# takah29/3d-reconstruction-from-multi-view-exp

Measured on AMD Instinct MI355X. Metric: BA iterations/sec + residual-Jacobian GObs/s, 1M pts x 100 cams fp64, higher is better.
Workload: dtype f64

## Files before the change

### 3d-reconstruction-from-multi-view-exp_amd/csrc/mvba.hip

```cpp
#include <dlfcn.h>
#include <hip/hip_runtime.h>
#include <rccl/rccl.h>

#include <algorithm>
#include <atomic>
#include <chrono>
#include <cmath>
#include <cstdlib>
#include <cstring>
#include <thread>
#include <type_traits>
#include <utility>
#include <vector>

#include "mvba_common.h"
#include "mvba_host.h"

namespace mvba {
thread_local std::string g_err;
}
using namespace mvba;

namespace {
struct Rccl {
// ... 13 lines not shown
int rccl_load() {
  if (g_rccl.lib) return MVBA_OK;
  const char *names[] = {"librccl.so.1", "librccl.so"};
  void *lib = nullptr;
  std::string origin;
  for (const char *n : names)
    if (!lib && (lib = dlopen(n, RTLD_NOW | RTLD_NOLOAD))) origin = std::string(n) + " (already mapped by the process)";
  if (const char *ev = getenv("MVBA_RCCL_LIBRARY"))
    if (!lib && (lib = dlopen(ev, RTLD_NOW | RTLD_GLOBAL))) origin = ev;
  for (const char *n : {"/opt/rocm/lib/librccl.so.1", "librccl.so.1"})
    if (!lib && (lib = dlopen(n, RTLD_NOW | RTLD_GLOBAL))) origin = n;
  if (!lib) return fail(MVBA_ERR_RCCL, std::string("librccl not found: ") + dlerror());
  Rccl r;
  r.lib = lib;
  r.origin = origin;
#define BIND(field, sym)                                                                       \
  if (!(r.field = reinterpret_cast<decltype(r.field)>(dlsym(lib, sym))))                       \
    return fail(MVBA_ERR_RCCL, std::string("librccl (") + origin + ") lacks " + sym)
  BIND(GetVersion, "ncclGetVersion");
  BIND(GetUniqueId, "ncclGetUniqueId");
  BIND(CommInitRank, "ncclCommInitRank");
  BIND(CommDestroy, "ncclCommDestroy");
  BIND(AllReduce, "ncclAllReduce");
  BIND(AllGather, "ncclAllGather");
  BIND(GetErrorString, "ncclGetErrorString");
#undef BIND
  if (r.GetVersion(&r.version) != ncclSuccess) return fail(MVBA_ERR_RCCL, "ncclGetVersion failed");
  const int major = r.version >= 10000 ? r.version / 10000 : r.version / 1000;
  if (major != NCCL_MAJOR)
    return fail(MVBA_ERR_RCCL, "librccl (" + origin + ") is NCCL " + std::to_string(r.version) + ", this library was built against " +
                                   std::to_string(NCCL_VERSION_CODE));
  g_rccl = r;
  return MVBA_OK;
}
}

namespace {

__device__ __forceinline__ double wave_sum(double v) {
#pragma unroll
  for (int off = 32; off > 0; off >>= 1) v += __shfl_down(v, off, 64);
  return v;
}

__device__ __forceinline__ double block_sum(double v, double *s_red ) {
  v = wave_sum(v);
  const int lane = threadIdx.x & 63, w = threadIdx.x >> 6;
  if (lane == 0) s_red[w] = v;
  __syncthreads();
  double t = 0.0;
  if (threadIdx.x == 0) {
    const int nw = (blockDim.x + 63) >> 6;
    for (int i = 0; i < nw; ++i) t += s_red[i];
  }
  return t;
}

__device__ __forceinline__ void load_cams_to_lds(const double *__restrict__ cam15, int m, double f0,
                                                 double *s_cam) {
  for (int k = threadIdx.x; k < m; k += blockDim.x) expand_cam(cam15 + (size_t)k * CAM_IN, f0, s_cam + k * CAM_LDS);
}

__host__ __device__ __forceinline__ size_t strip_offset(int k, int m) {
  return 81 * ((size_t)k * m - (size_t)k * (k - 1) / 2);
}

__device__ __forceinline__ int keep_index(int i, int gauge_axis) {
  if (i < 3) return i;
  return (i + 6 < 12 + gauge_axis) ? i + 6 : i + 7;
}

#define MVBA_CONST_AS __attribute__((address_space(4)))
template <typename T>
__device__ __forceinline__ const T MVBA_CONST_AS *as_const(const T *p) {
#pragma clang diagnostic push
#pragma clang diagnostic ignored "-Wold-style-cast"
  return (const T MVBA_CONST_AS *)p;
#pragma clang diagnostic pop
}

constexpr int REC = 8;
constexpr int LDS_CAMERAS = 646;

#define MVBA_RESID_JAC_ARGS                                                                                                 \
  long long nobs, int m, const double *__restrict__ cam15, const double *__restrict__ X, const int *__restrict__ obs_pt,   \
      const int *__restrict__ cam_idx, const double2 *__restrict__ xy, double f0, const int *__restrict__ tile_start,     \
      int n_tiles, double2 *__restrict__ rec, double *__restrict__ PL, const int *__restrict__ tile_slot,                 \
      double *__restrict__ PLsplit, const double *__restrict__ gcam
struct LossArgs {
  double b;
  double *sqw;
};
template <bool GCAM, int LOSS = LOSS_SQUARED, typename... Robust>
__global__ __launch_bounds__(1024, 4) void k_resid_jac(MVBA_RESID_JAC_ARGS, Robust... robust) {
  extern __shared__ __attribute__((aligned(16))) double smem[];
  double *s_cam = smem;
  const int lane = threadIdx.x & 63, wave = threadIdx.x >> 6, nwave = blockDim.x >> 6;
  double2 *stage = reinterpret_cast<double2 *>(smem + (GCAM ? 0 : ((m * CAM_LDS + 1) & ~1))) + wave * (64 * REC);
  constexpr int CS = 65;
  double *contrib = reinterpret_cast<double *>(stage);
  int *seg_start = reinterpret_cast<int *>(contrib + 9 * CS), *seg_pt = seg_start + 66;
  if (!GCAM) {
    load_cams_to_lds(cam15, m, f0, s_cam);
    __syncthreads();
  }
  for (int tile = blockIdx.x * nwave + wave; tile < n_tiles; tile += gridDim.x * nwave) {
    const int ts0 = tile_start[tile], ts1 = tile_start[tile + 1];
    const bool split = ts0 < 0;
    const int slot = split ? as_const(tile_slot)[tile] : 0;
    const long long wbase = split ? ~ts0 : ts0;
    const int n = (int)((ts1 < 0 ? ~ts1 : ts1) - wbase);
    const long long o = wbase + lane;
    const bool live = lane < n;
    int a = -1;
    double c9[9] = {0, 0, 0, 0, 0, 0, 0, 0, 0};
    if (live) {
      a = obs_pt[o];
      const int k = cam_idx[o];
      const double2 z = xy[o];
      const double *Xa = X + 3 * (size_t)a;
      ObsJ J;
      obs_math(Xa[0], Xa[1], Xa[2], GCAM ? gcam + (size_t)k * CAM_LDS : s_cam + k * CAM_LDS, z.x, z.y, f0, J);
      if constexpr (LOSS != LOSS_SQUARED) {
        const LossArgs la = (robust, ...);
        const double sw = loss_sqrt_w<LOSS>(J.e0 * J.e0 + J.e1 * J.e1, la.b);
        J.e0 *= sw;
        J.e1 *= sw;
#pragma unroll
        for (int rr = 0; rr < 2; ++rr) {
#pragma unroll
          for (int i = 0; i < 3; ++i) J.jx[rr][i] *= sw;
          J.jc[rr][0] *= sw;
#pragma unroll
          for (int i = 6; i < 9; ++i) J.jc[rr][i] *= sw;
        }
        la.sqw[o] = sw;
      }
      double2 *row = stage + lane * REC;
      const int sw = lane & 7;
      row[0 ^ sw] = make_double2(J.jx[0][0], J.jx[1][0]);
      row[1 ^ sw] = make_double2(J.jx[0][1], J.jx[1][1]);
      row[2 ^ sw] = make_double2(J.jx[0][2], J.jx[1][2]);
      row[3 ^ sw] = make_double2(J.jc[0][0], J.jc[1][0]);
      row[4 ^ sw] = make_double2(J.jc[0][6], J.jc[1][6]);
      row[5 ^ sw] = make_double2(J.jc[0][7], J.jc[1][7]);
      row[6 ^ sw] = make_double2(J.jc[0][8], J.jc[1][8]);
      row[7 ^ sw] = make_double2(J.e0, J.e1);
      c9[0] = 2.0 * (J.jx[0][0] * J.jx[0][0] + J.jx[1][0] * J.jx[1][0]);
      c9[1] = 2.0 * (J.jx[0][0] * J.jx[0][1] + J.jx[1][0] * J.jx[1][1]);
      c9[2] = 2.0 * (J.jx[0][0] * J.jx[0][2] + J.jx[1][0] * J.jx[1][2]);
      c9[3] = 2.0 * (J.jx[0][1] * J.jx[0][1] + J.jx[1][1] * J.jx[1][1]);
      c9[4] = 2.0 * (J.jx[0][1] * J.jx[0][2] + J.jx[1][1] * J.jx[1][2]);
      c9[5] = 2.0 * (J.jx[0][2] * J.jx[0][2] + J.jx[1][2] * J.jx[1][2]);
      c9[6] = 2.0 * (J.jx[0][0] * J.e0 + J.jx[1][0] * J.e1);
      c9[7] = 2.0 * (J.jx[0][1] * J.e0 + J.jx[1][1] * J.e1);
      c9[8] = 2.0 * (J.jx[0][2] * J.e0 + J.jx[1][2] * J.e1);
    }
    wave_sync();
#pragma unroll
    for (int q = 0; q < REC; ++q) {
      const int ol = q * 8 + (lane >> 3), pos = lane & 7;
      const double2 v = stage[ol * REC + pos];
      if (ol < n) rec[(wbase + ol) * REC + (pos ^ (ol & 7))] = v;
    }
    wave_sync();
    const int a_prev = __shfl_up(a, 1, 64);
    const bool head = live && (lane == 0 || a != a_prev);
    const unsigned long long heads = __ballot(head);
    const int nseg = __popcll(heads);
#pragma unroll
    for (int q = 0; q < 9; ++q) contrib[q * CS + lane] = c9[q];
    if (head) {
      const int rank = __popcll(heads & ((1ull << lane) - 1ull));
      seg_start[rank] = lane;
      seg_pt[rank] = a;
    }
    if (lane == 0) seg_start[nseg] = n;
    wave_sync();
    const int sl = lane / 9, comp = lane - 9 * sl;
    for (int s0 = 0; s0 < nseg; s0 += 7) {
      const int sg = s0 + sl;
      if (sl < 7 && sg < nseg) {
        const int i0 = seg_start[sg], i1 = seg_start[sg + 1];
        double acc = 0.0;
        for (int i = i0; i < i1; ++i) acc += contrib[comp * CS + i];
        if (split) PLsplit[9 * (size_t)slot + comp] = acc;
        else PL[9 * (size_t)seg_pt[sg] + comp] = acc;
      }
    }
    wave_sync();
  }
}

__global__ void k_sum_split(int n_split, const int4 *__restrict__ splits ,
                            const double *__restrict__ PLsplit, double *__restrict__ PL) {
  const int t = blockIdx.x * blockDim.x + threadIdx.x, sp = t / 9, comp = t - 9 * sp;
  if (sp >= n_split) return;
  const int4 d = splits[sp];
  double v = 0.0;
  for (int q = 0; q < d.z; ++q) v += PLsplit[9 * (size_t)(d.y + q) + comp];
  PL[9 * (size_t)d.x + comp] = v;
}

constexpr int PBS = 16;
constexpr int PACE_STRIDE = 32;
__global__ __launch_bounds__(256) void k_point_inv(long long npts, double c, const double *__restrict__ PL,
                                                   double *__restrict__ PB, int *__restrict__ flag,
                                                   double *__restrict__ Ab, long long nAb, int *__restrict__ prog, long long nprog, int want_r) {
  __shared__ double2 s_out[256 * 8];
  double *s_in = reinterpret_cast<double *>(s_out);
  const long long a0 = (long long)blockIdx.x * 256, a = a0 + threadIdx.x;
  for (long long i = a; i < nAb; i += (long long)gridDim.x * blockDim.x) Ab[i] = 0.0;
  for (long long i = a; i < nprog; i += (long long)gridDim.x * blockDim.x) prog[i] = 0;
  if (a0 >= npts) return;
  const int np = (int)min<long long>(256, npts - a0);
  {
    double t[9];
#pragma unroll
    for (int i = 0; i < 9; ++i) t[i] = PL[9 * a0 + min((int)threadIdx.x + 256 * i, 9 * np - 1)];
#pragma unroll
    for (int i = 0; i < 9; ++i)
      if ((int)threadIdx.x + 256 * i < 9 * np) s_in[threadIdx.x + 256 * i] = t[i];
  }
  __syncthreads();
  double in[9];
#pragma unroll
  for (int i = 0; i < 9; ++i) in[i] = s_in[9 * min((int)threadIdx.x, np - 1) + i];
  __syncthreads();
  if (threadIdx.x < np) {
    const double s = 1.0 + c;
    const double xx = in[0] * s, xy = in[1], xz = in[2], yy = in[3] * s, yz = in[4], zz = in[5] * s;
    const double c00 = yy * zz - yz * yz, c01 = xz * yz - xy * zz, c02 = xy * yz - xz * yy;
    const double det = xx * c00 + xy * c01 + xz * c02;
    if (!(det != 0.0) || !isfinite(det)) atomicOr(flag, 1);
    const double id = 1.0 / det;
    const double i00 = c00 * id, i01 = c01 * id, i02 = c02 * id;
    const double i11 = (xx * zz - xz * xz) * id, i12 = (xy * xz - xx * yz) * id, i22 = (xx * yy - xy * xy) * id;
    const double g0 = in[6], g1 = in[7], g2 = in[8];
    double2 *out = s_out + 8 * threadIdx.x;
    const int sw = threadIdx.x & 7;
    out[0 ^ sw] = make_double2(i00, i01);
    out[1 ^ sw] = make_double2(i02, i11);
    out[2 ^ sw] = make_double2(i12, i22);
    out[3 ^ sw] = make_double2(i00 * g0 + i01 * g1 + i02 * g2, i01 * g0 + i11 * g1 + i12 * g2);
    out[4 ^ sw] = make_double2(i02 * g0 + i12 * g1 + i22 * g2, 1.0);
    if (want_r) {
      const double d0 = i00, q0 = d0 != 0.0 ? 1.0 / d0 : 0.0, l10 = i01 * q0, l20 = i02 * q0;
      const double d1 = i11 - l10 * i01, q1 = d1 != 0.0 ? 1.0 / d1 : 0.0, l21 = (i12 - l20 * i01) * q1;
      const double d2 = i22 - l20 * i02 - l21 * l21 * d1;
      const double a0 = sqrt(fabs(d0)), a1 = sqrt(fabs(d1)), a2 = sqrt(fabs(d2));
      out[4 ^ sw].y = 1.0 + (d0 < 0.0 ? 1.0 : 0.0) + (d1 < 0.0 ? 2.0 : 0.0) + (d2 < 0.0 ? 4.0 : 0.0);
      out[5 ^ sw] = make_double2(a0, l10 * a0);
      out[6 ^ sw] = make_double2(l20 * a0, a1);
      out[7 ^ sw] = make_double2(l21 * a1, a2);
    } else {
      out[5 ^ sw] = out[6 ^ sw] = out[7 ^ sw] = make_double2(0.0, 0.0);
    }
  }
  __syncthreads();
  double2 *dst = reinterpret_cast<double2 *>(PB + PBS * a0);
  for (int e = threadIdx.x; e < 8 * np; e += 256) {
    const int p = e >> 3, sl = e & 7;
    dst[e] = s_out[8 * p + (sl ^ (p & 7))];
  }
}


constexpr int PSTEP = 21;
constexpr int PROW = 7 * 16;
constexpr int PWAVE_LDS = PSTEP * (2 * PROW + 5 * 16);
constexpr int UNIT_STRIDE = 104;
constexpr int SLOT_BUF = PSTEP * (2 * PROW + 3 * 16);
constexpr int SLOT_IDX = 64;
constexpr int SLOT_IDX_RING = 3;
constexpr int PAIRS_LDS = 2 * PWAVE_LDS;
constexpr int SLOT_LDS = 3 * SLOT_BUF + SLOT_IDX_RING * SLOT_IDX * 4;
static_assert(9 * ((SLOT_LDS + 511) / 512 * 512) <= 160 * 1024, "nine waves per CU");

__device__ __forceinline__ void lds_dma16(const void *gsrc, void *lds_wave_uniform) {
  __builtin_amdgcn_global_load_lds(gsrc, (__attribute__((address_space(3))) void *)lds_wave_uniform, 16, 0, 0);
}

struct SlotPace {
  const int *seg_end;
  int *prog;
  int need, nseg, lag;
};
template <bool DIAG, bool BIG, bool SLOTS = false, bool ROBUST = false>
__device__ __forceinline__ void schur_pairs_unit(char *wbuf, const int lane, const long long beg, const int n,
                                                 const int *__restrict__ it_k, const int *__restrict__ it_l,
                                                 const int *__restrict__ it_a, const double2 *__restrict__ rec,
                                                 const double *__restrict__ PB, const double c, const double cu,
                                                 double *__restrict__ out, const int *__restrict__ slot_unit = nullptr,
                                                 const SlotPace pace = SlotPace{nullptr, nullptr, 0, 0, 2},
                                                 const double *__restrict__ sqw = nullptr) {
  static_assert(!(SLOTS && ROBUST), "the slot form has no robust build");
  constexpr int NPS = DIAG ? 5 : 3;
  const int it = lane / 3, cg = lane - 3 * it;
  const int drow = lane / 7, dslot = lane - 7 * drow;
  const int prow = lane / NPS, pslot = lane - NPS * prow;
  const int prow2 = (64 + lane) / 5, pslot2 = (64 + lane) - 5 * prow2;
  const int sel0 = cg == 0 ? 3 : (cg == 1 ? 0 : 4);
  const int sel1 = cg == 0 ? 0 : sel0 + 1, sel2 = cg == 0 ? 0 : sel0 + 2;
  const double al12 = cg == 0 ? 0.0 : 1.0, bx1 = cg == 0 ? 1.0 : 0.0;
  double acc[9][3];
#pragma unroll
  for (int i = 0; i < 9; ++i)
#pragma unroll
    for (int q = 0; q < 3; ++q) acc[i][q] = 0.0;
  double dg[3] = {0.0, 0.0, 0.0}, rb[3] = {0.0, 0.0, 0.0};

  constexpr int LB_OFF = PSTEP * PROW;
  constexpr int PB_OFF = LB_OFF + ((SLOTS && DIAG) ? PSTEP * 16 : PSTEP * PROW);
  constexpr int BUFSZ = SLOTS ? PB_OFF + PSTEP * 16 * NPS : PWAVE_LDS;
  static_assert(!SLOTS || BUFSZ <= SLOT_BUF, "slot form: staging buffer larger than the launch provides");
  constexpr int W_OFF = DIAG ? LB_OFF + PSTEP * 16 : PB_OFF + PSTEP * 16 * NPS;
  static_assert(!ROBUST || (DIAG ? W_OFF + PSTEP * 8 <= PB_OFF : W_OFF + 2 * PSTEP * 8 <= BUFSZ), "robust weights fit the staging buffer");
  int ixk[1][3], ixl[1][3], ixa[1][2];
  int ixw[2] = {0, 0};
  auto load_idx = [&](int s0, int (&xk)[3], int (&xl)[3], int (&xa)[2]) {
    const unsigned last = (unsigned)(min(PSTEP, n - s0) - 1);
    typedef const int __attribute__((address_space(1))) *gint_p;
    auto uni = [](const int *p) {
      const unsigned long long v = (unsigned long long)p;
      const unsigned lo = __builtin_amdgcn_readfirstlane((unsigned)v), hi = __builtin_amdgcn_readfirstlane((unsigned)(v >> 32));
      return (gint_p)(((unsigned long long)hi << 32) | lo);
    };
    typedef const char __attribute__((address_space(1))) *gchar_p;
    auto row_of = [&](int r) {
      unsigned off = min((unsigned)r, last) << 2;
      asm("" : "+v"(off));
      return off;
    };
    auto at = [](gint_p base, unsigned off) { return *(gint_p)((gchar_p)base + off); };
    const gint_p pk = uni(it_k + (beg + s0)), pl = DIAG ? pk : uni(it_l + (beg + s0)), pa = uni(it_a + (beg + s0));
#pragma unroll
    for (int q = 0; q < 3; ++q) {
      const unsigned row = row_of(9 * q + drow);
      xk[q] = at(pk, row);
      if (!DIAG) xl[q] = at(pl, row);
    }
    if (DIAG) xl[0] = at(pk, row_of(lane));
    xa[0] = at(pa, row_of(prow));
    if (DIAG) xa[1] = at(pa, row_of(prow2));
    if (ROBUST) {
      ixw[0] = at(pk, row_of(lane >> 1));
      if (!DIAG) ixw[1] = at(pl, row_of(lane >> 1));
// ... 1945 lines not shown
    if (FILL && lo < NONE && lane == 0)
      while (sg < nSeg && lo >= o_lo + (sg + 1) * segG) seg_end[b * nSeg + sg++] = steps;
    if (lo >= NONE) break;
    const bool take = k0 < NONE && k0 <= lo + skew;
    if (FILL && slot) {
      const long long o = (base + steps) * PSTEP + lane;
      st_k[o] = take ? (int)(it_k[cur] - o_lo) : pad_obs;
      st_l[o] = take ? (int)(it_l[cur] - o_lo) : pad_obs;
      st_a[o] = take ? it_a[cur] : pad_pt;
    }
    if (take) {
      ++cur;
      k0 = k1;
      k1 = cur + 1 < end ? key_at(cur + 1) : NONE;
    }
    ++steps;
  }
  if (FILL) {
    if (lane == 0)
      while (sg < nSeg) seg_end[b * nSeg + sg++] = steps;
  } else if (lane == 0) {
    w_steps[b] = steps;
  }
}

__global__ void k_idx_interleave(long long n_steps, const int *__restrict__ st_k, const int *__restrict__ st_l, const int *__restrict__ st_a,
                                 int *__restrict__ out) {
  const long long t = (long long)blockIdx.x * blockDim.x + threadIdx.x;
  if (t >= n_steps * SLOT_IDX) return;
  const long long st = t / SLOT_IDX;
  const int e = (int)(t - st * SLOT_IDX), which = e / PSTEP, sl = e - which * PSTEP;
  const int *src = which == 0 ? st_k : (which == 1 ? st_l : st_a);
  out[t] = which < 3 ? src[st * PSTEP + sl] : 0;
}

#include "mvba_cov.h"
#include "mvba_map.h"

}

enum { SCHUR_PAIRS = 1, SCHUR_SLOTS = 2, SCHUR_DENSE = 3 };
struct mvba_handle {
  int device = 0;
  hipStream_t stream = nullptr;
  DevBufs mem;
  long long N = 0, nobs = 0;
  int m = 0, gauge_axis = 0, D = 0, ld = 0;
  double f0 = 1.0;
  long long *d_pt_ptr = nullptr;
  int *d_cam = nullptr, *d_obs_pt = nullptr;
  double2 *d_xy = nullptr;
  int *d_tiles = nullptr;
  int *d_tile_slot = nullptr;
  int4 *d_splits = nullptr;
  double *d_PLsplit = nullptr;
  int n_splits = 0;
  int n_tiles = 0;
  bool any_split = false;
  int k1_threads = 512;
  bool use_pairs = true;
  int schur_mode = 2;
  long long n_items = 0, n_items_offdiag = 0, n_slot_items = 0;
  int n_units = 0, rccl_version = 0, q_max = 0, n_waves = 0, slot_nR = 8, slot_nseg = 0;
  long long *d_range_o0 = nullptr;
  int *d_seg_end = nullptr, *d_prog = nullptr;
  bool check_solve = false;
  double check_solve_tol = 1e-8;
  bool gcam = false;
  double *d_cam18 = nullptr, *d_dxi10 = nullptr;
  bool index_on_device = false;
  int4 *d_wdesc = nullptr;
  int *d_it_x = nullptr;
  int *d_wunits = nullptr;
  bool force_big = false;
  int *d_it_k = nullptr, *d_it_l = nullptr, *d_it_a = nullptr, *d_unit_ptr = nullptr, *d_q_ptr = nullptr, *d_q_units = nullptr;
  int4 *d_units = nullptr;
  double *d_partial = nullptr;
  double *d_dense_part = nullptr;
  int *d_dense_obs = nullptr;
  int dense_blocks = 0, dense_tiles = 0;
  double *d_X[2] = {nullptr, nullptr}, *d_cam15[2] = {nullptr, nullptr};
  int cur = 0;
  bool have_params = false, linearized = false, have_trial = false;
  double2 *d_rec = nullptr;
  double *d_PL = nullptr, *d_PB = nullptr;
  double *d_Ab = nullptr, *d_Ared = nullptr, *d_Ztiles = nullptr, *d_Lblk = nullptr, *d_dxi = nullptr, *d_dX = nullptr, *d_lu = nullptr;
  int *d_ipiv = nullptr;
  double *d_partials = nullptr, *d_cost = nullptr, *h_cost = nullptr;
  double *d_mail = nullptr;
  unsigned long long cost_seq = 0;
  bool mail_pending = false;
  int n_partials = 0, cost_grid = 0;
  int *d_flag = nullptr, *h_flag = nullptr;
  unsigned *d_bar = nullptr;
  int n_cu = 1;
  bool chol_onepass = true;
  int trail64_min = 200;
  unsigned barrier_polls = 1u << 22;
  ncclComm_t comm = nullptr;
  mvba_host_allreduce_fn host_ar = nullptr;
  void *host_ar_user = nullptr;
  std::vector<double> host_buf;
  int rank = 0, nranks = 1;
  double *d_allcost = nullptr, *h_allcost = nullptr, *d_sim = nullptr;
  std::vector<double *> snap_slabs;
  long long n_snap = 0;
  int profiling = 0;
  mvba_stats stats{};
  struct Ev { int kid; hipEvent_t a, b; };
  std::vector<Ev> pending;
  std::vector<hipEvent_t> pool;
  double *d_cov_sig = nullptr, *d_cov_panel = nullptr, *d_cov_pts = nullptr, *d_cov_cam = nullptr;
  int loss = LOSS_SQUARED;
  double loss_b = 0.0;
  double *d_sqw = nullptr;
  double2 *d_resid = nullptr;
  double *d_init_cams = nullptr;
  bool mapped = false;
  int n_free = 0, map_ld = 0, map_U = 0;
  std::vector<int> map_col, map_ptr, map_mem;
  int *d_map_col = nullptr, *d_map_ptr = nullptr, *d_map_mem = nullptr;
  double *d_map_x = nullptr, *d_cov_sigv = nullptr;
  int2 *d_map_pairs = nullptr;
  double *d_map_part = nullptr;
  int n_map_pairs = 0, map_nblk = 1;
  int solve_D() const { return mapped ? n_free : D; }
  int solve_ld() const { return mapped ? map_ld : ld; }
};

namespace {

const char *kKernelNames[MVBA_K_COUNT] = {"resid_jac", "point_blocks", "point_inv", "schur",
                                          "allreduce", "solve",        "backsub_cost", "cost"};

struct Timed {
  mvba_handle *h;
  int kid;
  hipEvent_t a = nullptr, b = nullptr;
  bool on = false;
  Timed(mvba_handle *h_, int kid_) : h(h_), kid(kid_) {
    on = kid >= 0 && (h->profiling == 1 || (h->profiling == 2 && (kid == MVBA_K_SCHUR || kid == MVBA_K_RESID_JAC)));
    if (!on) return;
    auto get = [&]() {
      hipEvent_t e;
      if (!h->pool.empty()) { e = h->pool.back(); h->pool.pop_back(); }
      else hipEventCreate(&e);
      return e;
    };
    a = get(); b = get();
    hipEventRecord(a, h->stream);
  }
  ~Timed() {
    if (!on) return;
    hipEventRecord(b, h->stream);
    h->pending.push_back({kid, a, b});
  }
};

void drain_events(mvba_handle *h) {
  for (auto &p : h->pending) {
    float ms = 0.f;
    if (hipEventElapsedTime(&ms, p.a, p.b) == hipSuccess) {
      h->stats.ms[p.kid] += ms;
      h->stats.launches[p.kid] += 1;
    }
    h->pool.push_back(p.a);
// ... 15 lines not shown
}

double *cost_mail(mvba_handle *h) {
  if (h->comm || h->host_ar || h->profiling == 1 || !h->d_mail) return nullptr;
  ++h->cost_seq;
  h->mail_pending = true;
  return h->d_mail;
}

int global_cost(mvba_handle *h, double *E) {
  if (h->mail_pending) {
    h->mail_pending = false;
    volatile unsigned long long *seq = reinterpret_cast<volatile unsigned long long *>(h->h_cost + 2);
    const auto t0 = std::chrono::steady_clock::now();
    bool seen = false;
    for (unsigned spins = 0;; ++spins) {
      if (*seq == h->cost_seq) { seen = true; break; }
      if ((spins & 1023) == 1023 && std::chrono::steady_clock::now() - t0 > std::chrono::seconds(2)) break;
      cpu_relax();
    }
    if (seen) {
      std::atomic_thread_fence(std::memory_order_acquire);
      drain_events(h);
      *E = h->h_cost[0];
      return MVBA_OK;
    }
    int rc = sync_and_drain(h);
    if (rc) return rc;
    *E = h->h_cost[0];
    return MVBA_OK;
  }
  if (h->comm) {
    Timed t(h, MVBA_K_ALLREDUCE);
    ncclResult_t r = g_rccl.AllGather(h->d_cost, h->d_allcost, 2, ncclDouble, h->comm, h->stream);
    if (r != ncclSuccess) return fail(MVBA_ERR_RCCL, std::string("ncclAllGather: ") + g_rccl.GetErrorString(r));
    MVBA_HIP(hipMemcpyAsync(h->h_allcost, h->d_allcost, 2 * sizeof(double) * h->nranks, hipMemcpyDeviceToHost, h->stream));
  } else {
    MVBA_HIP(hipMemcpyAsync(h->h_cost, h->d_cost, 2 * sizeof(double), hipMemcpyDeviceToHost, h->stream));
  }
  int rc = sync_and_drain(h);
  if (rc) return rc;
  if (h->host_ar) {
    std::vector<double> v(2 * (size_t)h->nranks, 0.0);
    v[2 * h->rank] = h->h_cost[0];
    v[2 * h->rank + 1] = (double)*h->h_flag;
    if (h->host_ar(h->host_ar_user, v.data(), (int64_t)v.size())) return fail(MVBA_ERR_RCCL, "host all-reduce callback failed");
    double s = 0.0;
    int fl = 0;
    for (int i = 0; i < h->nranks; ++i) { s += v[2 * i]; fl |= (int)v[2 * i + 1]; }
    *E = s;
    *h->h_flag = fl;
  } else if (h->comm) {
    double s = 0.0;
    int fl = 0;
    for (int i = 0; i < h->nranks; ++i) {
      s += h->h_allcost[2 * i];
      int f;
      memcpy(&f, &h->h_allcost[2 * i + 1], sizeof(int));
      fl |= f;
    }
    *E = s;
    *h->h_flag = fl;
  } else {
    *E = *h->h_cost;
  }
  return MVBA_OK;
}

template <typename... A>
struct LossKernel {
  void (*squared)(A...);
  void (*robust)(A..., LossArgs);
  const void *fn(bool rb) const { return rb ? (const void *)robust : (const void *)squared; }
};
template <typename... A>
LossKernel<A...> loss_kernel(void (*squared)(A...), void (*robust)(A..., LossArgs)) { return {squared, robust}; }

template <typename... A, typename... Args>
void launch_loss(mvba_handle *h, LossKernel<A...> k, dim3 grid, dim3 block, size_t lds, Args... args) {
  if (h->loss != LOSS_SQUARED) hipLaunchKernelGGL(k.robust, grid, block, lds, h->stream, args..., LossArgs{h->loss_b, h->d_sqw});
  else hipLaunchKernelGGL(k.squared, grid, block, lds, h->stream, args...);
}

auto resid_jac_kernel(bool gcam, int loss) {
  if (loss == LOSS_CAUCHY)
    return gcam ? loss_kernel(k_resid_jac<true>, k_resid_jac<true, LOSS_CAUCHY, LossArgs>) : loss_kernel(k_resid_jac<false>, k_resid_jac<false, LOSS_CAUCHY, LossArgs>);
  return gcam ? loss_kernel(k_resid_jac<true>, k_resid_jac<true, LOSS_HUBER, LossArgs>) : loss_kernel(k_resid_jac<false>, k_resid_jac<false, LOSS_HUBER, LossArgs>);
}
auto cost_kernel(bool gcam, int loss) {
  if (loss == LOSS_CAUCHY)
    return gcam ? loss_kernel(k_cost<true>, k_cost<true, LOSS_CAUCHY, LossArgs>) : loss_kernel(k_cost<false>, k_cost<false, LOSS_CAUCHY, LossArgs>);
  return gcam ? loss_kernel(k_cost<true>, k_cost<true, LOSS_HUBER, LossArgs>) : loss_kernel(k_cost<false>, k_cost<false, LOSS_HUBER, LossArgs>);
}
template <int G>
auto backsub_kernel_g(int bt, bool gcam) {
  if (gcam) return loss_kernel(k_backsub<G, 256, true>, k_backsub<G, 256, true, true, LossArgs>);
  if (bt == 1024) return loss_kernel(k_backsub<G, 1024>, k_backsub<G, 1024, false, true, LossArgs>);
  if (bt == 512) return loss_kernel(k_backsub<G, 512>, k_backsub<G, 512, false, true, LossArgs>);
  return loss_kernel(k_backsub<G>, k_backsub<G, 256, false, true, LossArgs>);
}
auto backsub_kernel(int G, int bt, bool gcam) {
  return G == 2 ? backsub_kernel_g<2>(bt, gcam) : (G == 4 ? backsub_kernel_g<4>(bt, gcam) : backsub_kernel_g<8>(bt, gcam));
}
template <int T>
auto dense_kernel_t(bool table) {
  return table ? loss_kernel(k_schur_dense<T, true>, k_schur_dense<T, true, true, LossArgs>)
               : loss_kernel(k_schur_dense<T, false>, k_schur_dense<T, false, true, LossArgs>);
}
auto dense_kernel(int T, bool table) {
  switch (T) {
    case 1: return dense_kernel_t<1>(table);
    case 2: return dense_kernel_t<2>(table);
    case 3: return dense_kernel_t<3>(table);
    case 4: return dense_kernel_t<4>(table);
    case 5: return dense_kernel_t<5>(table);
    case 6: return dense_kernel_t<6>(table);
    case 7: return dense_kernel_t<7>(table);
    case 8: return dense_kernel_t<8>(table);
    case 9: return dense_kernel_t<9>(table);
    case 10: return dense_kernel_t<10>(table);
    case 11: return dense_kernel_t<11>(table);
    default: return dense_kernel_t<12>(table);
  }
}
size_t dense_lds_bytes(int T, int mm) {
  const int CH = dense_ch(T);
  return sizeof(double) * ((size_t)2 * 3 * CH * 16 * T + (size_t)2 * CH * mm * 32) + sizeof(double2) * CH * ((size_t)mm * REC + 8) +
         sizeof(double) * (CH * (size_t)mm + 2 * 3 * CH);
}

size_t k1_lds_bytes(int m, bool gcam, int threads) {
  return (size_t)((gcam ? 0 : ((m * CAM_LDS + 1) & ~1)) + (threads / 64) * 64 * 2 * REC) * sizeof(double);
}
size_t cam_lds_bytes(int m, bool gcam, bool with_dxi) { return gcam ? 0 : (size_t)m * (CAM_LDS + (with_dxi ? DXI_LDS : 0)) * sizeof(double); }

void cam_tables(mvba_handle *h, const double *cam15, const double *dxi) {
  if (h->gcam) hipLaunchKernelGGL(k_cam_tables, dim3((h->m + 255) / 256), dim3(256), 0, h->stream, h->m, cam15, dxi, h->f0, h->d_cam18, h->d_dxi10);
}
int launch_cost(mvba_handle *h, const double *cam15, const double *X) {
  const size_t lds = cam_lds_bytes(h->m, h->gcam, false);
  cam_tables(h, cam15, nullptr);
  launch_loss(h, cost_kernel(h->gcam, h->loss), dim3(h->cost_grid), dim3(lds > 40 * 1024 ? 512 : 256), lds, h->nobs, h->m, cam15, X,
              h->d_obs_pt, h->d_cam, h->d_xy, h->f0, h->d_partials, h->d_cam18);
  double *mail = cost_mail(h);
  const unsigned long long seq = h->cost_seq;
  hipLaunchKernelGGL(k_sum_partials, dim3(1), dim3(1024), 0, h->stream, h->d_partials, h->cost_grid, h->d_cost, h->d_flag, mail, seq);
  MVBA_HIP(hipGetLastError());
  return MVBA_OK;
}

struct CreateKnobs {
  bool schur_set = false;
  bool schur_slots = false, schur_pairs = false, schur_dense = false;
  bool index_host = false, index_global = false;
  bool force_big = false;
  bool chol_launches = false;
  int trail64_min = 200;
  unsigned barrier_polls = 1u << 22;
  bool check_solve = false;
  double check_solve_tol = 1e-8;
  bool timing = false;
};

CreateKnobs read_create_knobs() {
  CreateKnobs k;
  auto is = [](const char *ev, const char *v) { return ev && !strcmp(ev, v); };
  const char *schur = getenv("MVBA_SCHUR");
  k.schur_set = schur != nullptr;
  k.schur_slots = is(schur, "slots");
  k.schur_pairs = is(schur, "pairs");
  k.schur_dense = is(schur, "dense");
  const char *index = getenv("MVBA_INDEX");
  k.index_host = is(index, "host");
  k.index_global = is(index, "global");
  k.force_big = getenv("MVBA_FORCE_BIG") != nullptr;
  k.chol_launches = is(getenv("MVBA_CHOL"), "launches");
  if (const char *ev = getenv("MVBA_TRAIL64_MIN")) k.trail64_min = std::max(0, atoi(ev));
  if (const char *ev = getenv("MVBA_CHOL_BARRIER_POLLS")) k.barrier_polls = (unsigned)std::max(0LL, atoll(ev));
  if (const char *ev = getenv("MVBA_CHECK_SOLVE")) {
    const double v = atof(ev);
    k.check_solve = v != 0.0;
    if (v > 0.0 && v < 1.0) k.check_solve_tol = v;
  }
  k.timing = getenv("MVBA_CREATE_TIMING") != nullptr;
  return k;
}

#include "mvba_create.h"

}

extern "C" {

const char *mvba_version(void) { return "mvba 0.2 (gfx950)"; }
const char *mvba_last_error(void) { return g_err.c_str(); }
const char *mvba_kernel_name(int32_t k) { return (k >= 0 && k < MVBA_K_COUNT) ? kKernelNames[k] : ""; }

int mvba_device_count(int32_t *count) {
  int n = 0;
  hipError_t e = hipGetDeviceCount(&n);
  if (e != hipSuccess) {
    *count = 0;
    return fail(MVBA_ERR_HIP, std::string("hipGetDeviceCount: ") + hipGetErrorString(e));
  }
  *count = n;
  return MVBA_OK;
}

int mvba_create(const mvba_problem *p, mvba_handle **out) { return create_engine(p, LOSS_SQUARED, 0.0, out); }

int mvba_create_robust(const mvba_problem *p, int32_t loss, double scale, mvba_handle **out) {
  if (!p || !out) return fail(MVBA_ERR_BADARG, "null argument");
  if (loss == LOSS_SQUARED) return create_engine(p, LOSS_SQUARED, 0.0, out);
  if (loss != LOSS_HUBER && loss != LOSS_CAUCHY)
    return fail(MVBA_ERR_BADARG, "loss = " + std::to_string(loss) + " is not a loss (0 squared, 1 Huber, 2 Cauchy)");
  if (!(scale > 0.0) || !std::isfinite(scale))
    return fail(MVBA_ERR_BADARG, "loss scale = " + std::to_string(scale) + " must be finite and > 0 for a robust loss");
  if (!(p->f0 > 0.0) || !std::isfinite(p->f0)) return fail(MVBA_ERR_BADARG, "a robust loss needs f0 > 0");
  const double r = scale / p->f0;
  return create_engine(p, loss, r * r, out);
}

void mvba_destroy(mvba_handle *h) {
  if (!h) return;
  hipSetDevice(h->device);
  if (h->stream) hipStreamSynchronize(h->stream);
  if (h->comm) g_rccl.CommDestroy(h->comm);
  h->mem.release_all();
  if (h->h_cost) hipHostFree(h->h_cost);
  if (h->h_allcost) hipHostFree(h->h_allcost);
  for (auto &p : h->pending) { hipEventDestroy(p.a); hipEventDestroy(p.b); }
  for (auto e : h->pool) hipEventDestroy(e);
  if (h->stream) hipStreamDestroy(h->stream);
  delete h;
}

int mvba_set_params(mvba_handle *h, const double *X, const double *f, const double *u, const double *t, const double *R) {
  if (!h || !X || !f || !u || !t || !R) return fail(MVBA_ERR_BADARG, "null argument");
  MVBA_HIP(hipSetDevice(h->device));
  std::vector<double> cam((size_t)h->m * CAM_IN);
  for (int k = 0; k < h->m; ++k) {
    double *c = cam.data() + (size_t)k * CAM_IN;
    c[0] = f[k]; c[1] = u[2 * k]; c[2] = u[2 * k + 1];
    for (int i = 0; i < 3; ++i) c[3 + i] = t[3 * k + i];
    for (int i = 0; i < 9; ++i) c[6 + i] = R[9 * k + i];
  }
  MVBA_HIP(hipMemcpyAsync(h->d_X[h->cur], X, sizeof(double) * 3 * h->N, hipMemcpyHostToDevice, h->stream));
  MVBA_HIP(hipMemcpyAsync(h->d_cam15[h->cur], cam.data(), sizeof(double) * cam.size(), hipMemcpyHostToDevice, h->stream));
  MVBA_HIP(hipStreamSynchronize(h->stream));
  h->have_params = true; h->linearized = false; h->have_trial = false;
  return MVBA_OK;
}

int mvba_get_params(mvba_handle *h, double *X, double *f, double *u, double *t, double *R) {
  if (!h || !X || !f || !u || !t || !R) return fail(MVBA_ERR_BADARG, "null argument");
  if (!h->have_params) return fail(MVBA_ERR_STATE, "no parameters set");
  MVBA_HIP(hipSetDevice(h->device));
  std::vector<double> cam((size_t)h->m * CAM_IN);
  MVBA_HIP(hipMemcpyAsync(X, h->d_X[h->cur], sizeof(double) * 3 * h->N, hipMemcpyDeviceToHost, h->stream));
  MVBA_HIP(hipMemcpyAsync(cam.data(), h->d_cam15[h->cur], sizeof(double) * cam.size(), hipMemcpyDeviceToHost, h->stream));
  MVBA_HIP(hipStreamSynchronize(h->stream));
  for (int k = 0; k < h->m; ++k) {
    const double *c = cam.data() + (size_t)k * CAM_IN;
    f[k] = c[0]; u[2 * k] = c[1]; u[2 * k + 1] = c[2];
    for (int i = 0; i < 3; ++i) t[3 * k + i] = c[3 + i];
    for (int i = 0; i < 9; ++i) R[9 * k + i] = c[6 + i];
  }
  return MVBA_OK;
}

int mvba_apply_similarity(mvba_handle *h, const double *R0, const double *t0, double scale) {
  if (!h || !R0 || !t0) return fail(MVBA_ERR_BADARG, "null argument");
  if (!h->have_params) return fail(MVBA_ERR_STATE, "no parameters set");
  MVBA_HIP(hipSetDevice(h->device));
  double T[13];
  memcpy(T, R0, 9 * sizeof(double));
  memcpy(T + 9, t0, 3 * sizeof(double));
  T[12] = scale;
  if (!h->d_sim) {
    int rc = h->mem.alloc(&h->d_sim, 13);
    if (rc) return rc;
  }
  MVBA_HIP(hipMemcpyAsync(h->d_sim, T, sizeof(T), hipMemcpyHostToDevice, h->stream));
  const long long n = std::max<long long>(h->N, h->m);
  hipLaunchKernelGGL(k_similarity, dim3((unsigned)((n + 255) / 256)), dim3(256), 0, h->stream, h->N, h->m, h->d_X[h->cur],
                     h->d_cam15[h->cur], h->d_sim);
  MVBA_HIP(hipGetLastError());
  MVBA_HIP(hipStreamSynchronize(h->stream));
  h->linearized = false; h->have_trial = false;
  return MVBA_OK;
}

int mvba_cost(mvba_handle *h, double *E) {
  if (!h || !E) return fail(MVBA_ERR_BADARG, "null argument");
  if (!h->have_params) return fail(MVBA_ERR_STATE, "no parameters set");
  MVBA_HIP(hipSetDevice(h->device));
  {
    Timed t(h, MVBA_K_COST);
    int rc = launch_cost(h, h->d_cam15[h->cur], h->d_X[h->cur]);
    if (rc) return rc;
  }
  return global_cost(h, E);
}

namespace {
void launch_resid_jac(mvba_handle *h) {
  const int kt = h->k1_threads;
  cam_tables(h, h->d_cam15[h->cur], nullptr);
  const int wpb = kt / 64;
  const int grid = std::max(1, std::min(2048 * 256 / kt, (h->n_tiles + wpb - 1) / wpb));
  launch_loss(h, resid_jac_kernel(h->gcam, h->loss), dim3(grid), dim3(kt), k1_lds_bytes(h->m, h->gcam, kt), h->nobs, h->m, h->d_cam15[h->cur],
              h->d_X[h->cur], h->d_obs_pt, h->d_cam, h->d_xy, h->f0, h->d_tiles, h->n_tiles, h->d_rec, h->d_PL,
              h->d_tile_slot, h->d_PLsplit, h->d_cam18);
  if (h->n_splits)
    hipLaunchKernelGGL(k_sum_split, dim3((9 * h->n_splits + 255) / 256), dim3(256), 0, h->stream, h->n_splits, h->d_splits,
                       h->d_PLsplit, h->d_PL);
}

void launch_point_inv(mvba_handle *h, double c) {
  const int m = h->m;
  const size_t n9 = 9 * (size_t)m, nA = strip_offset(m, m);
  const long long nAb = (long long)(nA + n9);
  const unsigned grid = (unsigned)std::max<long long>((h->N + 255) / 256, std::min<long long>((nAb + 1023) / 1024, 4096));
  hipLaunchKernelGGL(k_point_inv, dim3(std::max(grid, 1u)), dim3(256), 0, h->stream, h->N, c, h->d_PL, h->d_PB, h->d_flag,
                     h->d_Ab, nAb, h->d_prog, (long long)h->slot_nR * h->slot_nseg * PACE_STRIDE,
                     h->schur_mode == SCHUR_DENSE ? 1 : 0);
}

void launch_schur(mvba_handle *h, double c) {
  const int m = h->m;
  const size_t nA = strip_offset(m, m);
  double *d_A = h->d_Ab, *d_b = h->d_Ab + nA;
  if (h->use_pairs) {
    const bool big = (std::max<long long>(h->nobs, h->N) + 1) * 128LL >= (1LL << 32) || h->force_big;
    if (h->schur_mode == SCHUR_SLOTS) {
      if (h->n_waves)
        hipLaunchKernelGGL(k_schur_slots, dim3(h->n_waves), dim3(64), SLOT_LDS, h->stream, h->d_wdesc,
                           h->d_wunits, h->d_it_x, (const int *)nullptr, (const int *)nullptr, h->d_rec, h->d_PB, c, h->f0, h->d_partial,
                           h->slot_nR, h->d_seg_end, h->d_prog, h->slot_nseg, SLOT_LAG, h->d_range_o0);
    } else if (h->n_units) {
      auto launch = [&](auto kern, auto... robust) {
        hipLaunchKernelGGL(kern, dim3(8 * h->q_max), dim3(64), PAIRS_LDS, h->stream, h->d_units, h->d_q_ptr, h->d_q_units, h->d_it_k, h->d_it_l,
                           h->d_it_a, h->d_rec, h->d_PB, c, h->f0, h->d_partial, robust...);
      };
      if (h->loss != LOSS_SQUARED) launch(big ? k_schur_pairs_big_robust : k_schur_pairs_robust, (const double *)h->d_sqw);
      else launch(big ? k_schur_pairs_big : k_schur_pairs);
    }
    hipLaunchKernelGGL(k_schur_reduce, dim3((unsigned)((long long)m * (m + 1) / 2)), dim3(128), 0, h->stream, m, h->d_unit_ptr,
                       h->d_partial, d_A, d_b);
  } else if (h->schur_mode == SCHUR_DENSE) {
    const int T = (9 * m + 15) / 16;
    launch_loss(h, dense_kernel(T, h->d_dense_obs != nullptr), dim3(h->dense_blocks), dim3(64 * (dense_consumers(T) + dense_ch(T))), dense_lds_bytes(T, m),
                (const double2 *)h->d_rec, (const double *)h->d_PB, (const int *)h->d_dense_obs, (long long)h->N, m, 1.0 / h->f0, h->d_dense_part);
    const long long n_el = (long long)nA + 9 * m;
    hipLaunchKernelGGL(k_schur_dense_finish, dim3((unsigned)((n_el + 3) / 4)), dim3(256), 0, h->stream, m, T, h->dense_blocks,
                       (const double *)h->d_dense_part, c, d_A, d_b);
  }
}

int allreduce_Ab(mvba_handle *h, bool timed) {
  const int m = h->m;
  const size_t n9 = 9 * (size_t)m, nA = strip_offset(m, m);
  if (h->comm) {
    Timed t(h, timed ? MVBA_K_ALLREDUCE : -1);
    ncclResult_t r = g_rccl.AllReduce(h->d_Ab, h->d_Ab, nA + n9, ncclDouble, ncclSum, h->comm, h->stream);
    if (r != ncclSuccess) return fail(MVBA_ERR_RCCL, std::string("ncclAllReduce: ") + g_rccl.GetErrorString(r));
  } else if (h->host_ar) {
    h->host_buf.resize(nA + n9);
    MVBA_HIP(hipMemcpyAsync(h->host_buf.data(), h->d_Ab, sizeof(double) * (nA + n9), hipMemcpyDeviceToHost, h->stream));
    MVBA_HIP(hipStreamSynchronize(h->stream));
    const auto t0 = std::chrono::steady_clock::now();
    if (h->host_ar(h->host_ar_user, h->host_buf.data(), (int64_t)(nA + n9))) return fail(MVBA_ERR_RCCL, "host all-reduce callback failed");
    MVBA_HIP(hipMemcpyAsync(h->d_Ab, h->host_buf.data(), sizeof(double) * (nA + n9), hipMemcpyHostToDevice, h->stream));
    if (timed && h->profiling) {
      h->stats.ms[MVBA_K_ALLREDUCE] += std::chrono::duration<double, std::milli>(std::chrono::steady_clock::now() - t0).count();
      h->stats.launches[MVBA_K_ALLREDUCE] += 1;
    }
  }
  return MVBA_OK;
}

void launch_map_tied(mvba_handle *h, double *M, int ld, int mirror) {
  if (!h->n_map_pairs) return;
  hipLaunchKernelGGL(k_map_tied, dim3(h->n_map_pairs, h->map_nblk), dim3(256), 0, h->stream, h->m, (const double *)h->d_Ab,
                     (const int *)h->d_map_ptr, (const int *)h->d_map_mem, (const int2 *)h->d_map_pairs, h->d_map_part);
  hipLaunchKernelGGL(k_map_tied_finish, dim3((h->n_map_pairs + 255) / 256), dim3(256), 0, h->stream, h->n_map_pairs, h->map_nblk, ld,
                     mirror, (const int2 *)h->d_map_pairs, (const double *)h->d_map_part, M);
}

void launch_factor(mvba_handle *h) {
  const int m = h->m, D = h->solve_D();
  double *d_A = h->d_Ab, *d_b = h->d_Ab + strip_offset(m, m);
  const int ld = h->solve_ld();
  const int ntc = (D + NB - 1) / NB;
  if (h->mapped) {
    const int U = h->map_U, ntu = (U + NB - 1) / NB;
    hipLaunchKernelGGL(k_map_compact, dim3(ntu * (ntu + 1) / 2 + (D + 255) / 256), dim3(256), 0, h->stream, D, ld, m, U, ntu, d_A, d_b,
                       h->d_map_ptr, h->d_map_mem, h->d_Ared, h->d_bar, 1 + 4 * ((D + SBW - 1) / SBW));
    if (U < D)
      hipLaunchKernelGGL(k_map_rows, dim3((D + 63) / 64, D - U), dim3(256), 0, h->stream, D, ld, m, U, d_A, h->d_map_ptr, h->d_map_mem,
                         h->d_Ared);
    launch_map_tied(h, h->d_Ared, ld, 0);
  } else
  hipLaunchKernelGGL(k_compact, dim3(ntc * (ntc + 1) / 2 + (D + 255) / 256), dim3(256), 0, h->stream, D, ld, m, h->gauge_axis, ntc, d_A, d_b,
                     h->d_Ared, h->d_bar, 1 + 4 * ((D + SBW - 1) / SBW));
  for (int jS = 0; jS < D; jS += SBW) {
    const int jE = std::min(jS + SBW, D);
    hipLaunchKernelGGL(k_chol_super, dim3((D + 1 - jE + 63) / 64), dim3(SUPER_THREADS), SUPER_LDS, h->stream, h->d_Ared, ld, D, jS,
                       h->d_Ztiles + (size_t)(jS / NB) * NB * NB, h->d_Lblk + (size_t)(jS / SBW) * SBW * SBW, h->d_flag);
    if (jE < D) {
      const int nt32 = (D + 1 - jE + NB - 1) / NB, nt64 = (D + 1 - jE + TB - 1) / TB;
      if (jE - jS == SBW && nt64 * (nt64 + 1) / 2 >= h->trail64_min)
        hipLaunchKernelGGL(k_chol_trail64, dim3(nt64 * (nt64 + 1) / 2), dim3(256), TRAIL64_LDS, h->stream, h->d_Ared, ld, D, jS, jE);
      else
        hipLaunchKernelGGL(k_chol_trail32, dim3(nt32 * (nt32 + 1) / 2), dim3(256), 0, h->stream, h->d_Ared, ld, D, jS, jE);
    }
  }
}
}

int mvba_linearize(mvba_handle *h) {
  if (!h) return fail(MVBA_ERR_BADARG, "null handle");
  if (!h->have_params) return fail(MVBA_ERR_STATE, "no parameters set");
  MVBA_HIP(hipSetDevice(h->device));
  if (h->nobs) {
    Timed t(h, MVBA_K_RESID_JAC);
    launch_resid_jac(h);
  }
  MVBA_HIP(hipGetLastError());
  h->linearized = true; h->have_trial = false;
  h->stats.n_linearize++;
  return MVBA_OK;
}

namespace {
double *solve_x(mvba_handle *h) { return h->mapped ? h->d_map_x : h->d_dxi; }
void launch_expand(mvba_handle *h) {
  const size_t n9 = 9 * (size_t)h->m;
  if (h->mapped && h->solve_D() > 0)
    hipLaunchKernelGGL(k_map_expand, dim3((unsigned)((n9 + 255) / 256)), dim3(256), 0, h->stream, (int)n9, h->gauge_axis, h->d_map_col,
                       h->d_map_x, h->d_dxi);
}

void launch_solve(mvba_handle *h, bool onepass) {
  const int m = h->m, D = h->solve_D();
  double *d_x = solve_x(h);
  Timed t(h, MVBA_K_SOLVE);
  if (D == 0) {
    hipMemsetAsync(h->d_dxi, 0, sizeof(double) * 9 * (size_t)m, h->stream);
    return;
  }
  launch_factor(h);
  const int ld = h->solve_ld();
  const int S = (D + SBW - 1) / SBW;
  if (onepass && (S == 1 || S < h->n_cu)) {
    const int ngrp = ((S - 1) * SBW + 31) / 32, nbulk = S > 1 ? std::max(1, std::min(h->n_cu - S, ngrp)) : 0;
    hipLaunchKernelGGL(k_chol_backsolve_all<true>, dim3(S + nbulk), dim3(SUPER_THREADS),
                       BACKSOLVE_LDS, h->stream, h->d_Ared, ld, D, m, h->gauge_axis, h->d_Ztiles, h->d_Lblk, d_x, h->d_flag,
                       h->d_bar, h->barrier_polls);
  } else
  for (int jS = ((D - 1) / SBW) * SBW; jS >= 0; jS -= SBW) {
    const int jE = std::min(jS + SBW, D), jE2 = std::min(jE + SBW, D);
    const int nwg = (jE == D) ? 1 : 1 + (jS + 255) / 256;
    hipLaunchKernelGGL(k_chol_backsolve, dim3(nwg), dim3(256), 0, h->stream, h->d_Ared, ld, D, m, h->gauge_axis, h->d_Ztiles,
                       h->d_Lblk + (size_t)(jS / SBW) * SBW * SBW, d_x, jS, jE, jE2);
  }
  launch_expand(h);
}

int launch_lu_solve(mvba_handle *h) {
  const int m = h->m, D = h->solve_D();
  double *d_A = h->d_Ab, *d_b = h->d_Ab + strip_offset(m, m), *d_x = solve_x(h);
  if (!h->d_lu) {
    int rc_ = h->mem.alloc(&h->d_lu, (size_t)h->D * (h->D + 1));
    if (rc_) return rc_;
    rc_ = h->mem.alloc(&h->d_ipiv, (size_t)h->D);
    if (rc_) return rc_;
  }
  MVBA_HIP(hipMemsetAsync(h->d_flag, 0, sizeof(int), h->stream));
  Timed t(h, MVBA_K_SOLVE);
  if (h->mapped) {
    hipLaunchKernelGGL(k_map_full, dim3((D + 1 + 255) / 256, D), dim3(256), 0, h->stream, D, m, d_A, d_b, h->d_map_ptr, h->d_map_mem, h->d_lu);
    launch_map_tied(h, h->d_lu, D + 1, 1);
  } else
  hipLaunchKernelGGL(k_compact_full, dim3((D + 1 + 255) / 256, D), dim3(256), 0, h->stream, D, m, h->gauge_axis, d_A, d_b, h->d_lu);
  for (int j0 = 0; j0 < D; j0 += LU_NB) {
    const int nb = std::min(LU_NB, D - j0), right = D + 1 - (j0 + nb);
    hipLaunchKernelGGL(k_lu_panel, dim3(1), dim3(1024), 0, h->stream, h->d_lu, D, j0, nb, h->d_ipiv, h->d_flag);
    hipLaunchKernelGGL(k_lu_swap, dim3((D + 1 - nb + 255) / 256), dim3(256), 0, h->stream, h->d_lu, D, j0, nb, h->d_ipiv);
    if (right > 0) hipLaunchKernelGGL(k_lu_trsm, dim3((right + 255) / 256), dim3(256), 0, h->stream, h->d_lu, D, j0, nb);
    const int below = D - (j0 + nb);
    if (below > 0)
      hipLaunchKernelGGL(k_lu_gemm, dim3((right + 63) / 64, (below + 63) / 64), dim3(256), 0, h->stream, h->d_lu, D, j0, nb);
  }
  hipLaunchKernelGGL(k_lu_backsub, dim3(1), dim3(1024), 0, h->stream, h->d_lu, D, m, h->gauge_axis, d_x);
  launch_expand(h);
  return MVBA_OK;
}

int launch_tail_and_cost(mvba_handle *h, double *E_trial) {
  const int m = h->m, trial = 1 - h->cur;
  {
    Timed t(h, MVBA_K_BACKSUB_COST);
    hipLaunchKernelGGL(k_update_cams, dim3((m + 63) / 64), dim3(64), 0, h->stream, m, h->d_cam15[h->cur], h->d_dxi,
                       h->d_cam15[trial]);
    if (h->N) {
      const size_t lds = cam_lds_bytes(m, h->gcam, true);
      cam_tables(h, h->d_cam15[h->cur], h->d_dxi);
      const double deg = (double)h->nobs / (double)h->N;
      const int G = deg <= 40.0 ? 2 : (deg <= 100.0 ? 4 : 8);
      const int bt = lds > 80 * 1024 ? 1024 : (lds > 40 * 1024 ? 512 : 256);
      const int nblk = (int)std::min<long long>(4096 * 256 / bt, (h->N * G + bt - 1) / bt);
      launch_loss(h, backsub_kernel(G, bt, h->gcam), dim3(nblk), dim3(bt), lds, h->N, m, h->d_pt_ptr, h->d_cam, h->d_PB, h->d_dxi,
                  h->d_X[h->cur], h->d_cam15[h->cur], h->f0, h->d_X[trial], h->d_dX, h->d_cam18, h->d_dxi10);
    }
    int rc = launch_cost(h, h->d_cam15[trial], h->d_X[trial]);
    if (rc) return rc;
  }
  return global_cost(h, E_trial);
}

int check_solve_residual(mvba_handle *h) {
  const int m = h->m, D = h->solve_D();
  const size_t n9 = 9 * (size_t)m, nA = strip_offset(m, m);
  std::vector<double> Ab(nA + n9), x(n9);
  MVBA_HIP(hipMemcpyAsync(Ab.data(), h->d_Ab, sizeof(double) * (nA + n9), hipMemcpyDeviceToHost, h->stream));
  MVBA_HIP(hipMemcpyAsync(x.data(), h->d_dxi, sizeof(double) * n9, hipMemcpyDeviceToHost, h->stream));
  MVBA_HIP(hipStreamSynchronize(h->stream));
  auto kept = [&](size_t g) { return !((g >= 3 && g <= 8) || g == (size_t)(12 + h->gauge_axis)); };
  std::vector<double> r(n9, 0.0), an(n9, 0.0);
  for (int k = 0; k < m; ++k) {
    const double *Ak = Ab.data() + strip_offset(k, m);
    const int Wk = 9 * (m - k);
    for (int i = 0; i < 9; ++i)
      for (int c = 0; c < Wk; ++c) {
        const size_t gi = 9 * (size_t)k + i, gj = 9 * (size_t)k + c;
        const double a = Ak[(size_t)i * Wk + c];
        r[gi] += a * x[gj]; an[gi] += std::fabs(a * x[gj]);
        if (c >= 9) { r[gj] += a * x[gi]; an[gj] += std::fabs(a * x[gi]); }
      }
  }
  double worst = 0.0;
  if (h->mapped) {
    for (int j = 0; j < D; ++j) {
      double res = 0.0, scale = 0.0;
      for (int q = h->map_ptr[j]; q < h->map_ptr[j + 1]; ++q) {
        const size_t g = (size_t)h->map_mem[q];
        res += Ab[nA + g] - r[g];
        scale += an[g] + std::fabs(Ab[nA + g]);
      }
      worst = std::max(worst, scale > 0.0 ? std::fabs(res) / scale : 0.0);
    }
  } else
  for (size_t g = 0; g < n9; ++g)
    if (kept(g)) {
      const double bg = Ab[nA + g], scale = an[g] + std::fabs(bg);
      worst = std::max(worst, scale > 0.0 ? std::fabs(bg - r[g]) / scale : 0.0);
    }
  if (!(worst <= h->check_solve_tol))
    return fail(MVBA_ERR_STATE, "MVBA_CHECK_SOLVE: the dense solve left a relative residual of " + std::to_string(worst) +
                                    " on the reduced camera system (a stale hand-over in the back-substitution?)");
  return MVBA_OK;
}
}

int mvba_try_step(mvba_handle *h, double c, double *E_trial) {
  if (!h || !E_trial) return fail(MVBA_ERR_BADARG, "null argument");
  if (!h->linearized) return fail(MVBA_ERR_STATE, "try_step before linearize");
  MVBA_HIP(hipSetDevice(h->device));
  {
    Timed t(h, MVBA_K_POINT_INV);
    launch_point_inv(h, c);
  }
  if (h->use_pairs || h->schur_mode == SCHUR_DENSE) {
    Timed t(h, MVBA_K_SCHUR);
    launch_schur(h, c);
  }
  MVBA_HIP(hipGetLastError());
  int rc = allreduce_Ab(h, true);
  if (rc) return rc;
  launch_solve(h, h->chol_onepass);
  MVBA_HIP(hipGetLastError());
  h->stats.n_try_step++;
  rc = launch_tail_and_cost(h, E_trial);
  if (rc) return rc;
  if ((*h->h_flag & 8) && !(*h->h_flag & 1)) {
    MVBA_HIP(hipMemsetAsync(h->d_flag, 0, sizeof(int), h->stream));
    h->chol_onepass = false;
    h->stats.n_barrier_fallback++;
    launch_solve(h, false);
    rc = launch_tail_and_cost(h, E_trial);
    if (rc) return rc;
  }
  if ((*h->h_flag & 2) && !(*h->h_flag & (1 | 8))) {
    rc = launch_lu_solve(h);
    if (rc) return rc;
    h->stats.n_lu_fallback++;
    rc = launch_tail_and_cost(h, E_trial);
    if (rc) return rc;
  }
  if (*h->h_flag) {
    const int fl = *h->h_flag;
    hipMemsetAsync(h->d_flag, 0, sizeof(int), h->stream);
    if (fl & 8) return fail(MVBA_ERR_HIP, "k_chol_backsolve_all: a wait for a progress word timed out twice (is another process holding the CUs?)");
    return fail(MVBA_ERR_SINGULAR, (fl & 1) ? "Singular matrix" : "Singular matrix (reduced camera system)");
  }
  if (h->check_solve) {
    rc = check_solve_residual(h);
    if (rc) return rc;
  }
  h->have_trial = true;
  return MVBA_OK;
}

int mvba_commit(mvba_handle *h) {
  if (!h) return fail(MVBA_ERR_BADARG, "null handle");
  if (!h->have_trial) return fail(MVBA_ERR_STATE, "commit without a trial step");
  h->cur = 1 - h->cur;
  h->have_trial = false; h->linearized = false;
  h->stats.n_commit++;
  return MVBA_OK;
}

int mvba_set_parameter_map(mvba_handle *h, const int32_t *col, int32_t n_free) {
  if (!h) return fail(MVBA_ERR_BADARG, "null handle");
  MVBA_HIP(hipSetDevice(h->device));
  const int m = h->m, n9 = 9 * m;
  auto is_gauge = [&](int g) { return (g >= 3 && g <= 8) || g == 12 + h->gauge_axis; };
  if (!col) {
    h->mapped = false;
    h->have_trial = false;
    return MVBA_OK;
  }
  if (n_free < 0 || n_free > h->D)
    return fail(MVBA_ERR_BADARG, "mvba_set_parameter_map: n_free = " + std::to_string(n_free) + " must be in 0 .. 9 n_images - 7 = " + std::to_string(h->D));
  std::vector<int> cnt(n_free + 1, 0), first(n_free, -1);
  for (int g = 0; g < n9; ++g) {
    const int j = col[g];
    if (j < -1 || j >= n_free)
      return fail(MVBA_ERR_BADARG, "mvba_set_parameter_map: col[" + std::to_string(g) + "] = " + std::to_string(j) + " is neither -1 nor below n_free = " + std::to_string(n_free));
    if (j >= 0 && is_gauge(g))
      return fail(MVBA_ERR_BADARG, "mvba_set_parameter_map: col[" + std::to_string(g) + "] is a gauge slot and must be -1");
    if (j < 0) continue;
    if (first[j] < 0) first[j] = g;
    else if (g % 9 != first[j] % 9 || g % 9 > 2)
      return fail(MVBA_ERR_BADARG, "mvba_set_parameter_map: col[" + std::to_string(g) + "] ties slot " + std::to_string(g) + " to slot " + std::to_string(first[j]) +
                                       " (unknown " + std::to_string(j) + "): only the same intrinsic parameter (f, u or v) of different cameras can be tied");
    ++cnt[j];
  }
  for (int j = 0; j < n_free; ++j)
    if (!cnt[j]) return fail(MVBA_ERR_BADARG, "mvba_set_parameter_map: unknown " + std::to_string(j) + " has no parameter slot");
  bool is_default = n_free == h->D;
  for (int g = 0, j = 0; is_default && g < n9; ++g) is_default = col[g] == (is_gauge(g) ? -1 : j++);
  h->have_trial = false;
  if (is_default) {
    h->mapped = false;
    return MVBA_OK;
  }
  std::vector<int> ptr(n_free + 1, 0), mem;
  for (int j = 0; j < n_free; ++j) ptr[j + 1] = ptr[j] + cnt[j];
  mem.resize(std::max(ptr[n_free], 1));
  {
    std::vector<int> fill(ptr.begin(), ptr.end() - 1);
    for (int g = 0; g < n9; ++g)
      if (col[g] >= 0) mem[fill[col[g]]++] = g;
  }
  int U = 0;
  while (U < n_free && cnt[U] == 1) ++U;
  std::vector<int2> pairs;
  int max_cnt = 1;
  {
    std::vector<int> tied;
    for (int j = 0; j < n_free; ++j)
      if (cnt[j] > 1) { tied.push_back(j); max_cnt = std::max(max_cnt, cnt[j]); }
    for (size_t a = 0; a < tied.size(); ++a)
      for (size_t b = 0; b <= a; ++b) pairs.push_back(make_int2(tied[a], tied[b]));
  }
  const int nblk = std::min(64, (max_cnt + 7) / 8);
  int2 *d_pairs = nullptr;
  double *d_part = nullptr;
  if (!pairs.empty()) {
    int rc = h->mem.alloc(&d_pairs, pairs.size());
    if (!rc) rc = h->mem.alloc(&d_part, pairs.size() * (size_t)nblk);
    if (rc) {
      h->mem.release(d_pairs);
      return rc;
    }
  }
  if (!h->d_map_col) {
    int rc = h->mem.alloc(&h->d_map_col, (size_t)n9);
    if (!rc) rc = h->mem.alloc(&h->d_map_ptr, (size_t)h->D + 1);
    if (!rc) rc = h->mem.alloc(&h->d_map_mem, (size_t)n9);
    if (!rc) rc = h->mem.alloc(&h->d_map_x, (size_t)n9 + 16);
    if (rc) {
      h->mem.release(h->d_map_col); h->mem.release(h->d_map_ptr); h->mem.release(h->d_map_mem); h->mem.release(h->d_map_x);
      h->mem.release(d_pairs); h->mem.release(d_part);
      return rc;
    }
  }
  MVBA_HIP(hipStreamSynchronize(h->stream));
  h->mem.release(h->d_map_pairs);
  h->mem.release(h->d_map_part);
  h->d_map_pairs = d_pairs;
  h->d_map_part = d_part;
  h->n_map_pairs = (int)pairs.size();
  h->map_nblk = nblk;
  if (!pairs.empty()) MVBA_HIP(hipMemcpy(h->d_map_pairs, pairs.data(), sizeof(int2) * pairs.size(), hipMemcpyHostToDevice));
  MVBA_HIP(hipMemcpy(h->d_map_col, col, sizeof(int) * n9, hipMemcpyHostToDevice));
  MVBA_HIP(hipMemcpy(h->d_map_ptr, ptr.data(), sizeof(int) * (n_free + 1), hipMemcpyHostToDevice));
  MVBA_HIP(hipMemcpy(h->d_map_mem, mem.data(), sizeof(int) * mem.size(), hipMemcpyHostToDevice));
  h->map_col.assign(col, col + n9);
  h->map_ptr = ptr;
  h->map_mem = mem;
  h->n_free = n_free;
  h->map_ld = (n_free + 3) & ~3;
  h->map_U = U;
  h->mapped = true;
  return MVBA_OK;
}

int mvba_residuals(mvba_handle *h, double *e) {
  if (!h || !e) return fail(MVBA_ERR_BADARG, "null argument");
  if (!h->have_params) return fail(MVBA_ERR_STATE, "no parameters set");
  MVBA_HIP(hipSetDevice(h->device));
  if (!h->nobs) return MVBA_OK;
  if (!h->d_resid) {
    int rc = h->mem.alloc(&h->d_resid, h->nobs);
    if (rc) return rc;
  }
  const size_t lds = h->gcam ? 0 : (size_t)h->m * CAM_LDS * sizeof(double);
  cam_tables(h, h->d_cam15[h->cur], nullptr);
  const unsigned grid = (unsigned)std::min<long long>(4096, (h->nobs + 255) / 256);
  hipLaunchKernelGGL(h->gcam ? k_residuals<true> : k_residuals<false>, dim3(grid), dim3(256), lds, h->stream, h->nobs, h->m,
                     (const double *)h->d_cam15[h->cur], (const double *)h->d_X[h->cur], (const int *)h->d_obs_pt, (const int *)h->d_cam,
                     (const double2 *)h->d_xy, h->f0, h->d_resid, (const double *)h->d_cam18);
  MVBA_HIP(hipGetLastError());
  MVBA_HIP(hipMemcpyAsync(e, h->d_resid, sizeof(double2) * h->nobs, hipMemcpyDeviceToHost, h->stream));
  MVBA_HIP(hipStreamSynchronize(h->stream));
  return MVBA_OK;
}

int mvba_covariance(mvba_handle *h, double *point_cov, double *cam_cov, double *cam_cov_full, double *timings_ms) {
  if (!h) return fail(MVBA_ERR_BADARG, "null handle");
  if (h->loss != LOSS_SQUARED)
    return fail(MVBA_ERR_BADARG, "mvba_covariance: the covariance is defined for the squared loss only (this engine has a robust loss)");
  if (!h->have_params) return fail(MVBA_ERR_STATE, "no parameters set");
  MVBA_HIP(hipSetDevice(h->device));
  const int m = h->m, D = h->solve_D(), ld = h->solve_ld(), nt = (D + NB - 1) / NB;
  const size_t n_sig = sig_block(m, m, m);
  auto free_cov = [&]() {
    for (double **q : {&h->d_cov_sig, &h->d_cov_panel, &h->d_cov_pts, &h->d_cov_cam}) h->mem.release(*q);
  };
  int local_rc = MVBA_OK;
  if (!h->d_cov_sig || !h->d_cov_panel || !h->d_cov_pts || !h->d_cov_cam) {
    free_cov();
    local_rc = h->mem.alloc(&h->d_cov_sig, n_sig);
    if (!local_rc) local_rc = h->mem.alloc(&h->d_cov_panel, 2 * (size_t)h->D * NB);
    if (!local_rc) local_rc = h->mem.alloc(&h->d_cov_pts, 6 * (size_t)h->N);
    if (!local_rc) local_rc = h->mem.alloc(&h->d_cov_cam, 81 * (size_t)m);
    if (local_rc) free_cov();
  }
  hipEvent_t ev[5] = {};
  struct EvFree { hipEvent_t *e; ~EvFree() { for (int i = 0; i < 5; ++i) if (e[i]) hipEventDestroy(e[i]); } } ev_free{ev};
  for (auto &e : ev)
    if (!local_rc && hipEventCreate(&e) != hipSuccess) local_rc = fail(MVBA_ERR_HIP, "hipEventCreate failed");
  const int mv = (D + 6) / 9 + 1;
  if (!local_rc && h->mapped && D > 0 && !h->d_cov_sigv) local_rc = h->mem.alloc(&h->d_cov_sigv, n_sig);
  const bool sharded = h->comm || h->host_ar;
  if (local_rc && !sharded) return local_rc;
  const std::string local_err = local_rc ? g_err : std::string();
  double *d_b = h->d_Ab + strip_offset(m, m);
  if (!local_rc) {
    MVBA_HIP(hipEventRecord(ev[0], h->stream));
    if (h->nobs) launch_resid_jac(h);
    h->linearized = true; h->have_trial = false;
    launch_point_inv(h, 0.0);
    launch_schur(h, 0.0);
    MVBA_HIP(hipGetLastError());
  } else {
    MVBA_HIP(hipMemsetAsync(d_b + 3, 0xFF, sizeof(double), h->stream));
  }
  {
    int rc = allreduce_Ab(h, false);
    if (rc) return rc;
  }
  if (sharded) {
    double mark = 0.0;
    MVBA_HIP(hipMemcpyAsync(&mark, d_b + 3, sizeof(double), hipMemcpyDeviceToHost, h->stream));
    MVBA_HIP(hipStreamSynchronize(h->stream));
    if (local_rc) return fail(local_rc, local_err);
    if (std::isnan(mark))
      return fail(MVBA_ERR_HIP, "mvba_covariance: another rank could not allocate its covariance buffers (or the reduced system is not finite)");
  }
  MVBA_HIP(hipEventRecord(ev[1], h->stream));
  if (D > 0) launch_factor(h);
  MVBA_HIP(hipEventRecord(ev[2], h->stream));
  if (D > 0)
  hipLaunchKernelGGL(k_cov_assemble, dim3(nt), dim3(256), 0, h->stream, h->d_Ared, ld, D, (const double *)h->d_Ztiles,
                     (const double *)h->d_Lblk);
  double *panel[2] = {h->d_cov_panel, h->d_cov_panel + (size_t)D * NB};
  for (int J = nt - 1; J >= 0; --J) {
    const int grid = (nt - 1 - J) + (J >= 1 ? nt - J : 0);
    if (grid)
      hipLaunchKernelGGL(k_cov_trtri, dim3(grid), dim3(256), 0, h->stream, h->d_Ared, ld, D, nt, J, (const double *)panel[J & 1],
                         panel[(J + 1) & 1]);
  }
  MVBA_HIP(hipMemsetAsync(h->d_cov_sig, 0, sizeof(double) * n_sig, h->stream));
  if (h->mapped) {
    if (D > 0) {
      hipLaunchKernelGGL(k_cov_lauum, dim3(nt * (nt + 1) / 2), dim3(256), 0, h->stream, (const double *)h->d_Ared, ld, D, nt, mv,
                         h->gauge_axis, h->d_cov_sigv);
      hipLaunchKernelGGL(k_map_cov_expand, dim3((unsigned)((81 * m + 255) / 256), m), dim3(256), 0, h->stream, m, mv, h->gauge_axis,
                         (const int *)h->d_map_col, (const double *)h->d_cov_sigv, h->d_cov_sig);
    }
  } else
  hipLaunchKernelGGL(k_cov_lauum, dim3(nt * (nt + 1) / 2), dim3(256), 0, h->stream, (const double *)h->d_Ared, ld, D, nt, m,
                     h->gauge_axis, h->d_cov_sig);
  MVBA_HIP(hipEventRecord(ev[3], h->stream));
  if (h->N && point_cov) {
    const double pairs = h->N ? 0.5 * ((double)h->nobs / (double)h->N) * ((double)h->nobs / (double)h->N + 1.0) : 0.0;
    const int G = pairs > 48.0 ? 64 : (pairs > 24.0 ? 32 : (pairs > 12.0 ? 16 : 8));
    const unsigned grid = (unsigned)std::min<long long>(8192, (h->N * G + 255) / 256);
    auto kern = G == 64 ? k_point_cov<64> : (G == 32 ? k_point_cov<32> : (G == 16 ? k_point_cov<16> : k_point_cov<8>));
    hipLaunchKernelGGL(kern, dim3(grid), dim3(256), 0, h->stream, h->N, m, (const long long *)h->d_pt_ptr, (const int *)h->d_cam,
                       (const double2 *)h->d_rec, (const double *)h->d_PL, (const double *)h->d_cov_sig, 1.0 / h->f0, h->d_cov_pts,
                       h->d_flag);
  }
  if (cam_cov)
    hipLaunchKernelGGL(k_cov_cam_diag, dim3((unsigned)((81LL * m + 255) / 256)), dim3(256), 0, h->stream, m,
                       (const double *)h->d_cov_sig, h->d_cov_cam);
  MVBA_HIP(hipGetLastError());
  MVBA_HIP(hipEventRecord(ev[4], h->stream));
  int fl = 0;
  MVBA_HIP(hipMemcpyAsync(&fl, h->d_flag, sizeof(int), hipMemcpyDeviceToHost, h->stream));
  MVBA_HIP(hipStreamSynchronize(h->stream));
  if (fl) {
    MVBA_HIP(hipMemsetAsync(h->d_flag, 0, sizeof(int), h->stream));
    MVBA_HIP(hipStreamSynchronize(h->stream));
    if (fl & (1 | COV_FLAG_POINT)) return fail(MVBA_ERR_SINGULAR, "Singular matrix (a point block E_a is singular: a point seen once, or without parallax)");
    return fail(MVBA_ERR_SINGULAR, "Singular matrix (the undamped reduced camera system is not positive definite)");
  }
  if (timings_ms)
    for (int i = 0; i < 4; ++i) {
      float ms = 0.f;
      MVBA_HIP(hipEventElapsedTime(&ms, ev[i], ev[i + 1]));
      timings_ms[i] = ms;
    }
  if (point_cov && h->N) MVBA_HIP(hipMemcpy(point_cov, h->d_cov_pts, sizeof(double) * 6 * h->N, hipMemcpyDeviceToHost));
  if (cam_cov) MVBA_HIP(hipMemcpy(cam_cov, h->d_cov_cam, sizeof(double) * 81 * m, hipMemcpyDeviceToHost));
  if (cam_cov_full) {
    std::vector<double> strip((size_t)SIG_BS * m);
    const size_t n9 = 9 * (size_t)m;
    for (int k = 0; k < m; ++k) {
      MVBA_HIP(hipMemcpy(strip.data(), h->d_cov_sig + sig_block(k, k, m), sizeof(double) * SIG_BS * (m - k), hipMemcpyDeviceToHost));
      for (int l = k; l < m; ++l) {
        const double *b = strip.data() + (size_t)SIG_BS * (l - k);
        for (int i = 0; i < 9; ++i)
          for (int j = 0; j < 9; ++j) {
            const double v = 2.0 * b[9 * i + j];
            cam_cov_full[(9 * (size_t)k + i) * n9 + 9 * (size_t)l + j] = v;
            cam_cov_full[(9 * (size_t)l + j) * n9 + 9 * (size_t)k + i] = v;
          }
      }
    }
  }
  return MVBA_OK;
}

namespace {
constexpr int SNAP_SLAB = 8;
size_t snap_stride(const mvba_handle *h) { return (3 * (size_t)h->N + (size_t)CAM_IN * h->m + 1) & ~(size_t)1; }
}

int mvba_snapshot(mvba_handle *h) {
  if (!h) return fail(MVBA_ERR_BADARG, "null handle");
  if (!h->have_params) return fail(MVBA_ERR_STATE, "no parameters set");
  MVBA_HIP(hipSetDevice(h->device));
  const size_t stride = snap_stride(h);
  const size_t slab = (size_t)(h->n_snap / SNAP_SLAB);
  if (slab >= h->snap_slabs.size()) {
    double *p = nullptr;
    int rc = h->mem.alloc(&p, stride * SNAP_SLAB);
    if (rc) return rc;
    h->snap_slabs.push_back(p);
  }
  double *dst = h->snap_slabs[slab] + stride * (size_t)(h->n_snap % SNAP_SLAB);
  MVBA_HIP(hipMemcpyAsync(dst, h->d_X[h->cur], sizeof(double) * 3 * h->N, hipMemcpyDeviceToDevice, h->stream));
  MVBA_HIP(hipMemcpyAsync(dst + 3 * h->N, h->d_cam15[h->cur], sizeof(double) * CAM_IN * h->m, hipMemcpyDeviceToDevice, h->stream));
  h->n_snap++;
  return MVBA_OK;
}

int mvba_snapshot_count(mvba_handle *h, int64_t *n) {
  if (!h || !n) return fail(MVBA_ERR_BADARG, "null argument");
  *n = h->n_snap;
  return MVBA_OK;
}

int mvba_snapshot_read(mvba_handle *h, int64_t i, double *X, double *f, double *u, double *t, double *R) {
  if (!h || !X || !f || !u || !t || !R) return fail(MVBA_ERR_BADARG, "null argument");
  if (i < 0 || i >= h->n_snap) return fail(MVBA_ERR_BADARG, "no such log entry");
  MVBA_HIP(hipSetDevice(h->device));
  const double *src = h->snap_slabs[(size_t)(i / SNAP_SLAB)] + snap_stride(h) * (size_t)(i % SNAP_SLAB);
  std::vector<double> cam((size_t)h->m * CAM_IN);
  MVBA_HIP(hipMemcpyAsync(X, src, sizeof(double) * 3 * h->N, hipMemcpyDeviceToHost, h->stream));
  MVBA_HIP(hipMemcpyAsync(cam.data(), src + 3 * h->N, sizeof(double) * cam.size(), hipMemcpyDeviceToHost, h->stream));
  MVBA_HIP(hipStreamSynchronize(h->stream));
  for (int k = 0; k < h->m; ++k) {
    const double *c = cam.data() + (size_t)k * CAM_IN;
    f[k] = c[0]; u[2 * k] = c[1]; u[2 * k + 1] = c[2];
    for (int q = 0; q < 3; ++q) t[3 * k + q] = c[3 + q];
    for (int q = 0; q < 9; ++q) R[9 * k + q] = c[6 + q];
  }
  return MVBA_OK;
}

int mvba_snapshot_restore(mvba_handle *h, int64_t i) {
  if (!h) return fail(MVBA_ERR_BADARG, "null handle");
  if (i < 0 || i >= h->n_snap) return fail(MVBA_ERR_BADARG, "no such log entry");
  MVBA_HIP(hipSetDevice(h->device));
  const double *src = h->snap_slabs[(size_t)(i / SNAP_SLAB)] + snap_stride(h) * (size_t)(i % SNAP_SLAB);
  MVBA_HIP(hipMemcpyAsync(h->d_X[h->cur], src, sizeof(double) * 3 * h->N, hipMemcpyDeviceToDevice, h->stream));
  MVBA_HIP(hipMemcpyAsync(h->d_cam15[h->cur], src + 3 * h->N, sizeof(double) * CAM_IN * h->m, hipMemcpyDeviceToDevice, h->stream));
  h->have_params = true; h->linearized = false; h->have_trial = false;
  return MVBA_OK;
}

int mvba_snapshot_clear(mvba_handle *h) {
  if (!h) return fail(MVBA_ERR_BADARG, "null handle");
  h->n_snap = 0;
  return MVBA_OK;
}

int mvba_set_profiling(mvba_handle *h, int32_t enabled) {
  if (!h) return fail(MVBA_ERR_BADARG, "null handle");
  h->profiling = enabled == 2 ? 2 : (enabled != 0);
  return MVBA_OK;
}

int mvba_get_stats(mvba_handle *h, mvba_stats *out) {
  if (!h || !out) return fail(MVBA_ERR_BADARG, "null argument");
  MVBA_HIP(hipSetDevice(h->device));
  int rc = sync_and_drain(h);
  if (rc) return rc;
  *out = h->stats;
  return MVBA_OK;
}

int mvba_get_info(mvba_handle *h, int64_t *out8) {
  if (!h || !out8) return fail(MVBA_ERR_BADARG, "null argument");
  out8[0] = h->n_items;
  out8[1] = h->n_items_offdiag;
  out8[2] = h->n_units;
  out8[3] = h->schur_mode;
  out8[4] = h->rccl_version;
  out8[5] = NCCL_VERSION_CODE;
  out8[6] = h->nranks;
  out8[7] = h->schur_mode == SCHUR_SLOTS ? h->n_slot_items : 0;
  return MVBA_OK;
}

int mvba_reset_stats(mvba_handle *h) {
  if (!h) return fail(MVBA_ERR_BADARG, "null handle");
  MVBA_HIP(hipSetDevice(h->device));
  int rc = sync_and_drain(h);
  if (rc) return rc;
  h->stats = mvba_stats{};
  return MVBA_OK;
}

int mvba_comm_unique_id(void *id128) {
  if (!id128) return fail(MVBA_ERR_BADARG, "null argument");
  static_assert(sizeof(ncclUniqueId) == 128, "ncclUniqueId size");
  if (int rc = rccl_load()) return rc;
  ncclUniqueId id;
  ncclResult_t r = g_rccl.GetUniqueId(&id);
  if (r != ncclSuccess) return fail(MVBA_ERR_RCCL, std::string("ncclGetUniqueId: ") + g_rccl.GetErrorString(r));
  memcpy(id128, &id, 128);
  return MVBA_OK;
}

int mvba_comm_init(mvba_handle *h, const void *id128, int32_t rank, int32_t n_ranks) {
  if (!h || !id128 || n_ranks < 1 || rank < 0 || rank >= n_ranks) return fail(MVBA_ERR_BADARG, "bad comm arguments");
  MVBA_HIP(hipSetDevice(h->device));
  if (int rc = rccl_load()) return rc;
  ncclUniqueId id;
  memcpy(&id, id128, 128);
  ncclResult_t r = g_rccl.CommInitRank(&h->comm, n_ranks, id, rank);
  if (r != ncclSuccess) return fail(MVBA_ERR_RCCL, std::string("ncclCommInitRank: ") + g_rccl.GetErrorString(r));
  h->rank = rank; h->nranks = n_ranks;
  h->rccl_version = g_rccl.version;
  int rc = h->mem.alloc(&h->d_allcost, 2 * (size_t)n_ranks);
  if (rc) return rc;
  MVBA_HIP(hipHostMalloc((void **)&h->h_allcost, 2 * sizeof(double) * n_ranks));
  return MVBA_OK;
}

int mvba_comm_init_host(mvba_handle *h, int32_t rank, int32_t n_ranks, mvba_host_allreduce_fn fn, void *user) {
  if (!h || !fn || n_ranks < 1 || rank < 0 || rank >= n_ranks) return fail(MVBA_ERR_BADARG, "bad comm arguments");
  if (h->comm) return fail(MVBA_ERR_STATE, "handle already has an RCCL communicator");
  h->host_ar = fn; h->host_ar_user = user;
  h->rank = rank; h->nranks = n_ranks;
  return MVBA_OK;
}

int mvba_debug_read(mvba_handle *h, int32_t which, double *out, int64_t capacity, int64_t *n) {
  if (!h || !n) return fail(MVBA_ERR_BADARG, "null argument");
// ... 171 lines not shown
```

### 3d-reconstruction-from-multi-view-exp_amd/csrc/mvba_common.h

```cpp
#pragma once
#include <hip/hip_runtime.h>

#include <cstdint>
#include <cstdio>
#include <string>

#include "../../include/mvba.h"

namespace mvba {

extern thread_local std::string g_err;
inline int fail(int code, const std::string &msg) {
  g_err = msg;
  return code;
}

#define MVBA_HIP(expr)                                                                        \
  do {                                                                                        \
    hipError_t e_ = (expr);                                                                   \
    if (e_ != hipSuccess)                                                                     \
      return ::mvba::fail(MVBA_ERR_HIP, std::string(#expr) + ": " + hipGetErrorString(e_));   \
  } while (0)

constexpr int CAM_IN = 15;
// ... 70 lines not shown
                                                     double f0, double &y0, double &y1, double &y2) {
  double cc[CAM_LDS], dd[DXI_LDS];
  load_row(c, cc);
  load_row(dk, dd);
  c = cc;
  dk = dd;
  const double f = c[0], u = c[1], v = c[2];
  const double d0 = X0 - c[3], d1 = X1 - c[4], d2 = X2 - c[5];
  const double *R = c + 6;
  const double c1 = R[0] * d0 + R[3] * d1 + R[6] * d2;
  const double c2 = R[1] * d0 + R[4] * d1 + R[7] * d2;
  const double c3 = R[2] * d0 + R[5] * d1 + R[8] * d2;
  const double p = f * c1 + u * c3, q = f * c2 + v * c3, r = f0 * c3;
  const double g0 = d1 * dk[8] - d2 * dk[7] - dk[3];
  const double g1 = d2 * dk[6] - d0 * dk[8] - dk[4];
  const double g2 = d0 * dk[7] - d1 * dk[6] - dk[5];
  const double h1 = R[0] * g0 + R[3] * g1 + R[6] * g2;
  const double h2 = R[1] * g0 + R[4] * g1 + R[7] * g2;
  const double h3 = R[2] * g0 + R[5] * g1 + R[8] * g2;
  const double dpdf = (p - c[16] * r) * c[15], dqdf = (q - c[17] * r) * c[15];
  const double dp = dpdf * dk[0] + f * h1 + u * h3, dq = dqdf * dk[0] + f * h2 + v * h3, dr = f0 * h3;
  const double inv_r2 = 1.0 / (r * r), cu = 1.0 / f0;
  const double s0 = (r * dp - p * dr) * inv_r2 + cu * dk[1];
  const double s1 = (r * dq - q * dr) * inv_r2 + cu * dk[2];
  const double w0 = r * f * s0, w1 = r * f * s1, w2 = r * (u * s0 + v * s1) - f0 * (p * s0 + q * s1);
  const double sc = 2.0 * inv_r2;
  y0 = sc * (R[0] * w0 + R[1] * w1 + R[2] * w2);
  y1 = sc * (R[3] * w0 + R[4] * w1 + R[5] * w2);
  y2 = sc * (R[6] * w0 + R[7] * w1 + R[8] * w2);
}

enum { LOSS_SQUARED = 0, LOSS_HUBER = 1, LOSS_CAUCHY = 2 };
template <int LOSS>
__host__ __device__ __forceinline__ double loss_rho(double s, double b) {
  if (LOSS == LOSS_HUBER) return s <= b ? s : 2.0 * sqrt(b * s) - b;
  if (LOSS == LOSS_CAUCHY) return b * log1p(s / b);
  return s;
}
template <int LOSS>
__host__ __device__ __forceinline__ double loss_sqrt_w(double s, double b) {
  if (LOSS == LOSS_HUBER) return s <= b ? 1.0 : sqrt(sqrt(b / s));
  if (LOSS == LOSS_CAUCHY) return rsqrt(1.0 + s / b);
  return 1.0;
}

__host__ __device__ __forceinline__ void obs_resid(double X0, double X1, double X2, const double *c, double x, double y,
                                                   double f0, double &e0, double &e1) {
  double cc[CAM_LDS];
  load_row(c, cc);
  c = cc;
  const double d0 = X0 - c[3], d1 = X1 - c[4], d2 = X2 - c[5];
  const double *R = c + 6;
  const double c1 = R[0] * d0 + R[3] * d1 + R[6] * d2;
  const double c2 = R[1] * d0 + R[4] * d1 + R[7] * d2;
  const double c3 = R[2] * d0 + R[5] * d1 + R[8] * d2;
  const double p = c[0] * c1 + c[1] * c3, q = c[0] * c2 + c[2] * c3, r = f0 * c3;
  e0 = p / r - x / f0;
  e1 = q / r - y / f0;
}

__host__ __device__ __forceinline__ double obs_cost(double X0, double X1, double X2, const double *c,
                                                    double x, double y, double f0) {
  double cc[CAM_LDS];
  load_row(c, cc);
  c = cc;
  const double d0 = X0 - c[3], d1 = X1 - c[4], d2 = X2 - c[5];
  const double *R = c + 6;
  const double c1 = R[0] * d0 + R[3] * d1 + R[6] * d2;
  const double c2 = R[1] * d0 + R[4] * d1 + R[7] * d2;
  const double c3 = R[2] * d0 + R[5] * d1 + R[8] * d2;
  const double p = c[0] * c1 + c[1] * c3, q = c[0] * c2 + c[2] * c3, r = f0 * c3;
  const double e0 = p / r - x / f0, e1 = q / r - y / f0;
  return e0 * e0 + e1 * e1;
}

__host__ __device__ __forceinline__ void expand_cam(const double *in15, double f0, double *out18) {
#pragma unroll
  for (int i = 0; i < CAM_IN; ++i) out18[i] = in15[i];
  out18[15] = 1.0 / in15[0];
  out18[16] = in15[1] / f0;
  out18[17] = in15[2] / f0;
}


#if defined(__HIP_DEVICE_COMPILE__)
__device__ __forceinline__ void wave_sync() {
  __builtin_amdgcn_fence(__ATOMIC_RELEASE, "wavefront");
  __builtin_amdgcn_wave_barrier();
  __builtin_amdgcn_fence(__ATOMIC_ACQUIRE, "wavefront");
}
#else
__device__ inline void wave_sync() {}
#endif

}
```

### 3d-reconstruction-from-multi-view-exp_amd/csrc/mvba_create.h

```cpp

__global__ __launch_bounds__(256) void k_xy_from_planes(const double2 *__restrict__ planes, long long N, int m, double2 *__restrict__ xy) {
  const long long a = (long long)blockIdx.x * 256 + threadIdx.x;
  const int k = blockIdx.y;
  if (a < N) xy[a * m + k] = planes[(long long)k * N + a];
}

#define CR(x) do { int rc_ = (x); if (rc_) return rc_; } while (0)
#define CRH(x) do { hipError_t e_ = (x); if (e_ != hipSuccess) return fail(MVBA_ERR_HIP, std::string(#x) + ": " + hipGetErrorString(e_)); } while (0)

struct CreateTimer {
  bool on;
  std::chrono::steady_clock::time_point t_last = std::chrono::steady_clock::now();
  void lap(const char *what) {
    if (!on) return;
    const auto now = std::chrono::steady_clock::now();
    fprintf(stderr, "mvba_create: %-28s %8.1f ms\n", what, std::chrono::duration<double, std::milli>(now - t_last).count());
    t_last = now;
  }
};

int validate_problem(const mvba_problem *p, std::vector<int> &obs_pt) {
  if (p->n_points < 0 || p->n_images < 2 || p->n_obs < 0 || !p->pt_ptr || (p->n_obs && (!p->cam_idx || !p->xy)))
    return fail(MVBA_ERR_BADARG, "bad problem sizes or null arrays (need n_images >= 2)");
  if (p->gauge_axis != 0 && p->gauge_axis != 1) return fail(MVBA_ERR_BADARG, "gauge_axis must be 0 or 1");
  if (p->xy_layout != 0 && p->xy_layout != 1) return fail(MVBA_ERR_BADARG, "xy_layout must be 0 (observation order) or 1 (image planes)");
  if (p->xy_layout == 1 && p->n_obs != p->n_points * (int64_t)p->n_images)
    return fail(MVBA_ERR_BADARG, "xy as image planes needs every point observed in every image (n_obs = n_points * n_images)");
  static_assert(LDS_CAMERAS * CAM_LDS + 8 * 64 * 2 * 8 + 2 <= 160 * 1024 / 8 && LDS_CAMERAS * (CAM_LDS + DXI_LDS) <= 160 * 1024 / 8,
                "the camera tables of LDS_CAMERAS cameras fit one workgroup's LDS");
  constexpr int MAX_CAMERAS = 4096;
  if (p->n_images > MAX_CAMERAS)
    return fail(MVBA_ERR_BADARG, "n_images = " + std::to_string(p->n_images) + " exceeds the " + std::to_string(MAX_CAMERAS) +
                                     " cameras this build solves a dense reduced system for");
  if (p->pt_ptr[0] != 0 || p->pt_ptr[p->n_points] != p->n_obs) return fail(MVBA_ERR_BADARG, "pt_ptr does not span n_obs");
  if (p->n_obs >= (1LL << 31) || p->n_points >= (1LL << 31))
    return fail(MVBA_ERR_BADARG, "n_obs and n_points per handle must be < 2^31");
  const long long N = p->n_points, nobs = p->n_obs;
  const int m = p->n_images;
  obs_pt.resize(nobs);
  for (long long a = 0; a < N; ++a) {
    const long long o0 = p->pt_ptr[a], o1 = p->pt_ptr[a + 1];
    if (o1 < o0 || o1 > nobs) return fail(MVBA_ERR_BADARG, "pt_ptr not monotone / out of range");
    for (long long o = o0; o < o1; ++o) {
      const int k = p->cam_idx[o];
      if (k < 0 || k >= m) return fail(MVBA_ERR_BADARG, "cam_idx out of range");
      if (o > o0 && p->cam_idx[o - 1] >= k) return fail(MVBA_ERR_BADARG, "cam_idx must ascend within a point");
      obs_pt[o] = (int)a;
    }
  }
  return MVBA_OK;
}

struct K1Tiles {
  std::vector<int> tiles, tile_slot;
  std::vector<int4> splits;
  int n_split_slots = 0;
  bool any_split = false;
};

K1Tiles build_k1_tiles(const mvba_problem *p) {
  K1Tiles t;
  const long long N = p->n_points;
  long long cur0 = 0, fill = 0;
  auto flush = [&](bool split_flag) { t.tiles.push_back(split_flag ? ~(int)cur0 : (int)cur0); };
  for (long long a = 0; a < N; ++a) {
    const long long d = p->pt_ptr[a + 1] - p->pt_ptr[a];
    if (d > 64) {
      if (fill) { flush(false); cur0 += fill; fill = 0; }
      t.any_split = true;
      t.splits.push_back(make_int4((int)a, t.n_split_slots, (int)((d + 63) / 64), 0));
      for (long long q = 0; q < d; q += 64) {
        t.tile_slot.resize(t.tiles.size() + 1, -1);
        t.tile_slot[t.tiles.size()] = t.n_split_slots++;
        flush(true);
        cur0 += std::min<long long>(64, d - q);
      }
      continue;
    }
    if (fill + d > 64) { flush(false); cur0 += fill; fill = 0; }
    fill += d;
  }
  if (fill) { flush(false); cur0 += fill; }
  t.tiles.push_back((int)p->n_obs);
  return t;
}

int k1_block_threads(int m, bool gcam) {
  int best_w = 8, best_tot = 0;
  for (int w = 8; w <= 16; ++w) {
    const size_t per = k1_lds_bytes(m, gcam, 64 * w);
    if (per > 160 * 1024) break;
    const int tot = std::min<int>(16, (int)(160 * 1024 / per) * w);
    if (tot > best_tot) { best_tot = tot; best_w = w; }
  }
  return 64 * best_w;
}

inline long long pair_id(int m, int k, int l) { return (long long)k * m - (long long)k * (k - 1) / 2 + (l - k); }

template <typename F>
void on_threads(int n_thr, F body) {
  std::vector<std::thread> th;
  for (int t = 1; t < n_thr; ++t) th.emplace_back(body, t);
  body(0);
  for (auto &x : th) x.join();
}

struct IndexInput {
  const mvba_problem *p;
  long long N, nobs, P;
  int m, n_thr;
  hipStream_t stream;
  const long long *d_pt_ptr;
  const int *d_cam;
};

struct PairLists {
  std::vector<long long> cnt;
  long long T = 0, Tdiag = 0;
  long long target = 1;
  long long unit_items = 600;
  std::vector<int> S, vp_ptr;
  int VP = 0;
  std::vector<long long> vp_off;
  long long slot_waves = 0;
};

int size_pair_lists(const IndexInput &in, PairLists &L) {
  const int m = in.m;
  const long long P = in.P, N = in.N;
  for (int k = 0; k < m; ++k) L.Tdiag += L.cnt[pair_id(m, k, k)];
  for (long long q = 0; q < P; ++q) L.T += L.cnt[q];
  if (L.T >= (1LL << 40)) return fail(MVBA_ERR_BADARG, "too many (point, camera pair) items");
  const long long T = L.T, Tdiag = L.Tdiag;
  L.target = std::max<long long>(1, (T - Tdiag) / std::max<long long>(1, P - m));
  const double pair_rate = N > 0 && P > m ? (double)(T - Tdiag) / ((double)(P - m) * (double)N) : 0.01;
  L.unit_items = (long long)std::max(300.0, std::min(600.0, 200.0 + 4000.0 * std::sqrt(pair_rate)));
  L.S.resize(P);
  L.vp_ptr.assign(P + 1, 0);
  for (long long q = 0; q < P; ++q) {
    L.S[q] = (int)std::max<long long>(1, std::min<long long>(256, (L.cnt[q] + L.target / 2) / L.target));
    L.vp_ptr[q + 1] = L.vp_ptr[q] + L.S[q];
  }
  L.VP = L.vp_ptr[P];
  long long n_diag_lists = 0, n_off_lists = 0;
  for (int k = 0; k < m; ++k) {
    n_diag_lists += L.S[pair_id(m, k, k)];
    for (int l = k + 1; l < m; ++l) n_off_lists += L.S[pair_id(m, k, l)];
  }
// ... 386 lines not shown
int build_index_device(const IndexInput &in, const SchurPlan &plan, DeviceIndexBuild &dv, DevBufs &engine, SchurIndex &ix, CreateTimer &timer) {
  const PairLists &L = plan.L;
  const PointRanges &R = plan.R;
  const long long N = in.N, P = in.P;
  const int m = in.m, nR = R.nR, VP = L.VP;
  hipStream_t stream = in.stream;
  DevBufs &tmp = dv.mem;
  int *d_pk = nullptr, *d_pl = nullptr, *d_pa = nullptr, *d_S = nullptr, *d_vp_ptr = nullptr;
  long long *d_vp_off = nullptr;
  CR(tmp.alloc(&d_pk, (size_t)L.T)); CR(tmp.alloc(&d_pl, (size_t)L.T)); CR(tmp.alloc(&d_pa, (size_t)L.T));
  CR(tmp.alloc(&d_S, (size_t)P)); CR(tmp.alloc(&d_vp_ptr, (size_t)P + 1)); CR(tmp.alloc(&d_vp_off, (size_t)VP + 1));
  CRH(hipMemcpyAsync(d_S, L.S.data(), sizeof(int) * P, hipMemcpyHostToDevice, stream));
  CRH(hipMemcpyAsync(d_vp_ptr, L.vp_ptr.data(), sizeof(int) * (P + 1), hipMemcpyHostToDevice, stream));
  CRH(hipMemcpyAsync(d_vp_off, L.vp_off.data(), sizeof(long long) * (VP + 1), hipMemcpyHostToDevice, stream));
  hipLaunchKernelGGL(dv.hist_lds ? k_idx_fill<false> : k_idx_fill<true>, dim3((unsigned)(dv.idx_waves / IDX_WAVES)), dim3(64 * IDX_WAVES), dv.idx_lds,
                     stream, N, m, (int)P, in.d_pt_ptr, in.d_cam, dv.idx_chunk, dv.d_hist, d_S, d_vp_ptr, d_vp_off, d_pk, d_pl, d_pa,
                     (const int *)nullptr);
  CRH(hipGetLastError());
  timer.lap("items sorted by pair");
  std::vector<long long> lo_tab((size_t)VP * (nR + 1));
  {
    long long *d_rl = nullptr, *d_lo = nullptr;
    CR(tmp.alloc(&d_rl, (size_t)nR + 1)); CR(tmp.alloc(&d_lo, lo_tab.size()));
    CRH(hipMemcpyAsync(d_rl, R.lo.data(), sizeof(long long) * (nR + 1), hipMemcpyHostToDevice, stream));
    const long long nt = (long long)lo_tab.size();
    hipLaunchKernelGGL(k_idx_bounds, dim3((unsigned)((nt + 255) / 256)), dim3(256), 0, stream, VP, nR, d_vp_off, d_rl, d_pa, d_lo, (const int *)nullptr);
    CRH(hipMemcpyAsync(lo_tab.data(), d_lo, sizeof(long long) * nt, hipMemcpyDeviceToHost, stream));
    CRH(hipStreamSynchronize(stream));
    tmp.release(d_rl); tmp.release(d_lo);
  }
  std::vector<int> uid;
  number_units(in, plan, [&](int v, int r) { return lo_tab[(size_t)v * (nR + 1) + r]; }, ix, uid);
  timer.lap("units");
  if (plan.mode == SCHUR_SLOTS) {
    SlotWaves sw = make_slot_waves(in, plan, uid, ix);
    const long long n_waves = sw.n_waves;
    const int nSeg = sw.nSeg;
    CR(upload_range_o0(in, R, engine, ix));
    long long *d_slbeg = nullptr, *d_wbeg = nullptr;
    int *d_sllen = nullptr, *d_wsteps = nullptr;
    CR(tmp.alloc(&d_slbeg, sw.sl_beg.size())); CR(tmp.alloc(&d_sllen, sw.sl_len.size()));
    CR(tmp.alloc(&d_wsteps, (size_t)n_waves)); CR(tmp.alloc(&d_wbeg, (size_t)n_waves + 1));
    CRH(hipMemcpyAsync(d_slbeg, sw.sl_beg.data(), sizeof(long long) * sw.sl_beg.size(), hipMemcpyHostToDevice, stream));
    CRH(hipMemcpyAsync(d_sllen, sw.sl_len.data(), sizeof(int) * sw.sl_len.size(), hipMemcpyHostToDevice, stream));
    hipLaunchKernelGGL(k_idx_merge<false>, dim3((unsigned)n_waves), dim3(64), 0, stream, n_waves, nR, nSeg, SLOT_SKEW, SLOT_SEG, d_slbeg, d_sllen,
                       ix.d_range_o0, d_pk, d_pl, d_pa, d_wbeg, 0, (int)N, d_wsteps, (int *)nullptr, (int *)nullptr, (int *)nullptr,
                       (int *)nullptr, (const long long *)in.d_pt_ptr);
    std::vector<int> ws32(n_waves);
    CRH(hipMemcpyAsync(ws32.data(), d_wsteps, sizeof(int) * n_waves, hipMemcpyDeviceToHost, stream));
    CRH(hipStreamSynchronize(stream));
    for (long long b = 0; b < n_waves; ++b) sw.w_steps[b] = ws32[b];
    timer.lap("slot merge (count)");
    long long total_steps = 0;
    CR(place_slot_steps(plan, sw, ix, total_steps));
    const size_t rows = (size_t)total_steps * PSTEP;
    CR(engine.alloc(&ix.d_it_k, rows)); CR(engine.alloc(&ix.d_it_l, rows)); CR(engine.alloc(&ix.d_it_a, rows));
    CR(engine.alloc(&ix.d_seg_end, ix.seg_end.size()));
    CRH(hipMemcpyAsync(d_wbeg, sw.w_beg.data(), sizeof(long long) * (n_waves + 1), hipMemcpyHostToDevice, stream));
    hipLaunchKernelGGL(k_idx_merge<true>, dim3((unsigned)n_waves), dim3(64), 0, stream, n_waves, nR, nSeg, SLOT_SKEW, SLOT_SEG, d_slbeg, d_sllen,
                       ix.d_range_o0, d_pk, d_pl, d_pa, d_wbeg, 0, (int)N, d_wsteps, ix.d_it_k, ix.d_it_l, ix.d_it_a, ix.d_seg_end, (const long long *)in.d_pt_ptr);
    CRH(hipGetLastError());
    CRH(hipStreamSynchronize(stream));
    timer.lap("slot merge (fill)");
    finish_slot_waves(R, sw, total_steps, ix);
  } else {
    build_work_queues(in, plan, uid, ix);
    engine.adopt(tmp, d_pk); engine.adopt(tmp, d_pl); engine.adopt(tmp, d_pa);
    ix.d_it_k = d_pk; ix.d_it_l = d_pl; ix.d_it_a = d_pa;
  }
  tmp.release_all();
  ix.on_device = true;
  return MVBA_OK;
}

int alloc_engine_buffers(mvba_handle *h, K1Tiles &t) {
  const long long N = h->N, nobs = h->nobs;
  const int m = h->m;
  h->cost_grid = (int)std::max<long long>(1, std::min<long long>(2048, (nobs + 255) / 256));
  h->n_partials = std::max(h->cost_grid, 4096);
  CR(h->mem.alloc(&h->d_obs_pt, nobs));
  CR(h->mem.alloc(&h->d_xy, nobs));
  h->n_tiles = (int)t.tiles.size() - 1;
  h->any_split = t.any_split;
  if (t.any_split) {
    t.tile_slot.resize(t.tiles.size(), -1);
    h->n_splits = (int)t.splits.size();
    CR(h->mem.alloc(&h->d_tile_slot, t.tile_slot.size()));
    CR(h->mem.alloc(&h->d_splits, t.splits.size()));
    CR(h->mem.alloc(&h->d_PLsplit, 9 * (size_t)t.n_split_slots));
    CRH(hipMemcpy(h->d_tile_slot, t.tile_slot.data(), sizeof(int) * t.tile_slot.size(), hipMemcpyHostToDevice));
    CRH(hipMemcpy(h->d_splits, t.splits.data(), sizeof(int4) * t.splits.size(), hipMemcpyHostToDevice));
  }
  CR(h->mem.alloc(&h->d_tiles, t.tiles.size()));
  for (int i = 0; i < 2; ++i) { CR(h->mem.alloc(&h->d_X[i], 3 * N)); CR(h->mem.alloc(&h->d_cam15[i], (size_t)CAM_IN * m)); }
  CR(h->mem.alloc(&h->d_rec, (size_t)REC * (nobs + 1)));
  if (h->loss != LOSS_SQUARED) {
    CR(h->mem.alloc(&h->d_sqw, nobs + 1));
    CRH(hipMemset(h->d_sqw, 0, sizeof(double) * (nobs + 1)));
  }
  CR(h->mem.alloc(&h->d_PL, 9 * N));
  CR(h->mem.alloc(&h->d_PB, (size_t)PBS * (N + 1)));
  CRH(hipMemset(h->d_rec + (size_t)REC * nobs, 0, sizeof(double2) * REC));
  CRH(hipMemset(h->d_PB + (size_t)PBS * N, 0, sizeof(double) * PBS));
  const size_t n9 = 9 * (size_t)m;
  CR(h->mem.alloc(&h->d_Ab, strip_offset(m, m) + n9));
  CR(h->mem.alloc(&h->d_Ared, (size_t)(h->D + 1) * h->ld));
  CR(h->mem.alloc(&h->d_Lblk, (size_t)((h->D + SBW - 1) / SBW) * SBW * SBW));
  CR(h->mem.alloc(&h->d_Ztiles, (size_t)((h->D + NB - 1) / NB) * NB * NB));
  CR(h->mem.alloc(&h->d_dxi, n9));
  CR(h->mem.alloc(&h->d_dX, 3 * N));
  CR(h->mem.alloc(&h->d_partials, h->n_partials));
  CR(h->mem.alloc(&h->d_cost, 2));
  CR(h->mem.alloc(&h->d_flag, 1));
  CR(h->mem.alloc(&h->d_bar, 1 + 4 * (size_t)((9 * m + SBW - 1) / SBW)));
  CRH(hipHostMalloc((void **)&h->h_cost, 4 * sizeof(double), hipHostMallocMapped));
  memset(h->h_cost, 0, 4 * sizeof(double));
  if (hipHostGetDevicePointer((void **)&h->d_mail, h->h_cost, 0) != hipSuccess) h->d_mail = nullptr;
  h->h_flag = reinterpret_cast<int *>(h->h_cost + 1);
  return MVBA_OK;
}

int upload_schur_index(mvba_handle *h, const SchurPlan &plan, SchurIndex &ix) {
  const int m = h->m;
  h->n_items = plan.L.T;
  h->n_items_offdiag = plan.L.T - plan.L.Tdiag;
  h->n_units = (int)ix.units.size();
  h->n_waves = ix.n_waves; h->slot_nR = ix.slot_nR; h->slot_nseg = ix.slot_nseg; h->n_slot_items = ix.n_slot_items;
  h->index_on_device = ix.on_device;
  h->d_range_o0 = ix.d_range_o0;
  if (ix.on_device) { h->d_it_k = ix.d_it_k; h->d_it_l = ix.d_it_l; h->d_it_a = ix.d_it_a; h->d_seg_end = ix.d_seg_end; }
  const size_t P1 = (size_t)m * (m + 1) / 2 + 1;
  if (!ix.on_device) { CR(h->mem.alloc(&h->d_it_k, ix.it_k.size())); CR(h->mem.alloc(&h->d_it_l, ix.it_l.size())); CR(h->mem.alloc(&h->d_it_a, ix.it_a.size())); }
  CR(h->mem.alloc(&h->d_units, ix.units.size())); CR(h->mem.alloc(&h->d_unit_ptr, P1));
  CR(h->mem.alloc(&h->d_q_ptr, 9)); CR(h->mem.alloc(&h->d_q_units, ix.q_units.size()));
  CR(h->mem.alloc(&h->d_wdesc, ix.wdesc.size())); CR(h->mem.alloc(&h->d_wunits, ix.wunits.size()));
  if (!ix.on_device) CR(h->mem.alloc(&h->d_seg_end, ix.seg_end.size()));
  CR(h->mem.alloc(&h->d_prog, (size_t)h->slot_nR * std::max(1, h->slot_nseg) * PACE_STRIDE));
  if (!ix.seg_end.empty() && !ix.on_device) CRH(hipMemcpy(h->d_seg_end, ix.seg_end.data(), sizeof(int) * ix.seg_end.size(), hipMemcpyHostToDevice));
  if (!ix.wdesc.empty()) {
    CRH(hipMemcpy(h->d_wdesc, ix.wdesc.data(), sizeof(int4) * ix.wdesc.size(), hipMemcpyHostToDevice));
    CRH(hipMemcpy(h->d_wunits, ix.wunits.data(), sizeof(int) * ix.wunits.size(), hipMemcpyHostToDevice));
  }
  CR(h->mem.alloc(&h->d_partial, (size_t)UNIT_STRIDE * ix.units.size()));
  if (!ix.it_k.empty()) {
    CRH(hipMemcpy(h->d_it_k, ix.it_k.data(), sizeof(int) * ix.it_k.size(), hipMemcpyHostToDevice));
    CRH(hipMemcpy(h->d_it_l, ix.it_l.data(), sizeof(int) * ix.it_l.size(), hipMemcpyHostToDevice));
    CRH(hipMemcpy(h->d_it_a, ix.it_a.data(), sizeof(int) * ix.it_a.size(), hipMemcpyHostToDevice));
  }
  if (!ix.it_k.empty() || ix.on_device) {
    if (h->schur_mode == SCHUR_PAIRS) {
      std::vector<int4> qdesc(ix.units.size());
      for (size_t i = 0; i < ix.q_units.size(); ++i) qdesc[i] = ix.units[ix.q_units[i]];
      CRH(hipMemcpy(h->d_units, qdesc.data(), sizeof(int4) * qdesc.size(), hipMemcpyHostToDevice));
      int mx = 0;
      for (int x = 0; x < 8; ++x) mx = std::max(mx, ix.q_ptr[x + 1] - ix.q_ptr[x]);
      h->q_max = mx;
    }
    if (!ix.q_units.empty()) CRH(hipMemcpy(h->d_q_units, ix.q_units.data(), sizeof(int) * ix.q_units.size(), hipMemcpyHostToDevice));
  }
  if (h->schur_mode == SCHUR_SLOTS && h->n_slot_items) {
    const long long n_steps = h->n_slot_items / PSTEP;
    CR(h->mem.alloc(&h->d_it_x, (size_t)n_steps * SLOT_IDX));
    hipLaunchKernelGGL(k_idx_interleave, dim3((unsigned)((n_steps * SLOT_IDX + 255) / 256)), dim3(256), 0, h->stream, n_steps, h->d_it_k, h->d_it_l,
                       h->d_it_a, h->d_it_x);
    CRH(hipGetLastError());
    CRH(hipStreamSynchronize(h->stream));
    h->mem.release(h->d_it_k); h->mem.release(h->d_it_l); h->mem.release(h->d_it_a);
  }
  CRH(hipMemcpy(h->d_unit_ptr, ix.unit_ptr.data(), sizeof(int) * P1, hipMemcpyHostToDevice));
  CRH(hipMemcpy(h->d_q_ptr, ix.q_ptr.data(), sizeof(int) * 9, hipMemcpyHostToDevice));
  CRH(hipMemset(h->d_partial, 0, sizeof(double) * UNIT_STRIDE * std::max<size_t>(ix.units.size(), 1)));
  return MVBA_OK;
}

int upload_engine(mvba_handle *h, const mvba_problem *p, const std::vector<int> &obs_pt, const K1Tiles &t, const SchurPlan &plan, SchurIndex &ix) {
  const long long N = h->N, nobs = h->nobs;
  const int m = h->m;
  if (nobs) {
    CRH(hipMemcpy(h->d_obs_pt, obs_pt.data(), sizeof(int) * nobs, hipMemcpyHostToDevice));
    if (p->xy_layout == 1) {
      DevBufs tmp;
      double2 *planes = nullptr;
      CRH(hipMalloc((void **)&planes, sizeof(double2) * nobs));
      tmp.own(planes);
      hipError_t e = hipMemcpy(planes, p->xy, sizeof(double2) * nobs, hipMemcpyHostToDevice);
      if (e == hipSuccess) {
        hipLaunchKernelGGL(k_xy_from_planes, dim3((unsigned)((N + 255) / 256), m), dim3(256), 0, 0, planes, N, m, h->d_xy);
        e = hipGetLastError();
        if (e == hipSuccess) e = hipDeviceSynchronize();
      }
      CRH(e);
    } else {
      CRH(hipMemcpy(h->d_xy, p->xy, sizeof(double2) * nobs, hipMemcpyHostToDevice));
    }
  }
  CRH(hipMemcpy(h->d_tiles, t.tiles.data(), sizeof(int) * t.tiles.size(), hipMemcpyHostToDevice));
  CRH(hipMemset(h->d_PL, 0, sizeof(double) * 9 * std::max<long long>(N, 1)));
  CRH(hipMemset(h->d_flag, 0, sizeof(int)));
  if (h->schur_mode == SCHUR_DENSE) {
    const int T = (9 * m + 15) / 16;
    int n_cu_dense = 256;
    hipDeviceGetAttribute(&n_cu_dense, hipDeviceAttributeMultiprocessorCount, h->device);
    h->dense_tiles = T * (T + 1) / 2 + m;
    h->dense_blocks = (int)std::max<long long>(1, std::min<long long>((N + dense_ch(T) - 1) / dense_ch(T), (long long)n_cu_dense * dense_wgs(T)));
    CR(h->mem.alloc(&h->d_dense_part, (size_t)h->dense_blocks * h->dense_tiles * 256));
    if (!plan.dense_obs.empty()) {
      CR(h->mem.alloc(&h->d_dense_obs, plan.dense_obs.size()));
      CRH(hipMemcpy(h->d_dense_obs, plan.dense_obs.data(), sizeof(int) * plan.dense_obs.size(), hipMemcpyHostToDevice));
    }
  }
  if (h->use_pairs) CR(upload_schur_index(h, plan, ix));
  return MVBA_OK;
}

int set_kernel_attributes(mvba_handle *h, const CreateKnobs &knobs) {
  const int m = h->m;
  const bool robust = h->loss != LOSS_SQUARED;
  auto set_lds = [](const void *f, size_t bytes) { return hipFuncSetAttribute(f, hipFuncAttributeMaxDynamicSharedMemorySize, (int)bytes); };
  const size_t cam_lds = cam_lds_bytes(m, h->gcam, true);
  if (h->gcam) { CR(h->mem.alloc(&h->d_cam18, (size_t)m * CAM_LDS)); CR(h->mem.alloc(&h->d_dxi10, (size_t)m * DXI_LDS)); }
  for (int G : {2, 4, 8})
    for (int bt : {256, 512, 1024}) {
      CRH(set_lds(backsub_kernel(G, bt, false).fn(false), cam_lds));
      if (robust) CRH(set_lds(backsub_kernel(G, bt, false).fn(true), cam_lds));
    }
  CRH(set_lds((const void *)k_chol_super, SUPER_LDS));
  CRH(set_lds((const void *)k_chol_backsolve_all<true>, BACKSOLVE_LDS));
  {
    int per_cu = 0;
    CRH(hipDeviceGetAttribute(&h->n_cu, hipDeviceAttributeMultiprocessorCount, h->device));
    CRH(hipOccupancyMaxActiveBlocksPerMultiprocessor(&per_cu, (const void *)k_chol_backsolve_all<true>, SUPER_THREADS, BACKSOLVE_LDS));
    h->chol_onepass = per_cu >= 1 && !knobs.chol_launches;
    h->trail64_min = knobs.trail64_min;
    h->barrier_polls = knobs.barrier_polls;
  }
  const size_t k1_lds = k1_lds_bytes(m, h->gcam, h->k1_threads);
  CRH(set_lds(resid_jac_kernel(h->gcam, h->loss).fn(false), k1_lds));
  CRH(set_lds(cost_kernel(false, h->loss).fn(false), cam_lds));
  CRH(set_lds((const void *)k_residuals<false>, cam_lds));
  if (robust) {
    CRH(set_lds(resid_jac_kernel(h->gcam, h->loss).fn(true), k1_lds));
    CRH(set_lds(cost_kernel(false, h->loss).fn(true), cam_lds));
  }
  if (h->schur_mode == SCHUR_DENSE) {
    const int T = (9 * m + 15) / 16;
    CRH(set_lds(dense_kernel(T, h->d_dense_obs != nullptr).fn(robust), dense_lds_bytes(T, 16 * T / 9)));
  }
  return MVBA_OK;
}

int build_engine(mvba_handle *h, const mvba_problem *p, const CreateKnobs &knobs, const std::vector<int> &obs_pt, K1Tiles &tiles, CreateTimer &timer) {
  const long long N = h->N, nobs = h->nobs;
  const int m = h->m;
  if (p->device >= 0) CRH(hipSetDevice(p->device));
  CRH(hipGetDevice(&h->device));
  CRH(hipStreamCreateWithFlags(&h->stream, hipStreamNonBlocking));
  CR(h->mem.alloc(&h->d_pt_ptr, N + 1));
  CR(h->mem.alloc(&h->d_cam, nobs));
  CRH(hipMemcpy(h->d_pt_ptr, p->pt_ptr, sizeof(long long) * (N + 1), hipMemcpyHostToDevice));
  if (nobs) CRH(hipMemcpy(h->d_cam, p->cam_idx, sizeof(int) * nobs, hipMemcpyHostToDevice));
  timer.lap("device, topology upload");
  h->k1_threads = k1_block_threads(m, h->gcam);

  const bool dev_build = N > 0 && nobs > 0 && !knobs.index_host;
  const IndexInput in{p, N, nobs, (long long)m * (m + 1) / 2, m,
                      (int)std::max(1u, std::min({std::thread::hardware_concurrency(), 16u, (unsigned)m})), h->stream, h->d_pt_ptr, h->d_cam};
  DeviceIndexBuild dv;
  SchurPlan plan;
  SchurIndex ix;
  CR(decide_schur_form(in, knobs, h->loss, h->device, [&](std::vector<long long> &cnt) {
    return dev_build ? count_pairs_device(in, knobs, dv, cnt) : count_pairs_host(in, cnt);
  }, plan, timer));
  h->schur_mode = plan.mode;
  h->use_pairs = plan.mode != SCHUR_DENSE;
  if (h->use_pairs) CR(dev_build ? build_index_device(in, plan, dv, h->mem, ix, timer) : build_index_host(in, plan, h->mem, ix, timer));
  timer.lap("queues / wave descriptors");

  CR(alloc_engine_buffers(h, tiles));
  timer.lap("allocations");
  CR(upload_engine(h, p, obs_pt, tiles, plan, ix));
  timer.lap("uploads");
  CR(set_kernel_attributes(h, knobs));
  timer.lap("attributes");
  return MVBA_OK;
}

int create_engine(const mvba_problem *p, int loss, double loss_b, mvba_handle **out) {
  if (!p || !out) return fail(MVBA_ERR_BADARG, "null argument");
  const CreateKnobs knobs = read_create_knobs();
  CreateTimer timer{knobs.timing};
  std::vector<int> obs_pt;
  CR(validate_problem(p, obs_pt));
  timer.lap("validate, obs_pt");
  K1Tiles tiles = build_k1_tiles(p);
  timer.lap("K1 tiles");

  mvba_handle *h = new mvba_handle();
  const int m = p->n_images;
  h->N = p->n_points; h->nobs = p->n_obs; h->m = m; h->gauge_axis = p->gauge_axis; h->f0 = p->f0; h->D = 9 * m - 7; h->ld = (h->D + 3) & ~3;
  h->loss = loss; h->loss_b = loss_b;
  h->gcam = m > LDS_CAMERAS;
  h->force_big = knobs.force_big;
  h->check_solve = knobs.check_solve;
  h->check_solve_tol = knobs.check_solve_tol;
  if (int rc = build_engine(h, p, knobs, obs_pt, tiles, timer)) {
    const std::string err = g_err;
    mvba_destroy(h);
    g_err = err;
    return rc;
  }
  *out = h;
  return MVBA_OK;
}

#undef CR
#undef CRH
```

### 3d-reconstruction-from-multi-view-exp_amd/csrc/mvba_init.h

```cpp

namespace {

__host__ __device__ __forceinline__ void init_camera_matrix(const double *Kk, const double *Rk, const double *tk, double *P) {
  double Rt[3][4];
  for (int i = 0; i < 3; ++i) {
    for (int j = 0; j < 3; ++j) Rt[i][j] = Rk[3 * j + i];
    Rt[i][3] = -(Rt[i][0] * tk[0] + Rt[i][1] * tk[1] + Rt[i][2] * tk[2]);
  }
  for (int i = 0; i < 3; ++i)
    for (int j = 0; j < 4; ++j) P[4 * i + j] = Kk[3 * i] * Rt[0][j] + Kk[3 * i + 1] * Rt[1][j] + Kk[3 * i + 2] * Rt[2][j];
}

struct InitObs {
  const int *cam;
  const double2 *xy;
  long long o0;
  int deg;
  __host__ __device__ __forceinline__ int camera(int i) const { return cam ? cam[o0 + i] : i; }
  static constexpr bool MASKED = false;
  __host__ __device__ __forceinline__ int count() const { return deg; }
};

struct InitObsMasked : InitObs {
  static constexpr bool MASKED = true;
// ... 346 lines not shown
  for (int i = 0; i < 12; ++i)
    for (int j = 0; j < 12; ++j) A[i][j] = 0.0;
  int e = 0;
  for (int a = 0; a < 4; ++a)
    for (int b = a; b < 4; ++b, ++e) {
      const double h = S40[e], xh = S40[10 + e], yh = S40[20 + e], wh = S40[30 + e];
      A[a][b] = A[b][a] = h;
      A[4 + a][4 + b] = A[4 + b][4 + a] = h;
      A[a][8 + b] = -xh; A[b][8 + a] = -xh;
      A[4 + a][8 + b] = -yh; A[4 + b][8 + a] = -yh;
      A[8 + a][8 + b] = A[8 + b][8 + a] = wh;
    }
  for (int i = 0; i < 12; ++i)
    for (int j = 0; j < i; ++j) A[i][j] = A[j][i];
  sym_eig_jacobi<12>(A, V);
  double l1, l2, lmax, p[12];
  eig_extremes<12>(A, V, l1, l2, lmax, p);
  *ratio = l1 / l2;
  if (!(l2 > INIT_REL_PIVOT * lmax)) return 2;
  return resect_denormalise(p, nm, P) ? 0 : 2;
}

}

extern "C" {

int mvba_triangulate(const double *K, const double *R, const double *t, int32_t n_images, int64_t n_points, const int64_t *pt_ptr,
                     const int32_t *cam_idx, const double *xy, int64_t n_obs, int32_t n_refine, double *X, double *quality,
                     int32_t *status, double *timings_ms, int32_t device) {
  if (!K || !R || !t || !xy || !X)
    return fail(MVBA_ERR_BADARG, std::string("null argument: ") + (!K ? "K" : (!R ? "R" : (!t ? "t" : (!xy ? "xy" : "X")))) + " (argument " +
                                     std::to_string(!K ? 1 : (!R ? 2 : (!t ? 3 : (!xy ? 8 : 11)))) + ")");
  if (n_refine < 0) return fail(MVBA_ERR_BADARG, "n_refine = " + std::to_string(n_refine) + " must be >= 0");
  int rc = init_check_list(n_points, n_images, pt_ptr, cam_idx, n_obs);
  if (rc) return rc;
  if ((rc = init_check_cameras(n_images))) return rc;
  if (timings_ms) timings_ms[0] = timings_ms[1] = timings_ms[2] = 0.0;
  if (n_points == 0) return MVBA_OK;
  if (device >= 0) MVBA_HIP(hipSetDevice(device));
  InitClock clk;
  DevBufs tmp;
  double *dK = nullptr, *dR = nullptr, *dt = nullptr, *dX = nullptr, *dq = nullptr;
  double2 *dxy = nullptr;
  long long *dptr = nullptr;
  int *dcam = nullptr, *dst = nullptr;
  if ((rc = tmp.alloc(&dK, 9 * (size_t)n_images)) || (rc = tmp.alloc(&dR, 9 * (size_t)n_images)) || (rc = tmp.alloc(&dt, 3 * (size_t)n_images)) ||
      (rc = tmp.alloc(&dX, 3 * (size_t)n_points)))
    return rc;
  if (quality && (rc = tmp.alloc(&dq, 3 * (size_t)n_points))) return rc;
  if (status && (rc = tmp.alloc(&dst, (size_t)n_points))) return rc;
  MVBA_HIP(hipMemcpy(dK, K, sizeof(double) * 9 * n_images, hipMemcpyHostToDevice));
  MVBA_HIP(hipMemcpy(dR, R, sizeof(double) * 9 * n_images, hipMemcpyHostToDevice));
  MVBA_HIP(hipMemcpy(dt, t, sizeof(double) * 3 * n_images, hipMemcpyHostToDevice));
  if ((rc = upload_list(tmp, n_points, n_obs, pt_ptr, cam_idx, xy, &dptr, &dcam, &dxy))) return rc;
  if (timings_ms) timings_ms[0] = clk.lap();
  double ms = 0.0;
  if ((rc = launch_triangulate(nullptr, n_points, n_images, dK, dR, dt, dptr, dcam, dxy, n_refine, dX, dq, dst, 0, timings_ms ? &ms : nullptr))) return rc;
  if (timings_ms) { timings_ms[1] = ms; clk.lap(); }
  MVBA_HIP(hipMemcpy(X, dX, sizeof(double) * 3 * n_points, hipMemcpyDeviceToHost));
  if (quality) MVBA_HIP(hipMemcpy(quality, dq, sizeof(double) * 3 * n_points, hipMemcpyDeviceToHost));
  if (status) MVBA_HIP(hipMemcpy(status, dst, sizeof(int) * n_points, hipMemcpyDeviceToHost));
  if (timings_ms) timings_ms[2] = clk.lap();
  return MVBA_OK;
}

int mvba_triangulate_state(mvba_handle *h, int32_t n_refine, double *quality, int32_t *status, double *timings_ms) {
  if (!h) return fail(MVBA_ERR_BADARG, "null argument: h (argument 1)");
  if (n_refine < 0) return fail(MVBA_ERR_BADARG, "n_refine = " + std::to_string(n_refine) + " must be >= 0");
  if (!h->have_params) return fail(MVBA_ERR_STATE, "no parameters set: the cameras to triangulate from are the committed ones");
  int rc = init_check_cameras(h->m);
  if (rc) return rc;
  if (timings_ms) timings_ms[0] = timings_ms[1] = timings_ms[2] = 0.0;
  MVBA_HIP(hipSetDevice(h->device));
  if (!h->d_init_cams && (rc = h->mem.alloc(&h->d_init_cams, 21 * (size_t)h->m))) return rc;
  double *dK = h->d_init_cams, *dR = dK + 9 * (size_t)h->m, *dt = dR + 9 * (size_t)h->m;
  DevBufs tmp;
  double *dq = nullptr;
  int *dst = nullptr;
  if (quality && (rc = tmp.alloc(&dq, 3 * (size_t)std::max<long long>(h->N, 1)))) return rc;
  if (status && (rc = tmp.alloc(&dst, (size_t)std::max<long long>(h->N, 1)))) return rc;
  hipLaunchKernelGGL(k_init_cams, dim3((h->m + 255) / 256), dim3(256), 0, h->stream, h->m, h->d_cam15[h->cur], dK, dR, dt);
  MVBA_HIP(hipGetLastError());
  h->linearized = false; h->have_trial = false;
  if (h->N == 0) return sync_and_drain(h);
  double ms = 0.0;
  if ((rc = launch_triangulate(h->stream, h->N, h->m, dK, dR, dt, h->d_pt_ptr, h->d_cam, h->d_xy, n_refine, h->d_X[h->cur], dq, dst, 1,
                               timings_ms ? &ms : nullptr)))
    return rc;
  drain_events(h);
  InitClock clk;
  if (quality) MVBA_HIP(hipMemcpy(quality, dq, sizeof(double) * 3 * h->N, hipMemcpyDeviceToHost));
  if (status) MVBA_HIP(hipMemcpy(status, dst, sizeof(int) * h->N, hipMemcpyDeviceToHost));
  if (timings_ms) { timings_ms[1] = ms; timings_ms[2] = clk.lap(); }
  return MVBA_OK;
}

int mvba_resect(const double *X, int64_t n_points, const int64_t *pt_ptr, const int32_t *cam_idx, const double *xy, int64_t n_obs,
                int32_t n_images, const uint8_t *point_ok, double *P, double *quality, int32_t *status, double *timings_ms,
                int32_t device) {
  if (!X || !xy || !P)
    return fail(MVBA_ERR_BADARG, std::string("null argument: ") + (!X ? "X" : (!xy ? "xy" : "P")) + " (argument " + std::to_string(!X ? 1 : (!xy ? 5 : 9)) + ")");
  int rc = init_check_list(n_points, n_images, pt_ptr, cam_idx, n_obs);
  if (rc) return rc;
  if (timings_ms) timings_ms[0] = timings_ms[1] = timings_ms[2] = 0.0;
  const int m = n_images;
  InitClock clk;
  ResectList list;
  resect_build_list(X, n_points, pt_ptr, cam_idx, xy, m, point_ok, false, list);
  const std::vector<long long> &cam_ptr = list.cam_ptr;
  const std::vector<int> &cm_pt = list.cm_pt;
  const std::vector<double> &cm_xy = list.cm_xy;
  const long long n_used = cam_ptr[m];
  std::vector<int> cam_ch_ptr((size_t)m + 1, 0), ch_cam, ch_cnt;
  std::vector<long long> ch_start;
  for (int k = 0; k < m; ++k) {
    for (long long s = cam_ptr[k]; s < cam_ptr[k + 1]; s += START_CHUNK) {
      ch_cam.push_back(k);
      ch_start.push_back(s);
      ch_cnt.push_back((int)std::min<long long>(START_CHUNK, cam_ptr[k + 1] - s));
    }
    cam_ch_ptr[k + 1] = (int)ch_cam.size();
  }
  const int n_ch = (int)ch_cam.size();
  std::vector<double> Pm(12 * (size_t)m, NAN), norm(RS_NORM * (size_t)m, 0.0), S40(40 * (size_t)m, 0.0), Sr((size_t)m, 0.0), ratio((size_t)m, NAN);
  std::vector<int> st((size_t)m, 1);
  double kernel_ms = 0.0;
  if (n_ch > 0) {
    if (device >= 0) MVBA_HIP(hipSetDevice(device));
    DevBufs tmp;
    double *dX = nullptr, *dpart = nullptr, *dS = nullptr, *dnorm = nullptr, *dP = nullptr;
    double2 *dxy = nullptr;
    int *dpt = nullptr, *dch_cam = nullptr, *dch_cnt = nullptr, *dcam_ch = nullptr;
    long long *dch_start = nullptr;
    if ((rc = tmp.alloc(&dX, 3 * (size_t)n_points)) || (rc = tmp.alloc(&dxy, (size_t)n_used)) || (rc = tmp.alloc(&dpt, (size_t)n_used)) ||
        (rc = tmp.alloc(&dch_cam, (size_t)n_ch)) || (rc = tmp.alloc(&dch_cnt, (size_t)n_ch)) || (rc = tmp.alloc(&dch_start, (size_t)n_ch)) ||
        (rc = tmp.alloc(&dcam_ch, (size_t)m + 1)) || (rc = tmp.alloc(&dpart, 40 * (size_t)n_ch)) || (rc = tmp.alloc(&dS, 40 * (size_t)m)) ||
        (rc = tmp.alloc(&dnorm, RS_NORM * (size_t)m)) || (rc = tmp.alloc(&dP, 12 * (size_t)m)))
      return rc;
    MVBA_HIP(hipMemcpy(dX, X, sizeof(double) * 3 * n_points, hipMemcpyHostToDevice));
    MVBA_HIP(hipMemcpy(dxy, cm_xy.data(), sizeof(double2) * n_used, hipMemcpyHostToDevice));
    MVBA_HIP(hipMemcpy(dpt, cm_pt.data(), sizeof(int) * n_used, hipMemcpyHostToDevice));
    MVBA_HIP(hipMemcpy(dch_cam, ch_cam.data(), sizeof(int) * n_ch, hipMemcpyHostToDevice));
    MVBA_HIP(hipMemcpy(dch_cnt, ch_cnt.data(), sizeof(int) * n_ch, hipMemcpyHostToDevice));
    MVBA_HIP(hipMemcpy(dch_start, ch_start.data(), sizeof(long long) * n_ch, hipMemcpyHostToDevice));
    MVBA_HIP(hipMemcpy(dcam_ch, cam_ch_ptr.data(), sizeof(int) * (m + 1), hipMemcpyHostToDevice));
    if (timings_ms) timings_ms[0] = clk.lap();
    hipEvent_t ev[4] = {nullptr, nullptr, nullptr, nullptr};
    EvGuard guard{ev, 4};
    for (auto &e : ev) MVBA_HIP(hipEventCreate(&e));
    const dim3 gm((m + 255) / 256), b256(256);
    auto combine = [&](int nv) { hipLaunchKernelGGL(k_resect_combine, dim3((m * nv + 255) / 256), b256, 0, 0, m, nv, dcam_ch, dpart, dS); };
    hipEventRecord(ev[0], 0);
    hipLaunchKernelGGL(k_resect_chunk<0>, dim3(n_ch), dim3(START_CHUNK), 0, 0, dch_cam, dch_start, dch_cnt, dpt, dxy, dX, (const double *)nullptr, dpart);
    combine(6);
    hipLaunchKernelGGL(k_resect_norm, gm, b256, 0, 0, m, 0, dS, dnorm);
    hipLaunchKernelGGL(k_resect_chunk<1>, dim3(n_ch), dim3(START_CHUNK), 0, 0, dch_cam, dch_start, dch_cnt, dpt, dxy, dX, dnorm, dpart);
    combine(2);
    hipLaunchKernelGGL(k_resect_norm, gm, b256, 0, 0, m, 1, dS, dnorm);
    hipLaunchKernelGGL(k_resect_chunk<2>, dim3(n_ch), dim3(START_CHUNK), 0, 0, dch_cam, dch_start, dch_cnt, dpt, dxy, dX, dnorm, dpart);
    combine(40);
    hipEventRecord(ev[1], 0);
    MVBA_HIP(hipGetLastError());
    MVBA_HIP(hipMemcpy(S40.data(), dS, sizeof(double) * 40 * m, hipMemcpyDeviceToHost));
    MVBA_HIP(hipMemcpy(norm.data(), dnorm, sizeof(double) * RS_NORM * m, hipMemcpyDeviceToHost));
    for (int k = 0; k < m; ++k) {
      if (cam_ptr[k + 1] - cam_ptr[k] < 6) continue;
// ... 33 lines not shown
```

### 3d-reconstruction-from-multi-view-exp_amd/lib/_mvba.py

```python
from __future__ import annotations

import ctypes as C
import os
import threading

import numpy as np

_HERE = os.path.dirname(os.path.abspath(__file__))
LIB_PATH = os.environ.get("MVBA_LIBRARY", os.path.join(os.path.dirname(_HERE), "libmvba.so"))

MVBA_OK, MVBA_ERR_BADARG, MVBA_ERR_SINGULAR, MVBA_ERR_HIP, MVBA_ERR_RCCL, MVBA_ERR_STATE = range(6)

KERNEL_IDS = ("resid_jac", "point_blocks", "point_inv", "schur", "allreduce", "solve", "backsub_cost", "cost")
BUF = {"residual": 0, "JX": 1, "JC": 2, "E": 3, "dP": 4, "A_full": 5, "b_full": 6, "dxi": 7, "dX": 8,
       "trial_X": 9, "trial_cam": 10, "index_k": 11, "index_l": 12, "index_a": 13, "index_seg": 14, "weight": 15}
LOSSES = {"squared": 0, "huber": 1, "cauchy": 2}


def check_loss(loss, loss_scale):
    if not isinstance(loss, str) or loss not in LOSSES:
        raise ValueError(f"loss must be one of {sorted(LOSSES)}, got {loss!r}")
    if loss == "squared":
        return 0, 0.0
    if loss_scale is None:
        raise ValueError(f"loss={loss!r} needs loss_scale (delta in image units)")
    try:
        scale = float(loss_scale)
    except (TypeError, ValueError):
        raise ValueError(f"loss_scale must be a number, got {loss_scale!r}") from None
    if not np.isfinite(scale) or scale <= 0.0:
        raise ValueError(f"loss_scale must be finite and > 0, got {loss_scale!r}")
    return LOSSES[loss], scale

_dp = C.POINTER(C.c_double)


class Problem(C.Structure):
    _fields_ = [("n_points", C.c_int64), ("n_obs", C.c_int64), ("n_images", C.c_int32),
                ("gauge_axis", C.c_int32), ("pt_ptr", C.POINTER(C.c_int64)),
                ("cam_idx", C.POINTER(C.c_int32)), ("xy", _dp), ("f0", C.c_double),
                ("device", C.c_int32), ("xy_layout", C.c_int32)]


class Stats(C.Structure):
    _fields_ = [("ms", C.c_double * 16), ("launches", C.c_int64 * 16),
                ("n_linearize", C.c_int64), ("n_try_step", C.c_int64), ("n_commit", C.c_int64),
                ("n_lu_fallback", C.c_int64), ("n_barrier_fallback", C.c_int64)]


SIGNATURES = {
    "mvba_version": (C.c_char_p, []),
    "mvba_last_error": (C.c_char_p, []),
    "mvba_kernel_name": (C.c_char_p, [C.c_int32]),
    "mvba_device_count": (C.c_int, [C.POINTER(C.c_int32)]),
    "mvba_create": (C.c_int, [C.POINTER(Problem), C.POINTER(C.c_void_p)]),
    "mvba_create_robust": (C.c_int, [C.POINTER(Problem), C.c_int32, C.c_double, C.POINTER(C.c_void_p)]),
    "mvba_destroy": (None, [C.c_void_p]),
    "mvba_set_params": (C.c_int, [C.c_void_p, _dp, _dp, _dp, _dp, _dp]),
    "mvba_get_params": (C.c_int, [C.c_void_p, _dp, _dp, _dp, _dp, _dp]),
    "mvba_apply_similarity": (C.c_int, [C.c_void_p, _dp, _dp, C.c_double]),
    "mvba_snapshot": (C.c_int, [C.c_void_p]),
    "mvba_snapshot_count": (C.c_int, [C.c_void_p, C.POINTER(C.c_int64)]),
    "mvba_snapshot_read": (C.c_int, [C.c_void_p, C.c_int64, _dp, _dp, _dp, _dp, _dp]),
    "mvba_snapshot_clear": (C.c_int, [C.c_void_p]),
    "mvba_snapshot_restore": (C.c_int, [C.c_void_p, C.c_int64]),
    "mvba_cost": (C.c_int, [C.c_void_p, _dp]),
    "mvba_linearize": (C.c_int, [C.c_void_p]),
    "mvba_try_step": (C.c_int, [C.c_void_p, C.c_double, _dp]),
    "mvba_commit": (C.c_int, [C.c_void_p]),
    "mvba_set_parameter_map": (C.c_int, [C.c_void_p, C.POINTER(C.c_int32), C.c_int32]),
    "mvba_covariance": (C.c_int, [C.c_void_p, _dp, _dp, _dp, _dp]),
    "mvba_residuals": (C.c_int, [C.c_void_p, _dp]),
    "mvba_set_profiling": (C.c_int, [C.c_void_p, C.c_int32]),
    "mvba_get_stats": (C.c_int, [C.c_void_p, C.POINTER(Stats)]),
    "mvba_reset_stats": (C.c_int, [C.c_void_p]),
    "mvba_get_info": (C.c_int, [C.c_void_p, C.POINTER(C.c_int64)]),
    "mvba_comm_unique_id": (C.c_int, [C.c_void_p]),
    "mvba_comm_init": (C.c_int, [C.c_void_p, C.c_void_p, C.c_int32, C.c_int32]),
    "mvba_comm_init_host": (C.c_int, [C.c_void_p, C.c_int32, C.c_int32, C.c_void_p, C.c_void_p]),
    "mvba_debug_read": (C.c_int, [C.c_void_p, C.c_int32, _dp, C.c_int64, C.POINTER(C.c_int64)]),
    "mvba_host_obs_math": (C.c_int, [_dp, _dp, _dp, C.c_double, _dp]),
    "mvba_triangulate": (C.c_int, [_dp, _dp, _dp, C.c_int32, C.c_int64, C.POINTER(C.c_int64), C.POINTER(C.c_int32), _dp, C.c_int64,
                                   C.c_int32, _dp, _dp, C.POINTER(C.c_int32), _dp, C.c_int32]),
    "mvba_triangulate_state": (C.c_int, [C.c_void_p, C.c_int32, _dp, C.POINTER(C.c_int32), _dp]),
    "mvba_resect": (C.c_int, [_dp, C.c_int64, C.POINTER(C.c_int64), C.POINTER(C.c_int32), _dp, C.c_int64, C.c_int32,
                              C.POINTER(C.c_uint8), _dp, _dp, C.POINTER(C.c_int32), _dp, C.c_int32]),
    "mvba_covisibility": (C.c_int, [C.c_int64, C.c_int32, C.POINTER(C.c_int64), C.POINTER(C.c_int32), C.c_int64, C.POINTER(C.c_int64),
                                    _dp, C.c_int32]),
    "mvba_two_view": (C.c_int, [C.c_int64, C.c_int32, C.POINTER(C.c_int64), C.POINTER(C.c_int32), _dp, C.c_int64, C.POINTER(C.c_int32),
                                C.c_int32, _dp, _dp, C.POINTER(C.c_int64), C.POINTER(C.c_int32), _dp, C.c_int32]),
    "mvba_two_view_robust": (C.c_int, [C.c_int64, C.c_int32, C.POINTER(C.c_int64), C.POINTER(C.c_int32), _dp, C.c_int64, C.POINTER(C.c_int32),
                                       C.c_int32, C.c_double, C.c_int32, C.c_uint64, C.c_int32, _dp, _dp, C.POINTER(C.c_int64),
                                       C.POINTER(C.c_int64), C.POINTER(C.c_int32), C.POINTER(C.c_uint8), C.POINTER(C.c_int32),
                                       C.POINTER(C.c_int32), _dp, C.c_int32]),
    "mvba_ransac_sample": (C.c_int, [C.c_uint64, C.c_int32, C.c_int32, C.c_int32, C.c_int64, C.POINTER(C.c_int64)]),
    "mvba_resect_robust": (C.c_int, [_dp, C.c_int64, C.POINTER(C.c_int64), C.POINTER(C.c_int32), _dp, C.c_int64, C.c_int32,
                                     C.POINTER(C.c_uint8), C.POINTER(C.c_int32), C.c_int32, C.c_double, C.c_int32, C.c_uint64, C.c_int32,
                                     _dp, _dp, C.POINTER(C.c_int64), C.POINTER(C.c_int64), C.POINTER(C.c_int32), C.POINTER(C.c_uint8),
                                     C.POINTER(C.c_int32), C.POINTER(C.c_int32), _dp, C.c_int32]),
    "mvba_resect_sample": (C.c_int, [C.c_uint64, C.c_int32, C.c_int32, C.c_int64, C.POINTER(C.c_int64)]),
    "mvba_triangulate_robust": (C.c_int, [_dp, _dp, _dp, C.c_int32, C.c_int64, C.POINTER(C.c_int64), C.POINTER(C.c_int32), _dp, C.c_int64,
                                          C.c_double, C.c_int32, C.c_uint64, C.c_int32, C.c_int32, _dp, _dp, C.POINTER(C.c_int32),
                                          C.POINTER(C.c_int32), C.POINTER(C.c_int32), C.POINTER(C.c_uint8), C.POINTER(C.c_int32), _dp,
                                          C.c_int32]),
    "mvba_triangulate_sample": (C.c_int, [C.c_uint64, C.c_int32, C.c_int32, C.c_int64, C.c_int32, C.POINTER(C.c_int64)]),
    "mvba_project": (C.c_int, [_dp, C.c_int64, _dp, _dp, _dp, C.c_int32, C.POINTER(C.c_int64), C.POINTER(C.c_int32),
                               C.c_int64, _dp, C.c_int32]),
    "mvsvd_factorize": (C.c_int, [C.c_void_p, C.c_int64, C.c_int32, C.c_int32, C.c_int32, C.c_int32,
                                  C.c_void_p, C.c_void_p, C.c_void_p, C.c_void_p, _dp, C.c_int32]),
    "mvsvd_create": (C.c_int, [C.c_int64, C.c_int32, C.c_int32, C.c_int32, C.POINTER(C.c_void_p)]),
    "mvsvd_load": (C.c_int, [C.c_void_p, C.c_void_p, C.c_int64]),
    "mvsvd_run": (C.c_int, [C.c_void_p, C.c_int32, C.c_int32, C.c_void_p, C.c_void_p, C.c_void_p, C.c_void_p, _dp]),
    "mvsvd_load_images": (C.c_int, [C.c_void_p, C.POINTER(C.c_void_p), C.c_int32, C.c_int64, C.c_int32]),
    "mvsvd_load_base": (C.c_int, [C.c_void_p, C.c_void_p, C.c_int64]),
    "mvsvd_load_base_images": (C.c_int, [C.c_void_p, C.POINTER(C.c_void_p), C.c_int32, C.c_int64, C.c_double]),
    "mvsvd_run_scaled": (C.c_int, [C.c_void_p, C.c_void_p, C.c_int32, C.c_int32, C.c_int32, C.c_void_p, C.c_void_p, C.c_void_p, _dp]),
    "mvsvd_depth_begin": (C.c_int, [C.c_void_p, C.c_int32]),
    "mvsvd_depth_step": (C.c_int, [C.c_void_p, C.c_int32, C.c_double, _dp, _dp]),
    "mvsvd_depth_read": (C.c_int, [C.c_void_p, C.c_void_p]),
    "mvsvd_destroy": (None, [C.c_void_p]),
}

_lib = None


def load_library():
    global _lib
    if _lib is None:
        if not os.path.exists(LIB_PATH):
            raise RuntimeError(
                f"libmvba.so not found at {LIB_PATH}: build it with `python -c 'import __graft_entry__ as g; "
                f"g.build()'` (or make -C 3d-reconstruction-from-multi-view-exp_amd/csrc). There is no CPU fallback.")
        lib = C.CDLL(LIB_PATH)
        for name, (res, args) in SIGNATURES.items():
            fn = getattr(lib, name)
            fn.restype, fn.argtypes = res, args
        _lib = lib
    return _lib


def _as(a, dtype):
    return np.ascontiguousarray(a, dtype=dtype)


def _ptr(a):
    return a.ctypes.data_as(_dp)


def raise_for(rc, lib=None):
    if rc == MVBA_OK:
# ... 46 lines not shown
        from .bundle_adjustment import AXES

        if axis not in AXES:
            raise ValueError()
        loss_code, scale = check_loss(loss, loss_scale)
        self.loss, self.loss_scale = loss, (scale if loss_code else None)
        self.lib = load_library()
        if device_count() < 1:
            raise RuntimeError("libmvba: no HIP device visible; the BA engine has no CPU fallback")
        self.n, self.m = int(n_points), int(n_images)
        self._pt_ptr = _as(pt_ptr, np.int64)
        self._cam = _as(cam_idx, np.int32)
        self._xy = _as(xy, np.float64)
        planes = self._xy.ndim == 3
        if planes and self._xy.shape != (self.m, self.n, 2):
            raise ValueError("xy as image planes must be (n_images, n_points, 2)")
        if not planes:
            self._xy = self._xy.reshape(-1, 2)
        self.n_obs = int(self._cam.shape[0])
        prob = Problem(self.n, self.n_obs, self.m, AXES[axis],
                       self._pt_ptr.ctypes.data_as(C.POINTER(C.c_int64)),
                       self._cam.ctypes.data_as(C.POINTER(C.c_int32)), _ptr(self._xy), float(f0), int(device), int(planes))
        h = C.c_void_p()
        if loss_code or loss_scale is not None:
            raise_for(self.lib.mvba_create_robust(C.byref(prob), loss_code, scale, C.byref(h)), self.lib)
        else:
            raise_for(self.lib.mvba_create(C.byref(prob), C.byref(h)), self.lib)
        self._h = h
        self.n_solves = 0
        self.n_free = 9 * self.m - 7

    def close(self):
        if getattr(self, "_h", None):
            self.lib.mvba_destroy(self._h)
            self._h = None

    __del__ = close

    def set_params(self, X, f, u, t, R):
        X, f, u, t, R = (_as(v, np.float64) for v in (X, f, u, t, R))
        assert X.shape == (self.n, 3) and f.shape == (self.m,) and u.shape == (self.m, 2)
        assert t.shape == (self.m, 3) and R.shape == (self.m, 3, 3)
        raise_for(self.lib.mvba_set_params(self._h, _ptr(X), _ptr(f), _ptr(u), _ptr(t), _ptr(R)), self.lib)

    def get_params(self):
        X = np.empty((self.n, 3)); f = np.empty(self.m); u = np.empty((self.m, 2))
        t = np.empty((self.m, 3)); R = np.empty((self.m, 3, 3))
        raise_for(self.lib.mvba_get_params(self._h, _ptr(X), _ptr(f), _ptr(u), _ptr(t), _ptr(R)), self.lib)
        return X, f, u, t, R

    def snapshot(self):
        raise_for(self.lib.mvba_snapshot(self._h), self.lib)

    def snapshot_count(self):
        n = C.c_int64()
        raise_for(self.lib.mvba_snapshot_count(self._h, C.byref(n)), self.lib)
        return n.value

    def snapshot_read(self, i):
        X = np.empty((self.n, 3)); f = np.empty(self.m); u = np.empty((self.m, 2))
        t = np.empty((self.m, 3)); R = np.empty((self.m, 3, 3))
        raise_for(self.lib.mvba_snapshot_read(self._h, int(i), _ptr(X), _ptr(f), _ptr(u), _ptr(t), _ptr(R)), self.lib)
        return X, f, u, t, R

    def snapshot_clear(self):
        raise_for(self.lib.mvba_snapshot_clear(self._h), self.lib)

    def snapshot_restore(self, i):
        raise_for(self.lib.mvba_snapshot_restore(self._h, int(i)), self.lib)

    def apply_similarity(self, R0, t0, scale):
        R0, t0 = _as(R0, np.float64), _as(t0, np.float64)
        assert R0.shape == (3, 3) and t0.shape == (3,)
        raise_for(self.lib.mvba_apply_similarity(self._h, _ptr(R0), _ptr(t0), float(scale)), self.lib)

    def cost(self):
        E = C.c_double()
        raise_for(self.lib.mvba_cost(self._h, C.byref(E)), self.lib)
        return E.value

    def linearize(self):
        raise_for(self.lib.mvba_linearize(self._h), self.lib)

    def try_step(self, c):
        E = C.c_double()
        raise_for(self.lib.mvba_try_step(self._h, float(c), C.byref(E)), self.lib)
        self.n_solves += 1
        return E.value

    def commit(self):
        raise_for(self.lib.mvba_commit(self._h), self.lib)

    def set_parameter_map(self, col, n_free=None):
        if col is None:
            raise_for(self.lib.mvba_set_parameter_map(self._h, None, 0), self.lib)
            self.n_free = 9 * self.m - 7
            return
        col = _as(col, np.int32).reshape(-1)
        if col.shape != (9 * self.m,):
            raise ValueError(f"col must have 9 n_images = {9 * self.m} entries, got {col.shape[0]}")
        if n_free is None:
            n_free = int(col.max()) + 1 if col.size else 0
        raise_for(self.lib.mvba_set_parameter_map(self._h, col.ctypes.data_as(C.POINTER(C.c_int32)), int(n_free)), self.lib)
        self.n_free = int(n_free)

    def covariance(self, points=True, cameras=True, full=False):
        P = np.empty((self.n, 6)) if points else None
        Cc = np.empty((self.m, 9, 9)) if cameras else None
        Cf = np.empty((9 * self.m, 9 * self.m)) if full else None
        tm = np.zeros(4)
        raise_for(self.lib.mvba_covariance(self._h, _ptr(P) if P is not None else None, _ptr(Cc) if Cc is not None else None,
                                           _ptr(Cf) if Cf is not None else None, _ptr(tm)), self.lib)
        out = {"timings_ms": dict(zip(("schur", "factor", "inverse", "points"), tm.tolist()))}
        if P is not None:
            i = np.array([[0, 1, 2], [1, 3, 4], [2, 4, 5]])
            out["points"] = P[:, i]
        if Cc is not None:
            out["cameras"] = Cc
        if Cf is not None:
            out["cameras_full"] = Cf
        return out

    def triangulate(self, n_refine=2):
        q = np.empty((self.n, 3))
        st = np.empty(self.n, np.int32)
        tm = np.zeros(3)
        raise_for(self.lib.mvba_triangulate_state(self._h, int(n_refine), _ptr(q), st.ctypes.data_as(C.POINTER(C.c_int32)), _ptr(tm)),
                  self.lib)
        return q, st, _timings3(tm)

    def residuals(self):
        e = np.empty((self.n_obs, 2))
        raise_for(self.lib.mvba_residuals(self._h, _ptr(e)), self.lib)
        return e

    def set_profiling(self, on):
        raise_for(self.lib.mvba_set_profiling(self._h, 2 if on == 2 and on is not True else int(bool(on))), self.lib)

    def reset_stats(self):
        raise_for(self.lib.mvba_reset_stats(self._h), self.lib)

    def stats(self):
        s = Stats()
        raise_for(self.lib.mvba_get_stats(self._h, C.byref(s)), self.lib)
        out = {k: {"ms": s.ms[i], "launches": s.launches[i]} for i, k in enumerate(KERNEL_IDS)}
        out["counts"] = {"linearize": s.n_linearize, "try_step": s.n_try_step, "commit": s.n_commit,
                         "lu_fallback": s.n_lu_fallback, "barrier_fallback": s.n_barrier_fallback}
        return out

    def _info(self):
        out = (C.c_int64 * 8)()
        raise_for(self.lib.mvba_get_info(self._h, out), self.lib)
        return list(out)

    def schur_info(self):
        i = self._info()
        return {"items": i[0], "offdiag_items": i[1], "units": i[2], "kernel": ("strip", "pairs", "slots", "dense")[i[3] & 0xff],
                "slot_rows": i[7]}

    def rccl_version(self):
        i = self._info()
        return {"loaded": i[4], "compiled_against": i[5], "ranks": i[6]}

    def comm_init(self, id128: bytes, rank: int, n_ranks: int):
        buf = C.create_string_buffer(bytes(id128), 128)
        raise_for(self.lib.mvba_comm_init(self._h, buf, int(rank), int(n_ranks)), self.lib)
# ... 389 lines not shown
```

### 3d-reconstruction-from-multi-view-exp_amd/lib/bundle_adjustment.py

```python
from __future__ import annotations

import os
from typing import Any

import numpy as np
import numpy.typing as npt

from ._mvba import check_loss

AXES = {"x-right_z-forward": 0, "x-up_z-forward": 1}


def dense_to_observations(x: npt.NDArray, visibility_index: npt.NDArray | None):
    n, m = x.shape[:2]
    if visibility_index is None:
        x = np.asarray(x, dtype=np.float64)
        planes = x.transpose(1, 0, 2)
        if not x.flags.c_contiguous and planes.flags.c_contiguous:
            xy = planes
        else:
            xy = np.ascontiguousarray(x.reshape(n * m, 2))
        cam_idx = np.empty((n, m), dtype=np.int32)
        cam_idx[:] = np.arange(m, dtype=np.int32)
        return np.arange(0, (n + 1) * m, m, dtype=np.int64), cam_idx.reshape(-1), xy
# ... 68 lines not shown
def gauge_slots(axis: str):
    if axis not in AXES:
        raise ValueError(f"axis must be one of {sorted(AXES)}, got {axis!r}")
    return np.array([3, 4, 5, 6, 7, 8, 12 + AXES[axis]])


def _slot_names(arg, table, what):
    names = [arg] if isinstance(arg, str) else list(arg)
    slots: set[int] = set()
    for nm in names:
        if not isinstance(nm, str) or nm not in table:
            raise ValueError(f"{what}: unknown name {nm!r} (known: {sorted(table)})")
        slots.update(table[nm])
    return slots


def parameter_map(n_images: int, axis: str = "x-right_z-forward", hold=None, share=None, share_groups=None):
    m = int(n_images)
    gauge = gauge_slots(axis)
    held = np.zeros((m, 9), dtype=bool)
    held_by_name: set[int] = set()
    if hold is not None:
        if isinstance(hold, str) or (len(hold) and all(isinstance(v, str) for v in hold)):
            held_by_name = _slot_names(hold, HOLD_NAMES, "hold")
            held[:, sorted(held_by_name)] = True
        else:
            mask = np.asarray(hold)
            if mask.dtype != np.bool_ or mask.shape != (m, 9):
                raise ValueError(f"hold: names or a bool array of shape ({m}, 9), got {mask.dtype} {mask.shape}")
            held |= mask
    shared = _slot_names(share, SHARE_NAMES, "share") if share is not None else set()
    both = sorted(shared & held_by_name)
    if both:
        raise ValueError(f"slot {SLOT_LABELS[both[0]]!r} is both held and shared")
    if share_groups is None:
        labels = np.zeros(m, dtype=np.int64)
    else:
        labels = np.asarray(share_groups)
        if labels.shape != (m,) or labels.dtype.kind not in "iu":
            raise ValueError(f"share_groups: an int array of shape ({m},)")
    held_flat = held.reshape(-1).copy()
    held_flat[gauge[gauge < 9 * m]] = True
    col = np.full(9 * m, -1, dtype=np.int32)
    tied_sets = []
    tied_mask = np.zeros(9 * m, dtype=bool)
    for lab in np.unique(labels) if shared else ():
        cams = np.nonzero(labels == lab)[0]
        for p in sorted(shared):
            h = held[cams, p]
            if h.all():
                continue
            if h.any():
                raise ValueError(f"group {int(lab)}: slot {SLOT_LABELS[p]!r} is held for some of its cameras and shared by the others")
            if len(cams) > 1:
                tied_sets.append((lab, p, 9 * cams + p))
                tied_mask[9 * cams + p] = True
    free = np.nonzero(~held_flat & ~tied_mask)[0]
    col[free] = np.arange(len(free), dtype=np.int32)
    for i, (_, _, slots) in enumerate(tied_sets):
        col[slots] = len(free) + i
    return col, len(free) + len(tied_sets)


def intrinsics_from(f, u, f0: float):
    m = len(f)
    K = np.zeros((m, 3, 3))
    K[:, 0, 0] = K[:, 1, 1] = f
    K[:, 0, 2], K[:, 1, 2] = u[:, 0], u[:, 1]
    K[:, 2, 2] = f0
    return K



class LevenbergMarquardt:

    def __init__(self, engine, scale_factor):
        self.engine, self.scale_factor = engine, scale_factor
        self.E = engine.cost()
        self.c = 0.0001
        self.count = 0

    def iterate(self):
        g = self.engine
        g.linearize()
        while True:
            E_ = g.try_step(self.c)
            if E_ > self.E:
                self.c *= self.scale_factor
            else:
                break
        g.commit()
        self.count += 1
        delta = np.abs(E_ - self.E)
        return E_, delta

    def carry_on(self, E_):
        self.E = E_
        self.c /= self.scale_factor


def lm_loop(engine, scale_factor, delta_tol, max_iter, on_state=None, verbose=True):
    lm = LevenbergMarquardt(engine, scale_factor)
    if on_state is not None:
        on_state(lm.E)
    while True:
        E_, reprojection_error_delta = lm.iterate()
        if on_state is not None:
            on_state(E_)
        if verbose:
            print(f"Iteration {lm.count}: reprojection_error_delta = {reprojection_error_delta}")
        if reprojection_error_delta <= delta_tol or lm.count >= max_iter:
            break
        lm.carry_on(E_)
    return E_


def loss_weights(e_px, f0, loss, loss_scale):
    code, scale = check_loss(loss, loss_scale)
    e = np.asarray(e_px, np.float64).reshape(-1, 2) / f0
    s = (e * e).sum(axis=1)
    if code == 0:
        return np.ones_like(s)
    b = (scale / f0) ** 2
    if code == 1:
        return np.where(s <= b, 1.0, np.sqrt(b / np.maximum(s, b)))
    return 1.0 / (1.0 + s / b)


class BundleAdjuster:
    def __init__(
        self,
        x: npt.NDArray,
        init_X: npt.NDArray | None,
        init_K: npt.NDArray,
        init_R: npt.NDArray,
        init_t: npt.NDArray,
        f0: float = 1.0,
        visibility_index: npt.NDArray | None = None,
        axis: str = "x-right_z-forward",
        loss: str = "squared",
        loss_scale: float | None = None,
        hold=None,
        share=None,
        share_groups=None,
    ):
        check_loss(loss, loss_scale)
        x = np.asarray(x)
        self._check_map(x.shape[1], axis, init_K, hold, share, share_groups)
        pt_ptr, cam_idx, xy = dense_to_observations(x, visibility_index)
        self._setup(x.shape[0], x.shape[1], pt_ptr, cam_idx, xy, init_X, init_K, init_R, init_t, f0, axis, loss=loss,
                    loss_scale=loss_scale)

    @classmethod
    def from_observations(cls, n_points, n_images, pt_ptr, cam_idx, xy, init_X, init_K, init_R, init_t,
                          f0: float = 1.0, axis: str = "x-right_z-forward", loss: str = "squared",
                          loss_scale: float | None = None, hold=None, share=None, share_groups=None, **engine_kw):
        check_loss(loss, loss_scale)
        self = cls.__new__(cls)
        self._check_map(n_images, axis, init_K, hold, share, share_groups)
        self._setup(n_points, n_images, pt_ptr, cam_idx, xy, init_X, init_K, init_R, init_t, f0, axis, loss=loss,
                    loss_scale=loss_scale, **engine_kw)
        return self

    _map = None

    def _check_map(self, n_images, axis, init_K, hold, share, share_groups):
        if hold is None and share is None:
# ... 151 lines not shown
```

### include/mvba.h

```cpp
#ifndef MVBA_H
#define MVBA_H

#include <stdint.h>

#ifdef __cplusplus
extern "C" {
#endif

#define MVBA_OK 0
#define MVBA_ERR_BADARG 1
#define MVBA_ERR_SINGULAR 2
#define MVBA_ERR_HIP 3
#define MVBA_ERR_RCCL 4
#define MVBA_ERR_STATE 5

typedef struct mvba_handle mvba_handle;

typedef struct mvba_problem {
  int64_t n_points;
  int64_t n_obs;
  int32_t n_images;
  int32_t gauge_axis;
  const int64_t *pt_ptr;
  const int32_t *cam_idx;
  const double *xy;
  double f0;
  int32_t device;
  int32_t xy_layout;
} mvba_problem;

enum {
  MVBA_K_RESID_JAC = 0,
  MVBA_K_POINT_BLOCKS,
  MVBA_K_POINT_INV,
  MVBA_K_SCHUR,
  MVBA_K_ALLREDUCE,
  MVBA_K_SOLVE,
  MVBA_K_BACKSUB_COST,
  MVBA_K_COST,
  MVBA_K_COUNT
};

typedef struct mvba_stats {
  double ms[16];
  int64_t launches[16];
  int64_t n_linearize, n_try_step, n_commit;
  int64_t n_lu_fallback;
  int64_t n_barrier_fallback;
} mvba_stats;

const char *mvba_version(void);
const char *mvba_last_error(void);
const char *mvba_kernel_name(int32_t kernel_id);
int mvba_device_count(int32_t *count);

int mvba_create(const mvba_problem *problem, mvba_handle **out);
#define MVBA_LOSS_SQUARED 0
#define MVBA_LOSS_HUBER 1
#define MVBA_LOSS_CAUCHY 2
int mvba_create_robust(const mvba_problem *problem, int32_t loss, double scale, mvba_handle **out);
void mvba_destroy(mvba_handle *h);

int mvba_set_params(mvba_handle *h, const double *X, const double *f, const double *u,
                    const double *t, const double *R);
int mvba_get_params(mvba_handle *h, double *X, double *f, double *u, double *t, double *R);

int mvba_apply_similarity(mvba_handle *h, const double *R0, const double *t0, double scale);

int mvba_cost(mvba_handle *h, double *E);
int mvba_linearize(mvba_handle *h);
int mvba_try_step(mvba_handle *h, double c, double *E_trial);
int mvba_commit(mvba_handle *h);

int mvba_set_parameter_map(mvba_handle *h, const int32_t *col, int32_t n_free);

int mvba_covariance(mvba_handle *h, double *point_cov, double *cam_cov, double *cam_cov_full, double *timings_ms);

int mvba_residuals(mvba_handle *h, double *e);

int mvba_snapshot(mvba_handle *h);
int mvba_snapshot_count(mvba_handle *h, int64_t *n);
int mvba_snapshot_read(mvba_handle *h, int64_t i, double *X, double *f, double *u, double *t, double *R);
int mvba_snapshot_clear(mvba_handle *h);
int mvba_snapshot_restore(mvba_handle *h, int64_t i);

int mvba_set_profiling(mvba_handle *h, int32_t enabled);
int mvba_get_stats(mvba_handle *h, mvba_stats *out);
int mvba_reset_stats(mvba_handle *h);

int mvba_get_info(mvba_handle *h, int64_t *out8);

int mvba_comm_unique_id(void *id128);
int mvba_comm_init(mvba_handle *h, const void *id128, int32_t rank, int32_t n_ranks);

typedef int (*mvba_host_allreduce_fn)(void *user, double *buf, int64_t n);
int mvba_comm_init_host(mvba_handle *h, int32_t rank, int32_t n_ranks, mvba_host_allreduce_fn fn, void *user);

enum {
  MVBA_BUF_RESIDUAL = 0,
  MVBA_BUF_JX,
  MVBA_BUF_JC,
  MVBA_BUF_E,
  MVBA_BUF_DP,
  MVBA_BUF_A_FULL,
  MVBA_BUF_B_FULL,
  MVBA_BUF_DXI,
  MVBA_BUF_DX,
  MVBA_BUF_TRIAL_X,
  MVBA_BUF_TRIAL_CAM,
  MVBA_BUF_INDEX_K,
  MVBA_BUF_INDEX_L,
  MVBA_BUF_INDEX_A,
  MVBA_BUF_INDEX_SEG,
  MVBA_BUF_WEIGHT
};
int mvba_debug_read(mvba_handle *h, int32_t which, double *out, int64_t capacity, int64_t *n);

int mvba_project(const double *X, int64_t n_points, const double *K, const double *R, const double *t, int32_t n_images,
                 const int64_t *pt_ptr, const int32_t *cam_idx, int64_t n_obs, double *xy, int32_t device);

int mvba_triangulate(const double *K, const double *R, const double *t, int32_t n_images, int64_t n_points, const int64_t *pt_ptr,
                     const int32_t *cam_idx, const double *xy, int64_t n_obs, int32_t n_refine, double *X, double *quality,
                     int32_t *status, double *timings_ms, int32_t device);
int mvba_triangulate_state(mvba_handle *h, int32_t n_refine, double *quality, int32_t *status, double *timings_ms);
int mvba_resect(const double *X, int64_t n_points, const int64_t *pt_ptr, const int32_t *cam_idx, const double *xy, int64_t n_obs,
                int32_t n_images, const uint8_t *point_ok, double *P, double *quality, int32_t *status, double *timings_ms,
                int32_t device);

int mvba_covisibility(int64_t n_points, int32_t n_images, const int64_t *pt_ptr, const int32_t *cam_idx, int64_t n_obs,
                      int64_t *count, double *timings_ms, int32_t device);

int mvba_two_view(int64_t n_points, int32_t n_images, const int64_t *pt_ptr, const int32_t *cam_idx, const double *xy,
                  int64_t n_obs, const int32_t *pairs, int32_t n_pairs, double *F, double *quality, int64_t *n_shared,
                  int32_t *status, double *timings_ms, int32_t device);

int mvba_two_view_robust(int64_t n_points, int32_t n_images, const int64_t *pt_ptr, const int32_t *cam_idx, const double *xy,
                         int64_t n_obs, const int32_t *pairs, int32_t n_pairs, double threshold, int32_t n_hypotheses,
                         uint64_t seed, int32_t n_refit, double *F, double *quality, int64_t *n_shared, int64_t *n_inliers,
                         int32_t *best, uint8_t *inlier, int32_t *hyp_count, int32_t *status, double *timings_ms, int32_t device);
int mvba_ransac_sample(uint64_t seed, int32_t k, int32_t l, int32_t h, int64_t n, int64_t *idx8);

int mvba_resect_robust(const double *X, int64_t n_points, const int64_t *pt_ptr, const int32_t *cam_idx, const double *xy,
                       int64_t n_obs, int32_t n_images, const uint8_t *point_ok, const int32_t *cameras, int32_t n_cameras,
                       double threshold, int32_t n_hypotheses, uint64_t seed, int32_t n_refit, double *P, double *quality,
                       int64_t *n_usable, int64_t *n_inliers, int32_t *best, uint8_t *inlier, int32_t *hyp_count, int32_t *status,
                       double *timings_ms, int32_t device);
int mvba_resect_sample(uint64_t seed, int32_t k, int32_t h, int64_t n, int64_t *idx6);

int mvba_triangulate_robust(const double *K, const double *R, const double *t, int32_t n_images, int64_t n_points, const int64_t *pt_ptr,
                            const int32_t *cam_idx, const double *xy, int64_t n_obs, double threshold, int32_t n_hypotheses,
                            uint64_t seed, int32_t n_refine, int32_t n_refit, double *X, double *quality, int32_t *status,
                            int32_t *n_inliers, int32_t *best, uint8_t *inlier, int32_t *hyp_count, double *timings_ms, int32_t device);
int mvba_triangulate_sample(uint64_t seed, int32_t point, int32_t h, int64_t deg, int32_t n_hypotheses, int64_t *idx2);
// ... 30 lines not shown
```

Measured before the change: 431.5.

## Fuse damped point-block inversion and Ab/progress zeroing into residual-Jacobian kernel

Adds a DAMP template variant of k_resid_jac that zeroes the Ab and progress buffers and, after the per-point segment reduction, inverts each point's damped 3x3 block in-wave and writes PB directly. Split points get a small follow-up kernel. try_step skips the standalone k_point_inv launch when the damping factor matches the one used at linearize. This removes a kernel launch and a full re-read of PL per iteration, at the cost of extra registers, wave syncs and scattered PB writes in the main kernel.

```diff
diff --git a/3d-reconstruction-from-multi-view-exp_amd/csrc/mvba.hip b/3d-reconstruction-from-multi-view-exp_amd/csrc/mvba.hip
--- a/3d-reconstruction-from-multi-view-exp_amd/csrc/mvba.hip
+++ b/3d-reconstruction-from-multi-view-exp_amd/csrc/mvba.hip
@@ -119,16 +119,26 @@
 constexpr int REC = 8;
 constexpr int LDS_CAMERAS = 646;
 
+struct DampArgs {
+  double c;
+  double *PB;
+  int *flag;
+  double *Ab;
+  long long nAb;
+  int *prog;
+  long long nprog;
+  int want_r;
+};
 #define MVBA_RESID_JAC_ARGS                                                                                                 \
   long long nobs, int m, const double *__restrict__ cam15, const double *__restrict__ X, const int *__restrict__ obs_pt,   \
       const int *__restrict__ cam_idx, const double2 *__restrict__ xy, double f0, const int *__restrict__ tile_start,     \
       int n_tiles, double2 *__restrict__ rec, double *__restrict__ PL, const int *__restrict__ tile_slot,                 \
-      double *__restrict__ PLsplit, const double *__restrict__ gcam
+      double *__restrict__ PLsplit, const double *__restrict__ gcam, DampArgs damp
 struct LossArgs {
   double b;
   double *sqw;
 };
-template <bool GCAM, int LOSS = LOSS_SQUARED, typename... Robust>
+template <bool GCAM, int LOSS = LOSS_SQUARED, bool DAMP = false, typename... Robust>
 __global__ __launch_bounds__(1024, 4) void k_resid_jac(MVBA_RESID_JAC_ARGS, Robust... robust) {
   extern __shared__ __attribute__((aligned(16))) double smem[];
   double *s_cam = smem;
@@ -137,6 +147,11 @@
   constexpr int CS = 65;
   double *contrib = reinterpret_cast<double *>(stage);
   int *seg_start = reinterpret_cast<int *>(contrib + 9 * CS), *seg_pt = seg_start + 66;
+  if constexpr (DAMP) {
+    const long long t0 = (long long)blockIdx.x * blockDim.x + threadIdx.x, nt = (long long)gridDim.x * blockDim.x;
+    for (long long i = t0; i < damp.nAb; i += nt) damp.Ab[i] = 0.0;
+    for (long long i = t0; i < damp.nprog; i += nt) damp.prog[i] = 0;
+  }
   if (!GCAM) {
     load_cams_to_lds(cam15, m, f0, s_cam);
     __syncthreads();
@@ -217,15 +232,46 @@
     const int sl = lane / 9, comp = lane - 9 * sl;
     for (int s0 = 0; s0 < nseg; s0 += 7) {
       const int sg = s0 + sl;
-      if (sl < 7 && sg < nseg) {
+      const bool on = sl < 7 && sg < nseg;
+      double acc = 0.0;
+      if (on) {
         const int i0 = seg_start[sg], i1 = seg_start[sg + 1];
-        double acc = 0.0;
         for (int i = i0; i < i1; ++i) acc += contrib[comp * CS + i];
         if (split) PLsplit[9 * (size_t)slot + comp] = acc;
         else PL[9 * (size_t)seg_pt[sg] + comp] = acc;
       }
+      if constexpr (DAMP) {
+        wave_sync();
+        if (on) contrib[comp * CS + sg] = acc;
+      }
     }
     wave_sync();
+    if constexpr (DAMP) {
+      if (!split && nseg > 0) {
+        const int p = min(lane, nseg - 1);
+        double in[9];
+#pragma unroll
+        for (int q = 0; q < 9; ++q) in[q] = contrib[q * CS + p];
+        const int my_pt = seg_pt[p];
+        wave_sync();
+        if (lane < nseg) {
+          double2 o[8];
+          point_inverse(in, damp.c, damp.want_r, damp.flag, o);
+          double2 *row = stage + lane * REC;
+          const int sw = lane & 7;
+#pragma unroll
+          for (int q = 0; q < 8; ++q) row[q ^ sw] = o[q];
+        }
+        wave_sync();
+        double2 *pb = reinterpret_cast<double2 *>(damp.PB);
+        for (int p0 = 0; p0 < nseg; p0 += 8) {
+          const int pp = p0 + (lane >> 3), sl8 = lane & 7;
+          const int pt = __shfl(my_pt, min(pp, nseg - 1), 64);
+          if (pp < nseg) pb[(size_t)pt * 8 + sl8] = stage[pp * REC + (sl8 ^ (pp & 7))];
+        }
+        wave_sync();
+      }
+    }
   }
 }
 
@@ -265,34 +311,12 @@
   for (int i = 0; i < 9; ++i) in[i] = s_in[9 * min((int)threadIdx.x, np - 1) + i];
   __syncthreads();
   if (threadIdx.x < np) {
-    const double s = 1.0 + c;
-    const double xx = in[0] * s, xy = in[1], xz = in[2], yy = in[3] * s, yz = in[4], zz = in[5] * s;
-    const double c00 = yy * zz - yz * yz, c01 = xz * yz - xy * zz, c02 = xy * yz - xz * yy;
-    const double det = xx * c00 + xy * c01 + xz * c02;
-    if (!(det != 0.0) || !isfinite(det)) atomicOr(flag, 1);
-    const double id = 1.0 / det;
-    const double i00 = c00 * id, i01 = c01 * id, i02 = c02 * id;
-    const double i11 = (xx * zz - xz * xz) * id, i12 = (xy * xz - xx * yz) * id, i22 = (xx * yy - xy * xy) * id;
-    const double g0 = in[6], g1 = in[7], g2 = in[8];
+    double2 o[8];
+    point_inverse(in, c, want_r, flag, o);
     double2 *out = s_out + 8 * threadIdx.x;
     const int sw = threadIdx.x & 7;
-    out[0 ^ sw] = make_double2(i00, i01);
-    out[1 ^ sw] = make_double2(i02, i11);
-    out[2 ^ sw] = make_double2(i12, i22);
-    out[3 ^ sw] = make_double2(i00 * g0 + i01 * g1 + i02 * g2, i01 * g0 + i11 * g1 + i12 * g2);
-    out[4 ^ sw] = make_double2(i02 * g0 + i12 * g1 + i22 * g2, 1.0);
-    if (want_r) {
-      const double d0 = i00, q0 = d0 != 0.0 ? 1.0 / d0 : 0.0, l10 = i01 * q0, l20 = i02 * q0;
-      const double d1 = i11 - l10 * i01, q1 = d1 != 0.0 ? 1.0 / d1 : 0.0, l21 = (i12 - l20 * i01) * q1;
-      const double d2 = i22 - l20 * i02 - l21 * l21 * d1;
-      const double a0 = sqrt(fabs(d0)), a1 = sqrt(fabs(d1)), a2 = sqrt(fabs(d2));
-      out[4 ^ sw].y = 1.0 + (d0 < 0.0 ? 1.0 : 0.0) + (d1 < 0.0 ? 2.0 : 0.0) + (d2 < 0.0 ? 4.0 : 0.0);
-      out[5 ^ sw] = make_double2(a0, l10 * a0);
-      out[6 ^ sw] = make_double2(l20 * a0, a1);
-      out[7 ^ sw] = make_double2(l21 * a1, a2);
-    } else {
-      out[5 ^ sw] = out[6 ^ sw] = out[7 ^ sw] = make_double2(0.0, 0.0);
-    }
+#pragma unroll
+    for (int q = 0; q < 8; ++q) out[q ^ sw] = o[q];
   }
   __syncthreads();
   double2 *dst = reinterpret_cast<double2 *>(PB + PBS * a0);
@@ -300,6 +324,21 @@
     const int p = e >> 3, sl = e & 7;
     dst[e] = s_out[8 * p + (sl ^ (p & 7))];
   }
+}
+
+__global__ void k_point_inv_split(int n_split, const int4 *__restrict__ splits, double c, const double *__restrict__ PL,
+                                  double *__restrict__ PB, int *__restrict__ flag, int want_r) {
+  const int sp = blockIdx.x * blockDim.x + threadIdx.x;
+  if (sp >= n_split) return;
+  const size_t a = (size_t)splits[sp].x;
+  double in[9];
+#pragma unroll
+  for (int i = 0; i < 9; ++i) in[i] = PL[9 * a + i];
+  double2 o[8];
+  point_inverse(in, c, want_r, flag, o);
+  double2 *dst = reinterpret_cast<double2 *>(PB + PBS * a);
+#pragma unroll
+  for (int q = 0; q < 8; ++q) dst[q] = o[q];
 }
 
 
@@ -2411,6 +2450,9 @@
   double *d_X[2] = {nullptr, nullptr}, *d_cam15[2] = {nullptr, nullptr};
   int cur = 0;
   bool have_params = false, linearized = false, have_trial = false;
+  bool damped = false, can_damp = true;
+  double damped_c = 0.0;
+  long long stats_point_inv_launches = 0;
   double2 *d_rec = nullptr;
   double *d_PL = nullptr, *d_PB = nullptr;
   double *d_Ab = nullptr, *d_Ared = nullptr, *d_Ztiles = nullptr, *d_Lblk = nullptr, *d_dxi = nullptr, *d_dX = nullptr, *d_lu = nullptr;
@@ -2592,10 +2634,14 @@
   else hipLaunchKernelGGL(k.squared, grid, block, lds, h->stream, args...);
 }
 
-auto resid_jac_kernel(bool gcam, int loss) {
-  if (loss == LOSS_CAUCHY)
-    return gcam ? loss_kernel(k_resid_jac<true>, k_resid_jac<true, LOSS_CAUCHY, LossArgs>) : loss_kernel(k_resid_jac<false>, k_resid_jac<false, LOSS_CAUCHY, LossArgs>);
-  return gcam ? loss_kernel(k_resid_jac<true>, k_resid_jac<true, LOSS_HUBER, LossArgs>) : loss_kernel(k_resid_jac<false>, k_resid_jac<false, LOSS_HUBER, LossArgs>);
+template <bool GCAM, bool DAMP>
+auto resid_jac_kernel_gd(int loss) {
+  if (loss == LOSS_CAUCHY) return loss_kernel(k_resid_jac<GCAM, LOSS_SQUARED, DAMP>, k_resid_jac<GCAM, LOSS_CAUCHY, DAMP, LossArgs>);
+  return loss_kernel(k_resid_jac<GCAM, LOSS_SQUARED, DAMP>, k_resid_jac<GCAM, LOSS_HUBER, DAMP, LossArgs>);
+}
+auto resid_jac_kernel(bool gcam, int loss, bool damp = false) {
+  if (damp) return gcam ? resid_jac_kernel_gd<true, true>(loss) : resid_jac_kernel_gd<false, true>(loss);
+  return gcam ? resid_jac_kernel_gd<true, false>(loss) : resid_jac_kernel_gd<false, false>(loss);
 }
 auto cost_kernel(bool gcam, int loss) {
   if (loss == LOSS_CAUCHY)
@@ -2657,6 +2703,12 @@
   hipLaunchKernelGGL(k_sum_partials, dim3(1), dim3(1024), 0, h->stream, h->d_partials, h->cost_grid, h->d_cost, h->d_flag, mail, seq);
   MVBA_HIP(hipGetLastError());
   return MVBA_OK;
+}
+
+void drop_damped(mvba_handle *h) {
+  if (!h->damped) return;
+  h->damped = false;
+  hipMemsetAsync(h->d_flag, 0, sizeof(int), h->stream);
 }
 
 struct CreateKnobs {
@@ -2759,6 +2811,7 @@
   MVBA_HIP(hipMemcpyAsync(h->d_cam15[h->cur], cam.data(), sizeof(double) * cam.size(), hipMemcpyHostToDevice, h->stream));
   MVBA_HIP(hipStreamSynchronize(h->stream));
   h->have_params = true; h->linearized = false; h->have_trial = false;
+  drop_damped(h);
   return MVBA_OK;
 }
 
@@ -2798,6 +2851,7 @@
   MVBA_HIP(hipGetLastError());
   MVBA_HIP(hipStreamSynchronize(h->stream));
   h->linearized = false; h->have_trial = false;
+  drop_damped(h);
   return MVBA_OK;
 }
 
@@ -2814,27 +2868,34 @@
 }
 
 namespace {
-void launch_resid_jac(mvba_handle *h) {
+long long packed_Ab_doubles(const mvba_handle *h) { return (long long)(strip_offset(h->m, h->m) + 9 * (size_t)h->m); }
+long long pace_ints(const mvba_handle *h) { return (long long)h->slot_nR * h->slot_nseg * PACE_STRIDE; }
+int want_r(const mvba_handle *h) { return h->schur_mode == SCHUR_DENSE ? 1 : 0; }
+
+void launch_resid_jac(mvba_handle *h, const double *damp_c = nullptr) {
   const int kt = h->k1_threads;
   cam_tables(h, h->d_cam15[h->cur], nullptr);
   const int wpb = kt / 64;
   const int grid = std::max(1, std::min(2048 * 256 / kt, (h->n_tiles + wpb - 1) / wpb));
-  launch_loss(h, resid_jac_kernel(h->gcam, h->loss), dim3(grid), dim3(kt), k1_lds_bytes(h->m, h->gcam, kt), h->nobs, h->m, h->d_cam15[h->cur],
-              h->d_X[h->cur], h->d_obs_pt, h->d_cam, h->d_xy, h->f0, h->d_tiles, h->n_tiles, h->d_rec, h->d_PL,
-              h->d_tile_slot, h->d_PLsplit, h->d_cam18);
-  if (h->n_splits)
+  DampArgs damp{};
+  if (damp_c) damp = DampArgs{*damp_c, h->d_PB, h->d_flag, h->d_Ab, packed_Ab_doubles(h), h->d_prog, pace_ints(h), want_r(h)};
+  launch_loss(h, resid_jac_kernel(h->gcam, h->loss, damp_c != nullptr), dim3(grid), dim3(kt), k1_lds_bytes(h->m, h->gcam, kt), h->nobs, h->m,
+              h->d_cam15[h->cur], h->d_X[h->cur], h->d_obs_pt, h->d_cam, h->d_xy, h->f0, h->d_tiles, h->n_tiles, h->d_rec, h->d_PL,
+              h->d_tile_slot, h->d_PLsplit, h->d_cam18, damp);
+  if (h->n_splits) {
     hipLaunchKernelGGL(k_sum_split, dim3((9 * h->n_splits + 255) / 256), dim3(256), 0, h->stream, h->n_splits, h->d_splits,
                        h->d_PLsplit, h->d_PL);
+    if (damp_c)
+      hipLaunchKernelGGL(k_point_inv_split, dim3((h->n_splits + 255) / 256), dim3(256), 0, h->stream, h->n_splits, h->d_splits, *damp_c,
+                         h->d_PL, h->d_PB, h->d_flag, want_r(h));
+  }
 }
 
 void launch_point_inv(mvba_handle *h, double c) {
-  const int m = h->m;
-  const size_t n9 = 9 * (size_t)m, nA = strip_offset(m, m);
-  const long long nAb = (long long)(nA + n9);
+  const long long nAb = packed_Ab_doubles(h);
   const unsigned grid = (unsigned)std::max<long long>((h->N + 255) / 256, std::min<long long>((nAb + 1023) / 1024, 4096));
   hipLaunchKernelGGL(k_point_inv, dim3(std::max(grid, 1u)), dim3(256), 0, h->stream, h->N, c, h->d_PL, h->d_PB, h->d_flag,
-                     h->d_Ab, nAb, h->d_prog, (long long)h->slot_nR * h->slot_nseg * PACE_STRIDE,
-                     h->schur_mode == SCHUR_DENSE ? 1 : 0);
+                     h->d_Ab, nAb, h->d_prog, pace_ints(h), want_r(h));
 }
 
 void launch_schur(mvba_handle *h, double c) {
@@ -2929,19 +2990,28 @@
 }
 }
 
-int mvba_linearize(mvba_handle *h) {
+namespace {
+int linearize(mvba_handle *h, const double *damp_c) {
   if (!h) return fail(MVBA_ERR_BADARG, "null handle");
   if (!h->have_params) return fail(MVBA_ERR_STATE, "no parameters set");
   MVBA_HIP(hipSetDevice(h->device));
+  drop_damped(h);
+  if (!h->nobs || !h->can_damp) damp_c = nullptr;
   if (h->nobs) {
     Timed t(h, MVBA_K_RESID_JAC);
-    launch_resid_jac(h);
+    launch_resid_jac(h, damp_c);
   }
   MVBA_HIP(hipGetLastError());
   h->linearized = true; h->have_trial = false;
+  if (damp_c) { h->damped = true; h->damped_c = *damp_c; }
   h->stats.n_linearize++;
   return MVBA_OK;
 }
+}
+
+int mvba_linearize(mvba_handle *h) { return linearize(h, nullptr); }
+int mvba_linearize_damped(mvba_handle *h, double c) { return linearize(h, &c); }
+int64_t mvba_point_inv_launches(mvba_handle *h) { return h ? (int64_t)h->stats_point_inv_launches : 0; }
 
 namespace {
 double *solve_x(mvba_handle *h) { return h->mapped ? h->d_map_x : h->d_dxi; }
@@ -3078,9 +3148,13 @@
   if (!h || !E_trial) return fail(MVBA_ERR_BADARG, "null argument");
   if (!h->linearized) return fail(MVBA_ERR_STATE, "try_step before linearize");
   MVBA_HIP(hipSetDevice(h->device));
-  {
+  if (h->damped && c == h->damped_c) {
+    h->damped = false;
+  } else {
+    drop_damped(h);
     Timed t(h, MVBA_K_POINT_INV);
     launch_point_inv(h, c);
+    h->stats_point_inv_launches++;
   }
   if (h->use_pairs || h->schur_mode == SCHUR_DENSE) {
     Timed t(h, MVBA_K_SCHUR);
@@ -3128,6 +3202,7 @@
   if (!h->have_trial) return fail(MVBA_ERR_STATE, "commit without a trial step");
   h->cur = 1 - h->cur;
   h->have_trial = false; h->linearized = false;
+  h->damped = false;
   h->stats.n_commit++;
   return MVBA_OK;
 }
@@ -3137,6 +3212,7 @@
   MVBA_HIP(hipSetDevice(h->device));
   const int m = h->m, n9 = 9 * m;
   auto is_gauge = [&](int g) { return (g >= 3 && g <= 8) || g == 12 + h->gauge_axis; };
+  drop_damped(h);
   if (!col) {
     h->mapped = false;
     h->have_trial = false;
@@ -3282,6 +3358,7 @@
   double *d_b = h->d_Ab + strip_offset(m, m);
   if (!local_rc) {
     MVBA_HIP(hipEventRecord(ev[0], h->stream));
+    drop_damped(h);
     if (h->nobs) launch_resid_jac(h);
     h->linearized = true; h->have_trial = false;
     launch_point_inv(h, 0.0);
@@ -3433,6 +3510,7 @@
   MVBA_HIP(hipMemcpyAsync(h->d_X[h->cur], src, sizeof(double) * 3 * h->N, hipMemcpyDeviceToDevice, h->stream));
   MVBA_HIP(hipMemcpyAsync(h->d_cam15[h->cur], src + 3 * h->N, sizeof(double) * CAM_IN * h->m, hipMemcpyDeviceToDevice, h->stream));
   h->have_params = true; h->linearized = false; h->have_trial = false;
+  drop_damped(h);
   return MVBA_OK;
 }
 
diff --git a/3d-reconstruction-from-multi-view-exp_amd/csrc/mvba_common.h b/3d-reconstruction-from-multi-view-exp_amd/csrc/mvba_common.h
--- a/3d-reconstruction-from-multi-view-exp_amd/csrc/mvba_common.h
+++ b/3d-reconstruction-from-multi-view-exp_amd/csrc/mvba_common.h
@@ -176,6 +176,34 @@
   out18[17] = in15[2] / f0;
 }
 
+__device__ __forceinline__ void point_inverse(const double (&in)[9], double c, int want_r, int *flag, double2 (&out)[8]) {
+  const double s = 1.0 + c;
+  const double xx = in[0] * s, xy = in[1], xz = in[2], yy = in[3] * s, yz = in[4], zz = in[5] * s;
+  const double c00 = yy * zz - yz * yz, c01 = xz * yz - xy * zz, c02 = xy * yz - xz * yy;
+  const double det = xx * c00 + xy * c01 + xz * c02;
+  if (!(det != 0.0) || !isfinite(det)) atomicOr(flag, 1);
+  const double id = 1.0 / det;
+  const double i00 = c00 * id, i01 = c01 * id, i02 = c02 * id;
+  const double i11 = (xx * zz - xz * xz) * id, i12 = (xy * xz - xx * yz) * id, i22 = (xx * yy - xy * xy) * id;
+  const double g0 = in[6], g1 = in[7], g2 = in[8];
+  out[0] = make_double2(i00, i01);
+  out[1] = make_double2(i02, i11);
+  out[2] = make_double2(i12, i22);
+  out[3] = make_double2(i00 * g0 + i01 * g1 + i02 * g2, i01 * g0 + i11 * g1 + i12 * g2);
+  out[4] = make_double2(i02 * g0 + i12 * g1 + i22 * g2, 1.0);
+  if (want_r) {
+    const double d0 = i00, q0 = d0 != 0.0 ? 1.0 / d0 : 0.0, l10 = i01 * q0, l20 = i02 * q0;
+    const double d1 = i11 - l10 * i01, q1 = d1 != 0.0 ? 1.0 / d1 : 0.0, l21 = (i12 - l20 * i01) * q1;
+    const double d2 = i22 - l20 * i02 - l21 * l21 * d1;
+    const double a0 = sqrt(fabs(d0)), a1 = sqrt(fabs(d1)), a2 = sqrt(fabs(d2));
+    out[4].y = 1.0 + (d0 < 0.0 ? 1.0 : 0.0) + (d1 < 0.0 ? 2.0 : 0.0) + (d2 < 0.0 ? 4.0 : 0.0);
+    out[5] = make_double2(a0, l10 * a0);
+    out[6] = make_double2(l20 * a0, a1);
+    out[7] = make_double2(l21 * a1, a2);
+  } else {
+    out[5] = out[6] = out[7] = make_double2(0.0, 0.0);
+  }
+}
 
 #if defined(__HIP_DEVICE_COMPILE__)
 __device__ __forceinline__ void wave_sync() {
diff --git a/3d-reconstruction-from-multi-view-exp_amd/csrc/mvba_create.h b/3d-reconstruction-from-multi-view-exp_amd/csrc/mvba_create.h
--- a/3d-reconstruction-from-multi-view-exp_amd/csrc/mvba_create.h
+++ b/3d-reconstruction-from-multi-view-exp_amd/csrc/mvba_create.h
@@ -56,6 +56,7 @@
   std::vector<int4> splits;
   int n_split_slots = 0;
   bool any_split = false;
+  bool any_empty = false;
 };
 
 K1Tiles build_k1_tiles(const mvba_problem *p) {
@@ -65,6 +66,7 @@
   auto flush = [&](bool split_flag) { t.tiles.push_back(split_flag ? ~(int)cur0 : (int)cur0); };
   for (long long a = 0; a < N; ++a) {
     const long long d = p->pt_ptr[a + 1] - p->pt_ptr[a];
+    if (d == 0) t.any_empty = true;
     if (d > 64) {
       if (fill) { flush(false); cur0 += fill; fill = 0; }
       t.any_split = true;
@@ -617,6 +619,7 @@
   CR(h->mem.alloc(&h->d_xy, nobs));
   h->n_tiles = (int)t.tiles.size() - 1;
   h->any_split = t.any_split;
+  h->can_damp = !t.any_empty;
   if (t.any_split) {
     t.tile_slot.resize(t.tiles.size(), -1);
     h->n_splits = (int)t.splits.size();
@@ -771,10 +774,12 @@
   }
   const size_t k1_lds = k1_lds_bytes(m, h->gcam, h->k1_threads);
   CRH(set_lds(resid_jac_kernel(h->gcam, h->loss).fn(false), k1_lds));
+  CRH(set_lds(resid_jac_kernel(h->gcam, h->loss, true).fn(false), k1_lds));
   CRH(set_lds(cost_kernel(false, h->loss).fn(false), cam_lds));
   CRH(set_lds((const void *)k_residuals<false>, cam_lds));
   if (robust) {
     CRH(set_lds(resid_jac_kernel(h->gcam, h->loss).fn(true), k1_lds));
+    CRH(set_lds(resid_jac_kernel(h->gcam, h->loss, true).fn(true), k1_lds));
     CRH(set_lds(cost_kernel(false, h->loss).fn(true), cam_lds));
   }
   if (h->schur_mode == SCHUR_DENSE) {
diff --git a/3d-reconstruction-from-multi-view-exp_amd/csrc/mvba_init.h b/3d-reconstruction-from-multi-view-exp_amd/csrc/mvba_init.h
--- a/3d-reconstruction-from-multi-view-exp_amd/csrc/mvba_init.h
+++ b/3d-reconstruction-from-multi-view-exp_amd/csrc/mvba_init.h
@@ -452,6 +452,7 @@
   hipLaunchKernelGGL(k_init_cams, dim3((h->m + 255) / 256), dim3(256), 0, h->stream, h->m, h->d_cam15[h->cur], dK, dR, dt);
   MVBA_HIP(hipGetLastError());
   h->linearized = false; h->have_trial = false;
+  drop_damped(h);
   if (h->N == 0) return sync_and_drain(h);
   double ms = 0.0;
   if ((rc = launch_triangulate(h->stream, h->N, h->m, dK, dR, dt, h->d_pt_ptr, h->d_cam, h->d_xy, n_refine, h->d_X[h->cur], dq, dst, 1,
diff --git a/3d-reconstruction-from-multi-view-exp_amd/lib/_mvba.py b/3d-reconstruction-from-multi-view-exp_amd/lib/_mvba.py
--- a/3d-reconstruction-from-multi-view-exp_amd/lib/_mvba.py
+++ b/3d-reconstruction-from-multi-view-exp_amd/lib/_mvba.py
@@ -66,6 +66,8 @@
     "mvba_snapshot_restore": (C.c_int, [C.c_void_p, C.c_int64]),
     "mvba_cost": (C.c_int, [C.c_void_p, _dp]),
     "mvba_linearize": (C.c_int, [C.c_void_p]),
+    "mvba_linearize_damped": (C.c_int, [C.c_void_p, C.c_double]),
+    "mvba_point_inv_launches": (C.c_int64, [C.c_void_p]),
     "mvba_try_step": (C.c_int, [C.c_void_p, C.c_double, _dp]),
     "mvba_commit": (C.c_int, [C.c_void_p]),
     "mvba_set_parameter_map": (C.c_int, [C.c_void_p, C.POINTER(C.c_int32), C.c_int32]),
@@ -278,6 +280,12 @@
     def linearize(self):
         raise_for(self.lib.mvba_linearize(self._h), self.lib)
 
+    def linearize_damped(self, c):
+        raise_for(self.lib.mvba_linearize_damped(self._h, float(c)), self.lib)
+
+    def point_inv_launches(self):
+        return int(self.lib.mvba_point_inv_launches(self._h))
+
     def try_step(self, c):
         E = C.c_double()
         raise_for(self.lib.mvba_try_step(self._h, float(c), C.byref(E)), self.lib)
diff --git a/3d-reconstruction-from-multi-view-exp_amd/lib/bundle_adjustment.py b/3d-reconstruction-from-multi-view-exp_amd/lib/bundle_adjustment.py
--- a/3d-reconstruction-from-multi-view-exp_amd/lib/bundle_adjustment.py
+++ b/3d-reconstruction-from-multi-view-exp_amd/lib/bundle_adjustment.py
@@ -174,7 +174,10 @@
 
     def iterate(self):
         g = self.engine
-        g.linearize()
+        if hasattr(g, "linearize_damped"):
+            g.linearize_damped(self.c)
+        else:
+            g.linearize()
         while True:
             E_ = g.try_step(self.c)
             if E_ > self.E:
diff --git a/include/mvba.h b/include/mvba.h
--- a/include/mvba.h
+++ b/include/mvba.h
@@ -69,6 +69,8 @@
 
 int mvba_cost(mvba_handle *h, double *E);
 int mvba_linearize(mvba_handle *h);
+int mvba_linearize_damped(mvba_handle *h, double c);
+int64_t mvba_point_inv_launches(mvba_handle *h);
 int mvba_try_step(mvba_handle *h, double c, double *E_trial);
 int mvba_commit(mvba_handle *h);
 
```

Result: no change. 431.0, median of 2 (-0.1%).
